# imaranresearch/LAMMPS-SPHERHARM

Hardware: NVIDIA B200
Metric: contact_pair_evals_per_s (higher is better)
Workload: dtype f64

## Files before the change

lammps-spherharm_b200/csrc/device_math.cuh:

```cuda
#pragma once
#include <cuda_runtime.h>
#include <stdint.h>

namespace shgpu {

struct DevShape {
  int lmax, nterms, nq, nchunks;
  double rmax, rmin, rmax2, rmin2, mass, inv_mass;
  double inertia[3], com[3], Rp[9];
  const double *Ap;
  const double2 *ab;
  const double *px, *py, *pz;
  const double *nx, *ny, *nz;
  int n_theta, n_phi;
  int tab_off;
  int nterms4;
  const float *row_x;
  const float2 *cube_ul;
  int cube_n, pad2_;
  const float4 *pf4;
  const float *cube_w2[4];
  double cache_delta[4];
};

__device__ __forceinline__ void quat_to_mat(const double q[4], double R[9]) {
  const double w2 = q[0] * q[0], i2 = q[1] * q[1], j2 = q[2] * q[2], k2 = q[3] * q[3];
  const double twoij = (2.0 * q[1]) * q[2], twoik = (2.0 * q[1]) * q[3], twojk = (2.0 * q[2]) * q[3];
  const double twoiw = (2.0 * q[1]) * q[0], twojw = (2.0 * q[2]) * q[0], twokw = (2.0 * q[3]) * q[0];
  R[0] = ((w2 + i2) - j2) - k2;  R[1] = twoij - twokw;          R[2] = twojw + twoik;
  R[3] = twoij + twokw;          R[4] = ((w2 - i2) + j2) - k2;  R[5] = twojk - twoiw;
  R[6] = twoik - twojw;          R[7] = twojk + twoiw;          R[8] = ((w2 - i2) - j2) + k2;
}

__device__ __forceinline__ double sh_radius_folded(int L, const double *__restrict__ Ap,
                                                   const double2 *__restrict__ ab, double s0, double s1,
                                                   double s2, double rho2, double &rho_out) {
  const double rho = sqrt(rho2);
  const double inv = 1.0 / rho;
  const double x = s2 * inv, zx = s0 * inv, zy = s1 * inv;
  double u = 1.0, v = 0.0, r = 0.0;
  int base = 0;
  for (int m = 0; m <= L; m++) {
    if (m > 0) {
      const double t1 = v * zy, un = fma(u, zx, -t1);
      const double t2 = v * zx, vn = fma(u, zy, t2);
      u = un; v = vn;
    }
    const double2 c0 = ab[base];
    double C = c0.x, S = c0.y;
    const int len = L - m;
    if (len >= 1) {
      double q1 = Ap[base + 1] * x, q2 = 1.0;
      const double2 c1 = ab[base + 1];
      C = fma(c1.x, q1, C); S = fma(c1.y, q1, S);
#pragma unroll 4
      for (int i = 2; i <= len; i++) {
        const double tx = Ap[base + i] * x;
        const double q = fma(tx, q1, -q2);
        const double2 ci = ab[base + i];
        C = fma(ci.x, q, C); S = fma(ci.y, q, S);
        q2 = q1; q1 = q;
      }
    }
    r = fma(u, C, r); r = fma(v, S, r);
    base += len + 1;
  }
  rho_out = rho;
  return r;
}

__device__ __forceinline__ void sh_radius_folded_x2(int L, const double *__restrict__ Ap,
                                                    const double2 *__restrict__ ab, const double sA[3],
                                                    double rhoA2, const double sB[3], double rhoB2, double &rhoA,
                                                    double &rhoB, double &rA_out, double &rB_out) {
  const double rA = sqrt(rhoA2), iA = 1.0 / rA, rB = sqrt(rhoB2), iB = 1.0 / rB;
  const double xA = sA[2] * iA, zxA = sA[0] * iA, zyA = sA[1] * iA;
  const double xB = sB[2] * iB, zxB = sB[0] * iB, zyB = sB[1] * iB;
  double uA = 1.0, vA = 0.0, rrA = 0.0, uB = 1.0, vB = 0.0, rrB = 0.0;
  int base = 0;
  for (int m = 0; m <= L; m++) {
    if (m > 0) {
      const double a1 = vA * zyA, un = fma(uA, zxA, -a1), a2 = vA * zxA, vn = fma(uA, zyA, a2);
      uA = un; vA = vn;
      const double b1 = vB * zyB, wn = fma(uB, zxB, -b1), b2 = vB * zxB, yn = fma(uB, zyB, b2);
      uB = wn; vB = yn;
    }
    const double2 c0 = ab[base];
    double CA = c0.x, SA = c0.y, CB = c0.x, SB = c0.y;
    const int len = L - m;
    if (len >= 1) {
      const double ap1 = Ap[base + 1];
      double qA1 = ap1 * xA, qA2 = 1.0, qB1 = ap1 * xB, qB2 = 1.0;
      const double2 c1 = ab[base + 1];
      CA = fma(c1.x, qA1, CA); SA = fma(c1.y, qA1, SA);
      CB = fma(c1.x, qB1, CB); SB = fma(c1.y, qB1, SB);
#pragma unroll 4
      for (int i = 2; i <= len; i++) {
        const double ap = Ap[base + i];
        const double2 ci = ab[base + i];
        const double txA = ap * xA, txB = ap * xB;
        const double qA = fma(txA, qA1, -qA2), qB = fma(txB, qB1, -qB2);
        CA = fma(ci.x, qA, CA); CB = fma(ci.x, qB, CB);
        SA = fma(ci.y, qA, SA); SB = fma(ci.y, qB, SB);
        qA2 = qA1; qA1 = qA; qB2 = qB1; qB1 = qB;
      }
    }
    rrA = fma(uA, CA, rrA); rrA = fma(vA, SA, rrA);
    rrB = fma(uB, CB, rrB); rrB = fma(vB, SB, rrB);
    base += len + 1;
  }
  rhoA = rA; rhoB = rB; rA_out = rrA; rB_out = rrB;
}

template <int N>
__device__ __forceinline__ void sh_radius_folded_n(int L, const double *__restrict__ Ap, const double2 *__restrict__ ab,
                                                   const double (&s)[N][3], const double (&rho2)[N], double (&rho)[N],
                                                   double (&r_out)[N]) {
  double x[N], zx[N], zy[N], u[N], v[N], rr[N];
#pragma unroll
  for (int p = 0; p < N; p++) {
    rho[p] = sqrt(rho2[p]);
    const double inv = 1.0 / rho[p];
    x[p] = s[p][2] * inv; zx[p] = s[p][0] * inv; zy[p] = s[p][1] * inv;
    u[p] = 1.0; v[p] = 0.0; rr[p] = 0.0;
  }
  int base = 0;
  for (int m = 0; m <= L; m++) {
    if (m > 0) {
#pragma unroll
      for (int p = 0; p < N; p++) {
        const double t1 = v[p] * zy[p], un = fma(u[p], zx[p], -t1), t2 = v[p] * zx[p], vn = fma(u[p], zy[p], t2);
        u[p] = un; v[p] = vn;
      }
    }
    const double2 c0 = ab[base];
    double C[N], S[N];
#pragma unroll
    for (int p = 0; p < N; p++) { C[p] = c0.x; S[p] = c0.y; }
    const int len = L - m;
    if (len >= 1) {
      const double ap1 = Ap[base + 1];
      const double2 c1 = ab[base + 1];
      double q1[N], q2[N];
#pragma unroll
      for (int p = 0; p < N; p++) {
        q1[p] = ap1 * x[p]; q2[p] = 1.0;
        C[p] = fma(c1.x, q1[p], C[p]); S[p] = fma(c1.y, q1[p], S[p]);
      }
#pragma unroll 2
      for (int i = 2; i <= len; i++) {
        const double ap = Ap[base + i];
        const double2 ci = ab[base + i];
        double q[N];
#pragma unroll
        for (int p = 0; p < N; p++) { const double tx = ap * x[p]; q[p] = fma(tx, q1[p], -q2[p]); }
#pragma unroll
        for (int p = 0; p < N; p++) C[p] = fma(ci.x, q[p], C[p]);
#pragma unroll
        for (int p = 0; p < N; p++) S[p] = fma(ci.y, q[p], S[p]);
#pragma unroll
        for (int p = 0; p < N; p++) { q2[p] = q1[p]; q1[p] = q[p]; }
      }
    }
#pragma unroll
    for (int p = 0; p < N; p++) { rr[p] = fma(u[p], C[p], rr[p]); rr[p] = fma(v[p], S[p], rr[p]); }
    base += len + 1;
  }
#pragma unroll
  for (int p = 0; p < N; p++) r_out[p] = rr[p];
}

__device__ __forceinline__ double warp_sum(double v) {
#pragma unroll
  for (int o = 16; o > 0; o >>= 1) v += __shfl_xor_sync(0xffffffffu, v, o);
  return v;
}

__device__ __forceinline__ void omega_from_angmom(const double q[4], const double L[3], const double I[3],
                                                  double w[3]) {
  double R[9];
  quat_to_mat(q, R);
  double wb[3];
#pragma unroll
  for (int k = 0; k < 3; k++) {
    const double lb = R[k] * L[0] + R[3 + k] * L[1] + R[6 + k] * L[2];
    wb[k] = (I[k] > 0) ? lb / I[k] : 0.0;
  }
#pragma unroll
  for (int r = 0; r < 3; r++) w[r] = R[3 * r] * wb[0] + R[3 * r + 1] * wb[1] + R[3 * r + 2] * wb[2];
}

}
```

lammps-spherharm_b200/csrc/pair_split_kernels.cuh:

```cuda
#pragma once
#include "pair_kernel.cuh"

namespace shgpu {

#define SPLIT_CAP 88
#define SURV_CAP 320
#define CACHE_CAP 384

struct __align__(16) SurvRec {
  double s0, s1, s2;
  int k;
  int flag;
};

struct __align__(16) PdEntry {
  long long off;
  int cnt;
  unsigned short ntrans;
  unsigned short cnt2;
  unsigned int off2;
  unsigned short nin;
  unsigned short in[5];
};
#define PD_INLINE 5

struct __align__(16) PairHot {
  int i, j, n0, n1;
  long long off;
  int img;
  unsigned char shp_i, shp_j, pad0, pad1;
};

struct EvalPlanDev {
  int total_blocks, nshape;
  int blk_start[SH_MAX_SHAPES + 1];
  long long count[SH_MAX_SHAPES];
};

struct SplitScalars {
  unsigned long long pool_count[SH_MAX_SHAPES];
  unsigned long long in_count;
  int nbig;
  int nslow;
  int slow_counter;
  int deep_counter;
};

struct SplitArgs {
  SurvRec *pool;
  unsigned char *pool_flag;
  const long long *pool_base;
  const long long *pool_cap;
  SplitScalars *sc;
  PdEntry *pd;
  int *big_list;
  int *slow_list;
  int *inpool;
  long long in_cap;
};

struct CacheArgs {
  unsigned short *pool;
  PairHot *hot;
  unsigned long long *count;
  long long cap;
  int *overflow;
  const int *invalid;
  int enabled;
  int level;
};

__device__ __forceinline__ float fp32_margin(float t0, float t1, float t2, float ra) {
  const float sc = sqrtf(fmaf(t2, t2, fmaf(t1, t1, t0 * t0))) + ra;
  return 1.9073486e-6f * sc * sc;
}

struct NodeWindow { bool skip; float cosA, xe, se, phie; };

__device__ __forceinline__ NodeWindow make_window(const DevShape &sa, double Rb, const double *x0) {
  NodeWindow w;
  const double e0 = 2.0 * x0[0], e1 = 2.0 * x0[1], e2 = 2.0 * x0[2];
  const double D2 = e0 * e0 + e1 * e1 + e2 * e2, D = sqrt(D2);
  w.skip = D >= (sa.rmax + Rb) * (1.0 + 1e-9);
  w.cosA = -2.0f; w.xe = 1.0f; w.se = 0.0f; w.phie = 0.0f;
  if (!w.skip && D > 1e-9 * (sa.rmax + Rb)) {
    const double q = D2 - Rb * Rb;
    double rc = sa.rmin;
    if (q > 0) rc = fmin(fmax(sqrt(q), sa.rmin), sa.rmax);
    const double g = (rc * rc + q) / (2.0 * rc * D);
    w.cosA = (float)g - 3e-5f;
    if (w.cosA >= 1.0f) w.skip = true;
    w.xe = fminf(1.0f, fmaxf(-1.0f, (float)(e2 / D)));
    w.se = sqrtf(fmaxf(0.0f, 1.0f - w.xe * w.xe));
    w.phie = atan2f((float)e1, (float)e0);
    if (w.phie < 0.0f) w.phie += 6.2831853f;
  }
  return w;
}

__device__ __forceinline__ void classify_row(const DevShape &sa, const NodeWindow &w, int row, int &c0, int &ccount) {
  c0 = 0; ccount = 0;
  const int nph = sa.n_phi;
  if (row >= sa.n_theta) return;
  if (w.cosA <= -1.0f) { ccount = nph; return; }
  const float xa = sa.row_x[row];
  const float sarow = sqrtf(fmaxf(0.0f, 1.0f - xa * xa));
  const float ss = sarow * w.se, xx = xa * w.xe;
  if (xx + ss < w.cosA) return;
  const float cd = (ss > 1e-12f) ? (w.cosA - xx) / ss : -2.0f;
  if (cd <= -1.0f) { ccount = nph; return; }
  const float inv_dphi = (float)nph * 0.15915494f;
  const float dl = acosf(fminf(cd, 1.0f)) + 2e-4f;
  const int b0 = (int)ceilf((w.phie - dl) * inv_dphi - 0.5f);
  const int b1 = (int)floorf((w.phie + dl) * inv_dphi - 0.5f);
  ccount = b1 - b0 + 1;
  if (ccount >= nph) { ccount = nph; c0 = 0; }
  else if (ccount > 0) { c0 = b0 % nph; if (c0 < 0) c0 += nph; }
  else ccount = 0;
}

__device__ __forceinline__ int cube_cell(float f0, float f1, float f2, int cn) {
  const float ax = fabsf(f0), ay = fabsf(f1), az = fabsf(f2);
  int face; float ma, uu, vv;
  if (ax >= ay && ax >= az) { face = f0 > 0 ? 0 : 1; ma = ax; uu = f1; vv = f2; }
  else if (ay >= az) { face = f1 > 0 ? 2 : 3; ma = ay; uu = f0; vv = f2; }
  else { face = f2 > 0 ? 4 : 5; ma = az; uu = f0; vv = f1; }
  const float im = __fdividef(1.0f, fmaxf(ma, 1e-30f)), hn = 0.5f * (float)cn;
  const int iu = min(cn - 1, max(0, (int)((uu * im + 1.0f) * hn)));
  const int iv = min(cn - 1, max(0, (int)((vv * im + 1.0f) * hn)));
  return (face * cn + iu) * cn + iv;
}

__device__ __forceinline__ double pose_element(const PairArgs &A, int a, int b, double dd0, double dd1, double dd2, int l) {
  const int st = A.stride;
  if (l < 9) {
    const int r = l / 3, k = l - 3 * r;
    double m = A.Rs[(0 + r) * st + b] * A.Rs[(0 + k) * st + a];
    m = fma(A.Rs[(3 + r) * st + b], A.Rs[(3 + k) * st + a], m);
    m = fma(A.Rs[(6 + r) * st + b], A.Rs[(6 + k) * st + a], m);
    return m;
  } else if (l < 12) {
    const int r = l - 9;
    double tt = A.Rs[(0 + r) * st + b] * dd0;
    tt = fma(A.Rs[(3 + r) * st + b], dd1, tt);
    tt = fma(A.Rs[(6 + r) * st + b], dd2, tt);
    return tt;
  }
  const int r = l - 12;
  double hx = A.Rs[(0 + r) * st + a] * dd0;
  hx = fma(A.Rs[(3 + r) * st + a], dd1, hx);
  hx = fma(A.Rs[(6 + r) * st + a], dd2, hx);
  return -0.5 * hx;
}
__device__ __forceinline__ void pose_to_smem(const PairArgs &A, int a, int b, double dd0, double dd1, double dd2, int lane,
                                             double *pose) {
  __syncwarp();
  if (lane < 15) pose[lane] = pose_element(A, a, b, dd0, dd1, dd2, lane);
  __syncwarp();
}

__device__ __forceinline__ int exact_node_stage(const double *M, const double *t, double p0, double p1, double p2, double rmax2,
                                                double rmin2, const float2 *__restrict__ cube, int cn, int use_bounds,
                                                double &s0, double &s1, double &s2) {
  s0 = fma(M[0], p0, t[0]); s0 = fma(M[1], p1, s0); s0 = fma(M[2], p2, s0);
  s1 = fma(M[3], p0, t[1]); s1 = fma(M[4], p1, s1); s1 = fma(M[5], p2, s1);
  s2 = fma(M[6], p0, t[2]); s2 = fma(M[7], p1, s2); s2 = fma(M[8], p2, s2);
  const double rho2 = fma(s2, s2, fma(s1, s1, s0 * s0));
  if (!(rho2 < rmax2)) return -1;
  if (rho2 <= rmin2) return 2;
  if (!use_bounds) return 0;
  const float2 ul = __ldg(&cube[cube_cell((float)s0, (float)s1, (float)s2, cn)]);
  if (rho2 <= (double)ul.y) return 2;
  return rho2 < (double)ul.x ? 0 : -1;
}

template <int WPB>
__global__ void __launch_bounds__(WPB * 32) pair_cache_build_kernel(PairArgs A, CacheArgs C, const int *list, const int *nlist) {
  __shared__ unsigned short s_buf[WPB][2][CACHE_CAP];
  __shared__ double s_pose[WPB][16];
  const int lane = threadIdx.x & 31, warp = threadIdx.x >> 5;
  const int nwork = list ? *nlist : A.npairs;
  for (int w = blockIdx.x * WPB + warp; w < nwork; w += gridDim.x * WPB) {
  const int p = list ? list[w] : w;
  const int i = A.pair_i[p], j = A.pair_j[p];
  double d[3];
  pair_separation(A, p, i, j, d);
  const int shp_i = A.shape[i], shp_j = A.shape[j];
  double *pose = s_pose[warp];
  int cnt0 = 0, cnt1 = 0;
  bool over = false;
  for (int dir = 0; dir < 2 && !over; dir++) {
    const int a = dir ? j : i, b = dir ? i : j;
    const DevShape &sa = A.shapes[dir ? shp_j : shp_i];
    const DevShape &sb = A.shapes[dir ? shp_i : shp_j];
    const double sgn = dir ? -1.0 : 1.0;
    pose_to_smem(A, a, b, sgn * d[0], sgn * d[1], sgn * d[2], lane, pose);
    const double *M = pose, *t = pose + 9, *x0 = pose + 12;
    const double delta = sb.cache_delta[C.level], Rb = sb.rmax + delta;
    const NodeWindow w = make_window(sa, Rb, x0);
    const float4 *__restrict__ pf = sa.pf4;
    const float *__restrict__ cube = sb.cube_w2[C.level];
    const int cn = sb.cube_n, nph = sa.n_phi, nth = sa.n_theta;
    const float fM0 = (float)M[0], fM1 = (float)M[1], fM2 = (float)M[2], fM3 = (float)M[3], fM4 = (float)M[4],
                fM5 = (float)M[5], fM6 = (float)M[6], fM7 = (float)M[7], fM8 = (float)M[8];
    const float ft0 = (float)t[0], ft1 = (float)t[1], ft2 = (float)t[2];
    const float eps = fp32_margin(ft0, ft1, ft2, (float)sa.rmax);
    const float fR2 = (float)(Rb * Rb) + eps;
    const float fin = (float)((sb.rmin + 2.0 * delta) * (sb.rmin + 2.0 * delta)) + eps;
    unsigned short *buf = s_buf[warp][dir];
    int n = 0;
    if (!w.skip) {
      for (int rb = 0; rb < nth && !over; rb += 32) {
        int c0, ccount;
        classify_row(sa, w, rb + lane, c0, ccount);
        unsigned rows = __ballot_sync(0xffffffffu, ccount > 0);
        while (rows && !over) {
          const int rl = __ffs(rows) - 1;
          rows &= rows - 1;
          const int rc0 = __shfl_sync(0xffffffffu, c0, rl), rcount = __shfl_sync(0xffffffffu, ccount, rl);
          const int rowbase = (rb + rl) * nph;
          for (int cb = 0; cb < rcount; cb += 32) {
            const int cc = cb + lane;
            bool pass = false;
            int k = 0;
            if (cc < rcount) {
              int col = rc0 + cc;
              if (col >= nph) col -= nph;
              k = rowbase + col;
              const float4 q = __ldg(&pf[k]);
              const float f0 = fmaf(fM2, q.z, fmaf(fM1, q.y, fmaf(fM0, q.x, ft0)));
              const float f1 = fmaf(fM5, q.z, fmaf(fM4, q.y, fmaf(fM3, q.x, ft1)));
              const float f2 = fmaf(fM8, q.z, fmaf(fM7, q.y, fmaf(fM6, q.x, ft2)));
              const float r2 = fmaf(f2, f2, fmaf(f1, f1, f0 * f0));
              if (r2 < fR2) pass = (r2 < fin) || (r2 < __ldg(&cube[cube_cell(f0, f1, f2, cn)]) + eps);
            }
            const unsigned pm = __ballot_sync(0xffffffffu, pass);
            if (pm) {
              const int nnew = __popc(pm);
              if (n + nnew > CACHE_CAP) { over = true; break; }
              if (pass) buf[n + __popc(pm & ((1u << lane) - 1u))] = (unsigned short)k;
              n += nnew;
            }
          }
        }
      }
    }
    if (dir) cnt1 = n; else cnt0 = n;
    __syncwarp();
  }
  const int ntot = cnt0 + cnt1;
  long long off = 0;
  if (lane == 0 && !over && ntot > 0) off = (long long)atomicAdd(C.count, (unsigned long long)ntot);
  off = __shfl_sync(0xffffffffu, off, 0);
  if (!over && ntot > 0) {
    if (off + ntot <= C.cap) {
      for (int r = lane; r < cnt0; r += 32) C.pool[off + r] = s_buf[warp][0][r];
      for (int r = lane; r < cnt1; r += 32) C.pool[off + cnt0 + r] = s_buf[warp][1][r];
    } else { if (lane == 0) *C.overflow = 1; over = true; }
  }
  if (lane == 0) {
    PairHot hrec;
    hrec.i = i; hrec.j = j; hrec.n0 = over ? -1 : cnt0; hrec.n1 = over ? -1 : cnt1; hrec.off = off; hrec.img = A.pair_img[p];
    hrec.shp_i = (unsigned char)shp_i; hrec.shp_j = (unsigned char)shp_j; hrec.pad0 = 0; hrec.pad1 = 0;
    C.hot[p] = hrec;
  }
  __syncwarp();
  }
}

__global__ void cache_remap_kernel(PairArgs A, const int *old_half_off, const int *old_pair_j, int old_nown, const PairHot *old_hot,
                                   const unsigned short *old_pool, CacheArgs C, int *fresh_list, int *nfresh, const int *amap) {
  const int p = blockIdx.x * blockDim.x + threadIdx.x;
  const int lane = threadIdx.x & 31;
  int ntot = 0, q = -1;
  PairHot hrec;
  hrec.i = hrec.j = 0; hrec.n0 = hrec.n1 = 0; hrec.off = 0; hrec.img = 0; hrec.shp_i = hrec.shp_j = 0; hrec.pad0 = hrec.pad1 = 0;
  if (p < A.npairs) {
    const int i = A.pair_i[p], j = A.pair_j[p], img = A.pair_img[p];
    const int oi = amap ? amap[i] : i, oj = amap ? amap[j] : j;
    if (oi >= 0 && oj >= 0 && oi < old_nown && oi < oj)
      for (int e = old_half_off[oi]; e < old_half_off[oi + 1]; e++)
        if (old_pair_j[e] == oj) { q = e; break; }
    if (q >= 0) {
      hrec = old_hot[q];
      if (hrec.n0 < 0 || hrec.img != img || hrec.i != oi || hrec.j != oj) q = -1;
      hrec.i = i; hrec.j = j;
    }
    if (q >= 0) ntot = hrec.n0 + hrec.n1;
    else fresh_list[atomicAdd(nfresh, 1)] = p;
  }
  int pre = ntot;
#pragma unroll
  for (int o = 1; o < 32; o <<= 1) { const int t = __shfl_up_sync(0xffffffffu, pre, o); if (lane >= o) pre += t; }
  const int wtot = __shfl_sync(0xffffffffu, pre, 31);
  long long base = 0;
  if (lane == 31 && wtot > 0) base = (long long)atomicAdd(C.count, (unsigned long long)wtot);
  base = __shfl_sync(0xffffffffu, base, 31);
  if (q >= 0) {
    const long long off = base + (pre - ntot);
    if (off + ntot <= C.cap) {
      const unsigned short *src = old_pool + hrec.off;
      for (int r = 0; r < ntot; r++) C.pool[off + r] = src[r];
      hrec.off = off;
    } else { *C.overflow = 1; hrec.n0 = -1; hrec.n1 = -1; hrec.off = 0; }
    C.hot[p] = hrec;
  }
}

__device__ __forceinline__ void store_pd(PdEntry *dst, long long off, int cnt, int ntrans, int nin, const unsigned short *in,
                                         unsigned int off2 = 0, int cnt2 = 0) {
  PdEntry e;
  e.off = off; e.cnt = cnt; e.ntrans = (unsigned short)ntrans; e.nin = (unsigned short)nin; e.off2 = off2; e.cnt2 = (unsigned short)cnt2;
#pragma unroll
  for (int q = 0; q < PD_INLINE; q++) e.in[q] = (in && q < nin) ? in[q] : (unsigned short)0;
  *dst = e;
}

struct ShapeLite {
  const float4 *pf4; const float2 *cube_ul; const double *px, *py, *pz;
  int cube_n, pad_;
  double rmax, rmax2, rmin2;
};
struct ShapeLiteTable { ShapeLite s[SH_MAX_SHAPES]; };

template <int WPB, int LPP>
__global__ void __launch_bounds__(WPB * 32, 32 / WPB) pair_cull_cached_kernel(PairArgs A, SplitArgs S, CacheArgs C, int use_bounds,
                                                                              const __grid_constant__ ShapeLiteTable T) {
  constexpr int PPW = 32 / LPP, U = 2;
  constexpr unsigned FULLSUB = LPP == 32 ? 0xffffffffu : ((1u << LPP) - 1u);
  __shared__ double s_dpose[WPB][PPW][2][12];
  __shared__ float s_fpose[WPB][PPW][2][12];
  __shared__ unsigned short s_surv[WPB][PPW][SURV_CAP];
  __shared__ signed char s_flag[WPB][PPW][SURV_CAP];
  __shared__ unsigned short s_in[WPB][PPW][2][8];
  const int lane = threadIdx.x & 31, warp = threadIdx.x >> 5;
  const int sub = lane / LPP, sl = lane % LPP, shift = sub * LPP;
  const int p = (blockIdx.x * WPB + warp) * PPW + sub;
  if (*C.invalid) return;
  const bool inrange = p < A.npairs;
  PairHot hot;
  hot.i = hot.j = 0; hot.n0 = hot.n1 = 0; hot.off = 0; hot.img = 21; hot.shp_i = hot.shp_j = 0;
  if (inrange) {
    const int4 *hp = reinterpret_cast<const int4 *>(C.hot + p);
    const int4 h0 = __ldg(hp), h1 = __ldg(hp + 1);
    hot.i = h0.x; hot.j = h0.y; hot.n0 = h0.z; hot.n1 = h0.w;
    hot.off = (long long)(((unsigned long long)(unsigned)h1.y << 32) | (unsigned)h1.x);
    hot.img = h1.z; hot.shp_i = (unsigned char)(h1.w & 255); hot.shp_j = (unsigned char)((h1.w >> 8) & 255);
  }
  if (inrange && hot.n0 < 0 && sl == 0) S.slow_list[atomicAdd(&S.sc->nslow, 1)] = p;
  const bool cached = inrange && hot.n0 >= 0;
  const int n0 = cached ? hot.n0 : 0, n1 = cached ? hot.n1 : 0, ntot = n0 + n1;
  if (cached && ntot == 0 && sl < 2) store_pd(&S.pd[2 * p + sl], 0, 0, 0, 0, nullptr);
  const int maxtot = __reduce_max_sync(0xffffffffu, ntot);
  if (maxtot == 0) return;
  const bool work = ntot > 0;
  const int i = hot.i, j = hot.j, shp_i = hot.shp_i, shp_j = hot.shp_j;
  const ShapeLite &si = T.s[shp_i], &sj = T.s[shp_j];
  if (work) {
    const int st = A.stride;
    double d[3];
#pragma unroll
    for (int k = 0; k < 3; k++) {
      double dk = A.c[k * st + i] - A.c[k * st + j];
      const int n = ((hot.img >> (2 * k)) & 3) - 1;
      if (n != 0) dk = dk - A.boxlen[k] * (double)n;
      d[k] = dk;
    }
    if (sl < 15) {
      const int half = sl >= 12, l = half ? sl - 3 : sl;
      const double sgn = half ? -1.0 : 1.0;
      const double val = pose_element(A, half ? j : i, half ? i : j, sgn * d[0], sgn * d[1], sgn * d[2], l);
      s_dpose[warp][sub][half][l] = val;
      s_fpose[warp][sub][half][l] = (float)val;
      if (sl < 9) {
        const int r = sl / 3, k = sl - 3 * r;
        s_dpose[warp][sub][1][3 * k + r] = val;
        s_fpose[warp][sub][1][3 * k + r] = (float)val;
      }
    }
  }
  __syncwarp();
  const float4 *__restrict__ pf_i = si.pf4, *__restrict__ pf_j = sj.pf4;
  const float2 *__restrict__ cube_i = si.cube_ul, *__restrict__ cube_j = sj.cube_ul;
  const int cn_i = si.cube_n, cn_j = sj.cube_n;
  const float eps0 = fp32_margin(s_fpose[warp][sub][0][9], s_fpose[warp][sub][0][10], s_fpose[warp][sub][0][11], (float)si.rmax);
  const float eps1 = fp32_margin(s_fpose[warp][sub][1][9], s_fpose[warp][sub][1][10], s_fpose[warp][sub][1][11], (float)sj.rmax);
  const float fR20 = (float)sj.rmax2 + eps0, fR21 = (float)si.rmax2 + eps1;
  const unsigned short *__restrict__ cl = C.pool + hot.off;
  unsigned short *surv = s_surv[warp][sub];
  signed char *sflag = s_flag[warp][sub];
  int nsurv = 0, ns0 = 0;
  bool big = false;
  for (int base = 0; base < maxtot; base += LPP * U) {
    int k[U];
    float4 q[U];
    bool pass[U];
#pragma unroll
    for (int u = 0; u < U; u++) {
      const int g = base + LPP * u + sl;
      k[u] = (work && !big && g < ntot) ? (int)__ldg(&cl[g]) : -1;
    }
#pragma unroll
    for (int u = 0; u < U; u++) {
      const int dirc = (base + LPP * u + sl) >= n0;
      q[u] = k[u] >= 0 ? __ldg(&(dirc ? pf_j : pf_i)[k[u]]) : make_float4(0.f, 0.f, 0.f, 0.f);
    }
#pragma unroll
    for (int u = 0; u < U; u++) {
      const int dirc = (base + LPP * u + sl) >= n0;
      const float *fp = s_fpose[warp][sub][dirc];
      const float f0 = fmaf(fp[2], q[u].z, fmaf(fp[1], q[u].y, fmaf(fp[0], q[u].x, fp[9])));
      const float f1 = fmaf(fp[5], q[u].z, fmaf(fp[4], q[u].y, fmaf(fp[3], q[u].x, fp[10])));
      const float f2 = fmaf(fp[8], q[u].z, fmaf(fp[7], q[u].y, fmaf(fp[6], q[u].x, fp[11])));
      const float r2 = fmaf(f2, f2, fmaf(f1, f1, f0 * f0));
      bool ok = k[u] >= 0 && r2 < (dirc ? fR21 : fR20);
      if (ok && use_bounds) ok = r2 < __ldg(&(dirc ? cube_i : cube_j)[cube_cell(f0, f1, f2, dirc ? cn_i : cn_j)]).x + (dirc ? eps1 : eps0);
      pass[u] = ok;
    }
#pragma unroll
    for (int u = 0; u < U; u++) {
      const unsigned mine = (__ballot_sync(0xffffffffu, pass[u]) >> shift) & FULLSUB;
      if (mine) {
        const int nnew = __popc(mine);
        if (nsurv + nnew > SURV_CAP) big = true;
        else {
          if (pass[u]) surv[nsurv + __popc(mine & ((1u << sl) - 1u))] = (unsigned short)k[u];
          const int nd0 = n0 - (base + LPP * u);
          ns0 += nd0 >= LPP ? nnew : (nd0 <= 0 ? 0 : __popc(mine & ((1u << nd0) - 1u)));
          nsurv += nnew;
        }
      }
    }
  }
  __syncwarp();
  const bool live = work && !big;
  const int maxs = __reduce_max_sync(0xffffffffu, live ? nsurv : 0);
  int c0d0 = 0, c0d1 = 0, c2d0 = 0, c2d1 = 0;
  for (int gb = 0; gb < maxs; gb += LPP) {
    const int g = gb + sl;
    int fl = -1;
    if (live && g < nsurv) {
      const int dirc = g >= ns0, k = surv[g];
      const ShapeLite &sa = dirc ? sj : si;
      const ShapeLite &sb = dirc ? si : sj;
      const double *M = s_dpose[warp][sub][dirc];
      double s0, s1, s2;
      fl = exact_node_stage(M, M + 9, sa.px[k], sa.py[k], sa.pz[k], sb.rmax2, sb.rmin2, sb.cube_ul, sb.cube_n, use_bounds, s0, s1, s2);
      sflag[g] = (signed char)fl;
    }
    const unsigned m0 = (__ballot_sync(0xffffffffu, fl == 0) >> shift) & FULLSUB;
    const unsigned m2 = (__ballot_sync(0xffffffffu, fl == 2) >> shift) & FULLSUB;
    const int nd0 = ns0 - gb;
    const unsigned md0 = nd0 >= LPP ? FULLSUB : (nd0 <= 0 ? 0u : ((1u << nd0) - 1u));
    c0d0 += __popc(m0 & md0); c0d1 += __popc(m0 & ~md0);
    c2d0 += __popc(m2 & md0); c2d1 += __popc(m2 & ~md0);
  }
  const int r0 = c0d0, r1 = c0d1, x0 = max(0, c2d0 - PD_INLINE), x1 = max(0, c2d1 - PD_INLINE);
  long long off0 = 0, off1 = 0, xoff = 0;
  if (live && sl == 0 && r0 > 0) off0 = (long long)atomicAdd(&S.sc->pool_count[shp_j], (unsigned long long)r0);
  if (live && sl == 1 && r1 > 0) off1 = (long long)atomicAdd(&S.sc->pool_count[shp_i], (unsigned long long)r1);
  if (live && sl == 2 && x0 + x1 > 0) xoff = (long long)atomicAdd(&S.sc->in_count, (unsigned long long)(x0 + x1));
  off0 = __shfl_sync(0xffffffffu, off0, shift);
  off1 = __shfl_sync(0xffffffffu, off1, shift + 1);
  xoff = __shfl_sync(0xffffffffu, xoff, shift + 2);
  if (live && (off0 + r0 > S.pool_cap[shp_j] || off1 + r1 > S.pool_cap[shp_i] || xoff + x0 + x1 > S.in_cap)) big = true;
  if (work && big && sl == 0) {
    store_pd(&S.pd[2 * p], 0, -1, 0, 0, nullptr);
    store_pd(&S.pd[2 * p + 1], 0, -1, 0, 0, nullptr);
    S.big_list[atomicAdd(&S.sc->nbig, 1)] = p;
  }
  const bool wr = work && !big;
  const long long base0 = S.pool_base[shp_j] + off0, base1 = S.pool_base[shp_i] + off1;
  int w0d0 = 0, w0d1 = 0, w2d0 = 0, w2d1 = 0;
  for (int gb = 0; gb < maxs; gb += LPP) {
    const int g = gb + sl;
    const bool v = wr && g < nsurv;
    const int fl = v ? (int)sflag[g] : -1;
    const unsigned m0 = (__ballot_sync(0xffffffffu, fl == 0) >> shift) & FULLSUB;
    const unsigned m2 = (__ballot_sync(0xffffffffu, fl == 2) >> shift) & FULLSUB;
    const int nd0 = ns0 - gb;
    const unsigned md0 = nd0 >= LPP ? FULLSUB : (nd0 <= 0 ? 0u : ((1u << nd0) - 1u));
    const unsigned lt = (1u << sl) - 1u;
    if (fl >= 0) {
      const int dirc = g >= ns0, k = surv[g];
      const unsigned dm = dirc ? ~md0 : md0;
      const int rank0 = (dirc ? w0d1 : w0d0) + __popc(m0 & dm & lt);
      const int rank2 = (dirc ? w2d1 : w2d0) + __popc(m2 & dm & lt);
      int slot = -1;
      if (fl == 0) slot = rank0;
      else if (rank2 < PD_INLINE) s_in[warp][sub][dirc][rank2] = (unsigned short)k;
      else S.inpool[xoff + (dirc ? x0 : 0) + (rank2 - PD_INLINE)] = k;
      if (slot >= 0) {
        const ShapeLite &sa = dirc ? sj : si;
        const double *M = s_dpose[warp][sub][dirc], *t = M + 9;
        const double p0 = sa.px[k], p1 = sa.py[k], p2 = sa.pz[k];
        SurvRec r;
        r.s0 = fma(M[0], p0, t[0]); r.s0 = fma(M[1], p1, r.s0); r.s0 = fma(M[2], p2, r.s0);
        r.s1 = fma(M[3], p0, t[1]); r.s1 = fma(M[4], p1, r.s1); r.s1 = fma(M[5], p2, r.s1);
        r.s2 = fma(M[6], p0, t[2]); r.s2 = fma(M[7], p1, r.s2); r.s2 = fma(M[8], p2, r.s2);
        r.k = k; r.flag = fl;
        const long long idx = (dirc ? base1 : base0) + slot;
        S.pool[idx] = r;
        S.pool_flag[idx] = 0;
      }
    }
    w0d0 += __popc(m0 & md0); w0d1 += __popc(m0 & ~md0);
    w2d0 += __popc(m2 & md0); w2d1 += __popc(m2 & ~md0);
  }
  __syncwarp();
  if (wr && sl < 2) {
    if (sl == 0) store_pd(&S.pd[2 * p], base0, r0, n0, min(c2d0, PD_INLINE), s_in[warp][sub][0], (unsigned int)xoff, x0);
    else store_pd(&S.pd[2 * p + 1], base1, r1, n1, min(c2d1, PD_INLINE), s_in[warp][sub][1], (unsigned int)(xoff + x0), x1);
  }
}

template <int WPB>
__global__ void __launch_bounds__(WPB * 32) pair_cull_window_kernel(PairArgs A, SplitArgs S, CacheArgs C, int use_bounds) {
  __shared__ __align__(16) SurvRec s_rec[WPB][2][SPLIT_CAP];
  __shared__ double s_pose[WPB][16];
  __shared__ unsigned short s_cand[WPB][64];
  __shared__ unsigned short s_in[WPB][2][8];
  const int lane = threadIdx.x & 31, warp = threadIdx.x >> 5;
  const bool all = !C.enabled || *C.invalid != 0;
  for (;;) {
    int w = 0;
    if (lane == 0) w = atomicAdd(&S.sc->slow_counter, 1);
    w = __shfl_sync(0xffffffffu, w, 0);
    const int nwork = all ? A.npairs : *(volatile int *)&S.sc->nslow;
    if (w >= nwork) break;
    const int p = all ? w : S.slow_list[w];
    const int i = A.pair_i[p], j = A.pair_j[p];
    double d[3];
    pair_separation(A, p, i, j, d);
    const int shp_i = A.shape[i], shp_j = A.shape[j];
    double *pose = s_pose[warp];
    int cnt0 = 0, cnt1 = 0, nin0 = 0, nin1 = 0, nt0 = 0, nt1 = 0;
    bool big = false;
    for (int dir = 0; dir < 2 && !big; dir++) {
      const int a = dir ? j : i, b = dir ? i : j;
      const DevShape &sa = A.shapes[dir ? shp_j : shp_i];
      const DevShape &sb = A.shapes[dir ? shp_i : shp_j];
      const double sgn = dir ? -1.0 : 1.0;
      pose_to_smem(A, a, b, sgn * d[0], sgn * d[1], sgn * d[2], lane, pose);
      const double *M = pose, *t = pose + 9, *x0 = pose + 12;
      const double rmax2 = sb.rmax2, rmin2 = sb.rmin2;
      const double *__restrict__ nodes = sa.px;
      const int nq = sa.nq;
      const float2 *__restrict__ cube = sb.cube_ul;
      const int cn = sb.cube_n;
      SurvRec *buf = s_rec[warp][dir];
      unsigned short *cand = s_cand[warp], *inl = s_in[warp][dir];
      int queued = 0, nin = 0, n_trans = 0;
      auto exact_stage = [&](bool valid, int k) {
        int flag = -1;
        double s0 = 0, s1 = 0, s2 = 0;
        if (valid) flag = exact_node_stage(M, t, nodes[k], nodes[nq + k], nodes[2 * nq + k], rmax2, rmin2, cube, cn, use_bounds, s0, s1, s2);
        const unsigned m2 = __ballot_sync(0xffffffffu, flag == 2);
        const int rank2 = nin + __popc(m2 & ((1u << lane) - 1u));
        const bool inline_it = flag == 2 && rank2 < PD_INLINE;
        if (inline_it) inl[rank2] = (unsigned short)k;
        nin = min(PD_INLINE, nin + __popc(m2));
        const bool rec = flag >= 0 && !inline_it;
        const unsigned sm = __ballot_sync(0xffffffffu, rec);
        if (sm) {
          const int nnew = __popc(sm);
          if (queued + nnew > SPLIT_CAP) { big = true; return; }
          if (rec) {
            SurvRec r; r.s0 = s0; r.s1 = s1; r.s2 = s2; r.k = k; r.flag = flag;
            buf[queued + __popc(sm & ((1u << lane) - 1u))] = r;
          }
          queued += nnew;
        }
      };
      const NodeWindow wd = make_window(sa, sb.rmax, x0);
      if (!wd.skip) {
        const float4 *__restrict__ pf = sa.pf4;
        const float fM0 = (float)M[0], fM1 = (float)M[1], fM2 = (float)M[2], fM3 = (float)M[3], fM4 = (float)M[4],
                    fM5 = (float)M[5], fM6 = (float)M[6], fM7 = (float)M[7], fM8 = (float)M[8];
        const float ft0 = (float)t[0], ft1 = (float)t[1], ft2 = (float)t[2];
        const float eps = fp32_margin(ft0, ft1, ft2, (float)sa.rmax);
        const float frmax2 = (float)rmax2 + eps;
        const int nth = sa.n_theta, nph = sa.n_phi;
        int ncand = 0;
        for (int rb = 0; rb < nth && !big; rb += 32) {
          int c0, ccount;
          classify_row(sa, wd, rb + lane, c0, ccount);
          unsigned rows = __ballot_sync(0xffffffffu, ccount > 0);
          while (rows && !big) {
            const int rl = __ffs(rows) - 1;
            rows &= rows - 1;
            const int rc0 = __shfl_sync(0xffffffffu, c0, rl), rcount = __shfl_sync(0xffffffffu, ccount, rl);
            const int rowbase = (rb + rl) * nph;
            for (int cb = 0; cb < rcount && !big; cb += 32) {
              const int cc = cb + lane;
              bool pass = false;
              int k = 0;
              if (cc < rcount) {
                int col = rc0 + cc;
                if (col >= nph) col -= nph;
                k = rowbase + col;
                const float4 q = __ldg(&pf[k]);
                const float f0 = fmaf(fM2, q.z, fmaf(fM1, q.y, fmaf(fM0, q.x, ft0)));
                const float f1 = fmaf(fM5, q.z, fmaf(fM4, q.y, fmaf(fM3, q.x, ft1)));
                const float f2 = fmaf(fM8, q.z, fmaf(fM7, q.y, fmaf(fM6, q.x, ft2)));
                const float r2 = fmaf(f2, f2, fmaf(f1, f1, f0 * f0));
                if (r2 < frmax2) pass = !use_bounds || r2 < __ldg(&cube[cube_cell(f0, f1, f2, cn)]).x + eps;
              }
              n_trans += min(32, rcount - cb);
              const unsigned pm = __ballot_sync(0xffffffffu, pass);
              if (pm) {
                if (pass) cand[ncand + __popc(pm & ((1u << lane) - 1u))] = (unsigned short)k;
                ncand += __popc(pm);
                __syncwarp();
                if (ncand >= 32) {
                  exact_stage(true, (int)cand[lane]);
                  __syncwarp();
                  const int rem = ncand - 32;
                  unsigned short mv = 0;
                  if (lane < rem) mv = cand[32 + lane];
                  __syncwarp();
                  if (lane < rem) cand[lane] = mv;
                  ncand = rem;
                  __syncwarp();
                }
              }
            }
          }
        }
        if (!big && ncand > 0) { exact_stage(lane < ncand, lane < ncand ? (int)cand[lane] : 0); __syncwarp(); }
      }
      if (dir) { cnt1 = queued; nin1 = nin; nt1 = n_trans; } else { cnt0 = queued; nin0 = nin; nt0 = n_trans; }
    }
    __syncwarp();
    long long off0 = 0, off1 = 0;
    if (!big) {
      if (lane == 0 && cnt0 > 0) off0 = (long long)atomicAdd(&S.sc->pool_count[shp_j], (unsigned long long)cnt0);
      if (lane == 1 && cnt1 > 0) off1 = (long long)atomicAdd(&S.sc->pool_count[shp_i], (unsigned long long)cnt1);
      off0 = __shfl_sync(0xffffffffu, off0, 0);
      off1 = __shfl_sync(0xffffffffu, off1, 1);
      if (off0 + cnt0 > S.pool_cap[shp_j] || off1 + cnt1 > S.pool_cap[shp_i]) big = true;
    }
    if (big) {
      if (lane == 0) {
        store_pd(&S.pd[2 * p], 0, -1, 0, 0, nullptr);
        store_pd(&S.pd[2 * p + 1], 0, -1, 0, 0, nullptr);
        S.big_list[atomicAdd(&S.sc->nbig, 1)] = p;
      }
    } else {
      const long long base0 = S.pool_base[shp_j] + off0, base1 = S.pool_base[shp_i] + off1;
      for (int r = lane; r < cnt0; r += 32) { S.pool[base0 + r] = s_rec[warp][0][r]; S.pool_flag[base0 + r] = s_rec[warp][0][r].flag == 2 ? 1 : 0; }
      for (int r = lane; r < cnt1; r += 32) { S.pool[base1 + r] = s_rec[warp][1][r]; S.pool_flag[base1 + r] = s_rec[warp][1][r].flag == 2 ? 1 : 0; }
      if (lane == 0) store_pd(&S.pd[2 * p], base0, cnt0, nt0, nin0, s_in[warp][0]);
      if (lane == 1) store_pd(&S.pd[2 * p + 1], base1, cnt1, nt1, nin1, s_in[warp][1]);
    }
    __syncwarp();
  }
}

__global__ void eval_plan_kernel(SplitArgs S, int nshape, int recs_per_block, EvalPlanDev *plan) {
  if (threadIdx.x != 0 || blockIdx.x != 0) return;
  int nblk = 0;
  for (int s = 0; s < nshape; s++) {
    const long long cnt = min((long long)S.sc->pool_count[s], S.pool_cap[s]);
    plan->blk_start[s] = nblk;
    plan->count[s] = cnt;
    nblk += (int)((cnt + recs_per_block - 1) / recs_per_block);
  }
  plan->blk_start[nshape] = nblk;
  plan->total_blocks = nblk;
  plan->nshape = nshape;
}

template <int WPB, int PTS, int MINB>
__global__ void __launch_bounds__(WPB * 32, MINB) pair_eval_kernel(const DevShape *shapes, SplitArgs S, const EvalPlanDev *plan,
                                                                   unsigned long long *counters, int chunked) {
  extern __shared__ __align__(16) unsigned char smem_raw[];
  constexpr int RPW = 32 * PTS;
  const int total = plan->total_blocks, nshape = plan->nshape;
  const int chunk = (total + (int)gridDim.x - 1) / (int)gridDim.x;
  const int b0 = chunked ? blockIdx.x * chunk : blockIdx.x, b1 = chunked ? min(total, b0 + chunk) : total;
  const int bstep = chunked ? 1 : (int)gridDim.x;
  if (b0 >= b1) return;
  const int lane = threadIdx.x & 31, warp = threadIdx.x >> 5;
  double2 *s_ab = reinterpret_cast<double2 *>(smem_raw);
  double *s_Ap = nullptr;
  int cur = -1, s = 0;
  unsigned long long nev_total = 0;
  for (int blk = b0; blk < b1; blk += bstep) {
    while (s + 1 < nshape && blk >= plan->blk_start[s + 1]) s++;
    const DevShape &sh = shapes[s];
    if (s != cur) {
      __syncthreads();
      s_Ap = reinterpret_cast<double *>(s_ab + sh.nterms4 + 4);
      for (int t = threadIdx.x; t < sh.nterms4 + 4; t += WPB * 32) { s_ab[t] = sh.ab[t]; s_Ap[t] = sh.Ap[t]; }
      __syncthreads();
      cur = s;
    }
    const long long n = plan->count[s];
    const long long r0 = ((long long)(blk - plan->blk_start[s]) * WPB + warp) * RPW;
    if (r0 >= n) continue;
    SurvRec *rec = S.pool + S.pool_base[s];
    unsigned char *flg = S.pool_flag + S.pool_base[s];
    const int L = sh.lmax;
    int nev = 0;
    if (PTS == 2) {
      const long long ia = r0 + lane, ib = r0 + 32 + lane;
      const bool va = ia < n, vb = ib < n;
      if (__ballot_sync(0xffffffffu, vb)) {
        const long long ja = va ? ia : r0, jb = vb ? ib : ja;
        const SurvRec ra = rec[ja], rb = rec[jb];
        const double sA[3] = {ra.s0, ra.s1, ra.s2}, sB[3] = {rb.s0, rb.s1, rb.s2};
        const double rhoA2 = fma(sA[2], sA[2], fma(sA[1], sA[1], sA[0] * sA[0]));
        const double rhoB2 = fma(sB[2], sB[2], fma(sB[1], sB[1], sB[0] * sB[0]));
        double rhoA, rhoB, rA, rB;
        sh_radius_folded_x2(L, s_Ap, s_ab, sA, rhoA2, sB, rhoB2, rhoA, rhoB, rA, rB);
        if (va && ra.flag == 0) { flg[ia] = rhoA < rA ? 1 : 0; nev++; }
        if (vb && rb.flag == 0) { flg[ib] = rhoB < rB ? 1 : 0; nev++; }
      } else if (va) {
        const SurvRec ra = rec[ia];
        const double rho2 = fma(ra.s2, ra.s2, fma(ra.s1, ra.s1, ra.s0 * ra.s0));
        double rho;
        const double r = sh_radius_folded(L, s_Ap, s_ab, ra.s0, ra.s1, ra.s2, rho2, rho);
        if (ra.flag == 0) { flg[ia] = rho < r ? 1 : 0; nev++; }
      }
    } else {
      double sv[PTS][3], rho2[PTS], rho[PTS], rr[PTS];
      int fl[PTS];
      long long idx[PTS];
#pragma unroll
      for (int q = 0; q < PTS; q++) {
        idx[q] = r0 + 32 * q + lane;
        const bool v = idx[q] < n;
        const SurvRec r = rec[v ? idx[q] : r0];
        sv[q][0] = r.s0; sv[q][1] = r.s1; sv[q][2] = r.s2;
        fl[q] = v ? r.flag : 3;
        rho2[q] = fma(r.s2, r.s2, fma(r.s1, r.s1, r.s0 * r.s0));
      }
      sh_radius_folded_n<PTS>(L, s_Ap, s_ab, sv, rho2, rho, rr);
#pragma unroll
      for (int q = 0; q < PTS; q++)
        if (fl[q] == 0) { flg[idx[q]] = rho[q] < rr[q] ? 1 : 0; nev++; }
    }
    nev_total += nev;
  }
  nev_total = __reduce_add_sync(0xffffffffu, (unsigned)nev_total);
  if (lane == 0 && nev_total) { atomicAdd(&counters[2], nev_total); atomicAdd(&counters[5], nev_total); }
}

struct NodeSums { double S0, S1, S2, Av, T0, T1, T2, G0, G1, G2; int n; };

__device__ __forceinline__ void add_node(NodeSums &a, const double *__restrict__ nodes, int nq, int k, const double x0[3]) {
  const double p0 = nodes[k], p1 = nodes[nq + k], p2 = nodes[2 * nq + k];
  const double n0 = nodes[3 * nq + k], n1 = nodes[4 * nq + k], n2 = nodes[5 * nq + k];
  const double dp0 = p0 - x0[0], dp1 = p1 - x0[1], dp2 = p2 - x0[2];
  const double dn = fma(dp2, n2, fma(dp1, n1, dp0 * n0));
  a.S0 += n0; a.S1 += n1; a.S2 += n2;
  a.Av += dn;
  a.T0 += fma(p1, n2, -(p2 * n1));
  a.T1 += fma(p2, n0, -(p0 * n2));
  a.T2 += fma(p0, n1, -(p1 * n0));
  a.G0 = fma(dp0, dn, a.G0); a.G1 = fma(dp1, dn, a.G1); a.G2 = fma(dp2, dn, a.G2);
  a.n++;
}

template <int MINB>
__global__ void __launch_bounds__(128, MINB) pair_reduce_kernel(PairArgs A, SplitArgs S) {
  const int p = blockIdx.x * blockDim.x + threadIdx.x;
  int c_pairs = 0, c_trans = 0, c_inside = 0, c_ghost = 0;
  if (p < A.npairs) {
    const int4 *ep = reinterpret_cast<const int4 *>(S.pd + 2 * (size_t)p);
    const int4 e0a = __ldg(ep), e0b = __ldg(ep + 1), e1a = __ldg(ep + 2), e1b = __ldg(ep + 3);
    const int cnt0 = e0a.z, cnt1 = e1a.z;
    if (cnt0 >= 0) {
      const int i = A.pair_i[p], j = A.pair_j[p];
      c_pairs = 1; c_trans = (e0a.w & 0xffff) + (e1a.w & 0xffff); c_ghost = j >= A.nlocal;
      const int nin0 = e0b.y & 0xffff, nin1 = e1b.y & 0xffff;
      const int xc0 = (e0a.w >> 16) & 0xffff, xc1 = (e1a.w >> 16) & 0xffff;
      double out[14];
#pragma unroll
      for (int r = 0; r < 14; r++) out[r] = 0.0;
      const long long off0 = (long long)(((unsigned long long)(unsigned)e0a.y << 32) | (unsigned)e0a.x);
      const long long off1 = (long long)(((unsigned long long)(unsigned)e1a.y << 32) | (unsigned)e1a.x);
      unsigned long long msk0 = 0, msk1 = 0;
      bool any = nin0 > 0 || nin1 > 0 || xc0 > 0 || xc1 > 0;
      {
        const int m0 = min(cnt0, 64), m1 = min(cnt1, 64);
        for (int r = 0; r < m0; r += 8) {
#pragma unroll
          for (int q = 0; q < 8; q++) if (r + q < m0 && S.pool_flag[off0 + r + q]) msk0 |= 1ull << (r + q);
        }
        for (int r = 0; r < m1; r += 8) {
#pragma unroll
          for (int q = 0; q < 8; q++) if (r + q < m1 && S.pool_flag[off1 + r + q]) msk1 |= 1ull << (r + q);
        }
        any = any || msk0 || msk1 || cnt0 > 64 || cnt1 > 64;
      }
      if (any) {
        const int st = A.stride;
        double d[3];
        pair_separation(A, p, i, j, d);
        const int shp_i = A.shape[i], shp_j = A.shape[j];
        double Ss[2][3], Ts[2][3], Gs[2][3], Asum[2];
        int ninside_pair = 0;
#pragma unroll
        for (int dir = 0; dir < 2; dir++) {
          const int a = dir ? j : i;
          const DevShape &sa = A.shapes[dir ? shp_j : shp_i];
          const double sgn = dir ? -1.0 : 1.0;
          const long long off = dir ? off1 : off0;
          const int cnt = dir ? cnt1 : cnt0, nin = dir ? nin1 : nin0, xc = dir ? xc1 : xc0;
          unsigned long long msk = dir ? msk1 : msk0;
          const int4 eb = dir ? e1b : e0b;
          NodeSums acc;
          acc.S0 = acc.S1 = acc.S2 = acc.Av = acc.T0 = acc.T1 = acc.T2 = acc.G0 = acc.G1 = acc.G2 = 0.0; acc.n = 0;
          double Ra[9];
#pragma unroll
          for (int e = 0; e < 9; e++) Ra[e] = A.Rs[e * st + a];
          if (msk || nin > 0 || cnt > 64 || xc > 0) {
            double x0[3];
#pragma unroll
            for (int r = 0; r < 3; r++) {
              double hx = Ra[0 + r] * (sgn * d[0]);
              hx = fma(Ra[3 + r], sgn * d[1], hx);
              hx = fma(Ra[6 + r], sgn * d[2], hx);
              x0[r] = -0.5 * hx;
            }
            const double *__restrict__ nodes = sa.px;
            const int nq = sa.nq;
            while (msk) {
              const int r = __ffsll((long long)msk) - 1;
              msk &= msk - 1;
              add_node(acc, nodes, nq, S.pool[off + r].k, x0);
            }
            for (int r = 64; r < cnt; r++)
              if (S.pool_flag[off + r]) add_node(acc, nodes, nq, S.pool[off + r].k, x0);
            {
              const unsigned xo = (unsigned)eb.x;
              for (int r = 0; r < xc; r++) add_node(acc, nodes, nq, S.inpool[xo + r], x0);
            }
            for (int q = 0; q < nin; q++) {
              const int h = q + 3;
              const unsigned w = (h >> 1) == 0 ? (unsigned)eb.x : (h >> 1) == 1 ? (unsigned)eb.y : (h >> 1) == 2 ? (unsigned)eb.z : (unsigned)eb.w;
              add_node(acc, nodes, nq, (int)((w >> (16 * (h & 1))) & 0xffffu), x0);
            }
          }
#pragma unroll
          for (int r = 0; r < 3; r++) {
            Ss[dir][r] = Ra[3 * r] * acc.S0 + Ra[3 * r + 1] * acc.S1 + Ra[3 * r + 2] * acc.S2;
            Ts[dir][r] = Ra[3 * r] * acc.T0 + Ra[3 * r + 1] * acc.T1 + Ra[3 * r + 2] * acc.T2;
            Gs[dir][r] = 0.25 * (Ra[3 * r] * acc.G0 + Ra[3 * r + 1] * acc.G1 + Ra[3 * r + 2] * acc.G2);
          }
          Asum[dir] = acc.Av;
          ninside_pair += acc.n;
        }
        c_inside = ninside_pair;
        const double V = Asum[0] / 3.0 + Asum[1] / 3.0;
        if (ninside_pair > 0 && V > 0) {
          const double kk = A.pk[shp_i * SH_MAX_SHAPES + shp_j], mm = A.pm[shp_i * SH_MAX_SHAPES + shp_j];
          double E, pr;
          if (mm == 1.0) { E = kk * V; pr = kk; }
          else { const double pw = pow(V, mm - 1.0); E = kk * pw * V; pr = mm * kk * pw; }
          out[0] = V; out[1] = E;
          double li[3], lj[3];
#pragma unroll
          for (int r = 0; r < 3; r++) {
            li[r] = A.c[r * st + i] - A.x[r * st + i];
            lj[r] = A.c[r * st + j] - A.x[r * st + j];
          }
          const double *Sij = Ss[0], *Sji = Ss[1], *Tij = Ts[0], *Tji = Ts[1];
          const double Ti[3] = {Tij[0] + (li[1] * Sij[2] - li[2] * Sij[1]), Tij[1] + (li[2] * Sij[0] - li[0] * Sij[2]),
                                Tij[2] + (li[0] * Sij[1] - li[1] * Sij[0])};
          const double Tj[3] = {Tji[0] + (lj[1] * Sji[2] - lj[2] * Sji[1]), Tji[1] + (lj[2] * Sji[0] - lj[0] * Sji[2]),
                                Tji[2] + (lj[0] * Sji[1] - lj[1] * Sji[0])};
#pragma unroll
          for (int r = 0; r < 3; r++) {
            out[2 + r] = -pr * (0.5 * (Sij[r] - Sji[r]));
            out[5 + r] = -pr * Ti[r];
            out[8 + r] = -pr * Tj[r];
            out[11 + r] = (A.c[r * st + i] - 0.5 * d[r]) + (Gs[0][r] + Gs[1][r]) / V;
          }
          if (A.dissip) contact_dissipation(A, i, j, shp_i, shp_j, d, lj, out);
        }
      }
#pragma unroll
      for (int r = 0; r < 14; r++) A.pres[(size_t)r * A.pres_stride + p] = out[r];
      const int eij = A.pair_eij[p], eji = A.pair_eji[p];
#pragma unroll
      for (int r = 0; r < 3; r++) {
        A.slot[(size_t)r * A.slot_stride + eij] = out[2 + r];
        A.slot[(size_t)(3 + r) * A.slot_stride + eij] = out[5 + r];
        if (eji >= 0) {
          A.slot[(size_t)r * A.slot_stride + eji] = -out[2 + r];
          A.slot[(size_t)(3 + r) * A.slot_stride + eji] = out[8 + r];
        }
      }
    }
  }
  c_pairs = __reduce_add_sync(0xffffffffu, c_pairs); c_trans = __reduce_add_sync(0xffffffffu, c_trans);
  c_inside = __reduce_add_sync(0xffffffffu, c_inside); c_ghost = __reduce_add_sync(0xffffffffu, c_ghost);
  if ((threadIdx.x & 31) == 0) {
    if (c_pairs) atomicAdd(&A.counters[0], (unsigned long long)c_pairs);
    if (c_trans) atomicAdd(&A.counters[1], (unsigned long long)c_trans);
    if (c_inside) atomicAdd(&A.counters[3], (unsigned long long)c_inside);
    if (c_ghost) atomicAdd(&A.counters[4], (unsigned long long)c_ghost);
  }
}

}
```

lammps-spherharm_b200/csrc/shgpu_api.cu:

```cuda
#include <cuda_runtime.h>

#include <algorithm>
#include <cmath>
#include <cstdio>
#include <cstring>
#include <string>
#include <vector>

#include "../../include/shgpu.h"
#include "devbuf.h"
#include "dd_types.h"
#include "neighbor_kernels.cuh"
#include "pair_kernel.cuh"
#include "pair_warp_kernel.cuh"
#include "pair_split_kernels.cuh"
#include "shape_tables.h"
#include "step_kernels.cuh"
#include "atom_stress_kernels.cuh"

using namespace shgpu;

namespace {

struct ShapeDev {
  DevBuf<double> Ap, node;
  DevBuf<double2> ab;
  DevBuf<float> row_x, cubew[SH_CACHE_LEVELS];
  DevBuf<float2> cube;
  DevBuf<float4> pf4;
};

}

enum { CACHE_INVALID = 0, CACHE_VALID = 1, CACHE_REMAP = 2 };

struct sh_ctx {
  std::string err;
  int device = 0, sm_count = 148;
  cudaStream_t stream = nullptr;
  double lo[3] = {-1e30, -1e30, -1e30}, hi[3] = {1e30, 1e30, 1e30};
  int periodic[3] = {0, 0, 0};
  bool box_set = false;
  int n_theta = 32, n_phi = 64;
  std::vector<ShapeTables> shapes;
  std::vector<ShapeDev> shape_dev;
  std::vector<DevShape> shape_host_view;
  DevBuf<DevShape> d_shapes;
  bool shapes_dirty = true;
  int total_terms = 0;
  std::vector<double> pk, pm;
  std::vector<double> pgn, pgt, pmu;
  bool dissip = false;
  DevBuf<double> d_pk, d_pm, d_pgn, d_pgt, d_pmu, stress_part;
  bool coeff_dirty = true;
  WallSet walls{};
  double g[3] = {0, 0, 0}, skin = 0.0, dt = 1e-4, gamma_lin = 0.0, gamma_rot = 0.0;
  int neigh_every = 1, neigh_check = 1;
  int64_t n = 0, nghost = 0;
  int stride = 0;
  DevBuf<double> x, v, q, L, f, tq, c, Rs, c0, wallf, ewall, ke;
  DevBuf<int> shape;
  std::vector<int64_t> tag;
  DevBuf<long long> d_tag;
  bool tags_host_valid = true;
  DevBuf<double> gf;
  double time = 0.0;
  DdCtx dd;
  int *h_lagflag = nullptr;
  cudaEvent_t ev_lag[2] = {nullptr, nullptr};
  int lag_slot = 0; bool lag_pending = false, lag_mode = true, lag_pred_valid = false;
  bool cache_sync_ranks = false;
  int64_t step_index = 0, cache_build_step = -10;
  double cache_time = 0.0;
  bool step_trace = false;
  std::vector<cudaEvent_t> ev_step;
  std::vector<float> step_ms;
  std::vector<int> step_flags, step_flags_last;
  DevBuf<int> cell_of, cell_count, cell_start, cell_fill, cell_atoms, tile_sum, cnt_full, cnt_half, nbr_off, half_off,
      nbr_j, pair_i, pair_j, pair_eij, pair_eji, pair_img, scalars;
  DevBuf<double> bbox, slot, pres, stage;
  DevBuf<SurvRec> pool;
  DevBuf<unsigned char> pool_flag;
  DevBuf<long long> pool_base, pool_cap;
  DevBuf<PdEntry> pd;
  DevBuf<PairHot> cache_hot[2];
  DevBuf<SplitScalars> split_sc;
  DevBuf<EvalPlanDev> eval_plan;
  DevBuf<int> big_list, slow_list, split_flags;
  DevBuf<int> inpool;
  long long h_in_cap = 0;
  std::vector<long long> h_pool_cap;
  unsigned long long *h_pool_count = nullptr;
  SplitScalars *h_split_sc = nullptr;
  int *h_cache_invalid = nullptr;
  cudaEvent_t ev_sc = nullptr;
  bool sc_pending = false;
  int sc_nshape = 0;
  double sec_eval = 0, sec_cull = 0, sec_reduce = 0, sec_deep = 0, sec_cache = 0; int64_t eval_launches = 0;
  std::vector<int> ev2_kind;
  int64_t big_pairs = 0, slow_pairs = 0, pool_grows = 0, cache_builds = 0;
  int cache_level = 0, cache_level_pin = -1;
  int64_t cache_age = 0;
  bool cache_exhausted = false;
  int cube_n = 0;
  int reduce_occ = 0;
  int eval_pts = 0, eval_occ = 0, eval_mode = 0;
  long long last_records = 0;
  DevBuf<unsigned short> cache_pool[2];
  DevBuf<int> old_half_off, old_pair_j, fresh_list;
  int old_nown = 0, cache_cur = 0;
  DevBuf<double> old_c, old_cc0, old_cq0;
  DevBuf<long long> old_tag;
  DevBuf<int> ghost_hash, amap;
  int old_n = 0, old_stride = 0, ghost_hash_size = 0;
  bool carry = false;
  int64_t cache_remaps = 0, atoms_epoch = 0, cache_epoch = -1;
  DevBuf<unsigned long long> cache_count;
  long long cache_cap = 0;
  int cache_state = 0;
  DevBuf<double> cc0, cq0, drift;
  bool eval_pending = false;
  DevBuf<unsigned long long> counters;
  int npairs = 0, nentries = 0, nrows = 0;
  int slot_stride = 0, pres_stride = 0;
  int *h_pinned = nullptr;
  bool forces_valid = false, list_valid = false;
  int64_t steps_since_build = 0;
  int64_t neighbor_builds = 0, kernel_launches = 0;
  std::vector<cudaEvent_t> ev, ev2;
  size_t ev_used = 0, ev2_used = 0;
  double sec_pair = 0, sec_neigh = 0, sec_comm = 0, sec_other = 0, sec_run_last = 0, sec_run_total = 0;
  cudaEvent_t run_e0 = nullptr, run_e1 = nullptr;
  int64_t pair_launches = 0;
  DevBuf<double> as_vir, as_kin, as_en, as_send, as_recv;
  DevBuf<int> as_cnt, as_epair;
  int tune_threads = 0, tune_ctas_per_sm = 0, tune_variant = 0, tune_cull_wpb = 0, tune_cull_lpp = 0;
};

namespace {

int fail(sh_ctx *h, const std::string &m) { h->err = m; return -1; }
int cuda_fail(sh_ctx *h, const char *where, cudaError_t e) {
  h->err = std::string(where) + ": " + cudaGetErrorString(e);
  return -2;
}
#define CU(call) do { cudaError_t _e = (call); if (_e != cudaSuccess) return cuda_fail(h, #call, _e); } while (0)

inline int cdiv(int64_t a, int b) { return (int)((a + b - 1) / b); }

AtomView view(sh_ctx *h) {
  AtomView A;
  A.x = h->x.p; A.v = h->v.p; A.q = h->q.p; A.L = h->L.p; A.f = h->f.p; A.tq = h->tq.p;
  A.c = h->c.p; A.Rs = h->Rs.p; A.c0 = h->c0.p; A.wallf = h->wallf.p; A.shape = h->shape.p;
  A.cc0 = h->cc0.p; A.cq0 = h->cq0.p;
  A.n = (int)(h->n - h->nghost); A.stride = h->stride;
  return A;
}
AtomView view_all(sh_ctx *h) { AtomView A = view(h); A.n = (int)h->n; return A; }

int upload_shapes(sh_ctx *h) {
  if (!h->shapes_dirty) return 0;
  const int ns = (int)h->shapes.size();
  h->shape_dev.resize(ns);
  h->shape_host_view.resize(ns);
  try {
    for (int s = 0; s < ns; s++) {
      const ShapeTables &t = h->shapes[s];
      ShapeDev &d = h->shape_dev[s];
      if (d.Ap.p) continue;
      const int tpad = (t.nterms + 3) / 4 * 4 + 4;
      d.Ap.ensure(tpad); d.ab.ensure(tpad); d.node.ensure((size_t)6 * t.nq); d.row_x.ensure(t.n_theta);
      CU(cudaMemset(d.Ap.p, 0, tpad * sizeof(double))); CU(cudaMemset(d.ab.p, 0, tpad * sizeof(double2)));
      {
        std::vector<float> rx(t.row_x.begin(), t.row_x.end());
        CU(cudaMemcpy(d.row_x.p, rx.data(), rx.size() * sizeof(float), cudaMemcpyHostToDevice));
        std::vector<float4> pf((size_t)t.nq);
        for (int k = 0; k < t.nq; k++) pf[k] = make_float4((float)t.node_p[0][k], (float)t.node_p[1][k], (float)t.node_p[2][k], 0.0f);
        d.pf4.ensure(pf.size());
        CU(cudaMemcpy(d.pf4.p, pf.data(), pf.size() * sizeof(float4), cudaMemcpyHostToDevice));
        for (int lv = 0; lv < SH_CACHE_LEVELS; lv++) {
          d.cubew[lv].ensure(t.cube_wide2[lv].size());
          CU(cudaMemcpy(d.cubew[lv].p, t.cube_wide2[lv].data(), t.cube_wide2[lv].size() * sizeof(float), cudaMemcpyHostToDevice));
        }
        std::vector<float2> ul(t.cube_ub2.size());
        for (size_t c = 0; c < ul.size(); c++) ul[c] = make_float2(t.cube_ub2[c], t.cube_lb2[c]);
        d.cube.ensure(ul.size());
        CU(cudaMemcpy(d.cube.p, ul.data(), ul.size() * sizeof(float2), cudaMemcpyHostToDevice));
      }
      std::vector<double2> ab(t.nterms);
      for (int k = 0; k < t.nterms; k++) ab[k] = make_double2(t.ah[k], t.bh[k]);
      CU(cudaMemcpy(d.Ap.p, t.Ap.data(), t.nterms * sizeof(double), cudaMemcpyHostToDevice));
      CU(cudaMemcpy(d.ab.p, ab.data(), t.nterms * sizeof(double2), cudaMemcpyHostToDevice));
      for (int e = 0; e < 3; e++) {
        CU(cudaMemcpy(d.node.p + (size_t)e * t.nq, t.node_p[e].data(), t.nq * sizeof(double), cudaMemcpyHostToDevice));
        CU(cudaMemcpy(d.node.p + (size_t)(3 + e) * t.nq, t.node_n[e].data(), t.nq * sizeof(double), cudaMemcpyHostToDevice));
      }
      DevShape &v = h->shape_host_view[s];
      v.lmax = t.lmax; v.nterms = t.nterms; v.nq = t.nq; v.nchunks = (t.nq + 31) / 32;
      v.rmax = t.rmax; v.rmin = t.rmin; v.rmax2 = t.rmax * t.rmax; v.rmin2 = t.rmin * t.rmin;
      v.mass = t.mass; v.inv_mass = 1.0 / t.mass;
      for (int e = 0; e < 3; e++) { v.inertia[e] = t.inertia[e]; v.com[e] = t.com[e]; }
      for (int r = 0; r < 3; r++) for (int cidx = 0; cidx < 3; cidx++) v.Rp[3 * r + cidx] = t.Rp[r][cidx];
      v.Ap = d.Ap.p; v.ab = d.ab.p;
      v.px = d.node.p; v.py = d.node.p + t.nq; v.pz = d.node.p + 2 * (size_t)t.nq;
      v.nx = d.node.p + 3 * (size_t)t.nq; v.ny = d.node.p + 4 * (size_t)t.nq; v.nz = d.node.p + 5 * (size_t)t.nq;
      v.n_theta = t.n_theta; v.n_phi = t.n_phi; v.nterms4 = (t.nterms + 3) / 4 * 4; v.row_x = d.row_x.p; v.cube_ul = d.cube.p; v.cube_n = t.cube_n; v.pad2_ = 0; v.pf4 = d.pf4.p;
      for (int lv = 0; lv < SH_CACHE_LEVELS; lv++) { v.cube_w2[lv] = d.cubew[lv].p; v.cache_delta[lv] = t.cache_delta[lv]; }
    }
    int off = 0;
    for (int s = 0; s < ns; s++) { h->shape_host_view[s].tab_off = off; off += h->shape_host_view[s].nterms4 + 4; }
    h->total_terms = off;
    h->d_shapes.ensure(std::max(ns, 1));
  } catch (std::string &e) { return fail(h, e); }
  if (ns) CU(cudaMemcpy(h->d_shapes.p, h->shape_host_view.data(), ns * sizeof(DevShape), cudaMemcpyHostToDevice));
  h->shapes_dirty = false;
  return 0;
}

int upload_coeffs(sh_ctx *h) {
  if (!h->coeff_dirty) return 0;
  const size_t nn = SH_MAX_SHAPES * SH_MAX_SHAPES;
  try { h->d_pk.ensure(nn); h->d_pm.ensure(nn); h->d_pgn.ensure(nn); h->d_pgt.ensure(nn); h->d_pmu.ensure(nn); }
  catch (std::string &e) { return fail(h, e); }
  CU(cudaMemcpy(h->d_pk.p, h->pk.data(), nn * sizeof(double), cudaMemcpyHostToDevice));
  CU(cudaMemcpy(h->d_pm.p, h->pm.data(), nn * sizeof(double), cudaMemcpyHostToDevice));
  CU(cudaMemcpy(h->d_pgn.p, h->pgn.data(), nn * sizeof(double), cudaMemcpyHostToDevice));
  CU(cudaMemcpy(h->d_pgt.p, h->pgt.data(), nn * sizeof(double), cudaMemcpyHostToDevice));
  CU(cudaMemcpy(h->d_pmu.p, h->pmu.data(), nn * sizeof(double), cudaMemcpyHostToDevice));
  h->coeff_dirty = false;
  return 0;
}

int exclusive_scan(sh_ctx *h, const int *in, int *out, int n, int *d_total) {
  const int ntiles = std::max(1, cdiv(n, SCAN_TILE));
  try { h->tile_sum.ensure(ntiles); } catch (std::string &e) { return fail(h, e); }
  scan_tile_kernel<<<ntiles, SCAN_THREADS, 0, h->stream>>>(in, out, h->tile_sum.p, n);
  scan_sums_kernel<<<1, 1024, 0, h->stream>>>(h->tile_sum.p, ntiles, d_total);
  scan_add_kernel<<<std::max(1, cdiv(n, 256)), 256, 0, h->stream>>>(out, h->tile_sum.p, n, d_total);
  h->kernel_launches += 3;
  return 0;
}

int ev_tick(sh_ctx *h, int kind) {
  if (h->ev2_used + 2 > h->ev2.size()) return 0;
  h->ev2_kind[h->ev2_used / 2] = kind;
  if (cudaEventRecord(h->ev2[h->ev2_used], h->stream) != cudaSuccess) return -2;
  return 0;
}
void ev_tock(sh_ctx *h) {
  if (h->ev2_used + 2 <= h->ev2.size()) { cudaEventRecord(h->ev2[h->ev2_used + 1], h->stream); h->ev2_used += 2; }
}

int build_neighbors(sh_ctx *h) {
  const int n = (int)h->n, st = h->stride, nown = (int)(h->n - h->nghost);
  if (ev_tick(h, 5)) return -2;
  const bool keep_cache = h->carry || (h->cache_state == CACHE_VALID && h->list_valid && h->nghost == 0 && h->npairs > 0 && h->atoms_epoch == h->cache_epoch);
  if (keep_cache && !h->carry) {
    try { h->old_half_off.ensure((size_t)nown + 2); h->old_pair_j.ensure((size_t)h->npairs + 1); } catch (std::string &e) { return fail(h, e); }
    CU(cudaMemcpyAsync(h->old_half_off.p, h->half_off.p, ((size_t)nown + 1) * sizeof(int), cudaMemcpyDeviceToDevice, h->stream));
    CU(cudaMemcpyAsync(h->old_pair_j.p, h->pair_j.p, (size_t)h->npairs * sizeof(int), cudaMemcpyDeviceToDevice, h->stream));
    h->old_nown = nown;
  }
  CU(cudaMemsetAsync(h->scalars.p + 1, 0, sizeof(int), h->stream));
  double rmaxg = 0;
  for (auto &s : h->shapes) rmaxg = std::max(rmaxg, s.rmax);
  const double cut = 2.0 * rmaxg + h->skin;
  BinGrid G;
  G.skin = h->skin;
  bool need_bbox = false;
  for (int d = 0; d < 3; d++) {
    G.periodic[d] = h->periodic[d];
    G.boxlen[d] = h->hi[d] - h->lo[d];
    if (h->periodic[d]) {
      if (G.boxlen[d] < 2.0 * cut) return fail(h, "periodic box shorter than 2x cutoff");
    } else need_bbox = true;
  }
  double bmin[3] = {0, 0, 0}, bmax[3] = {0, 0, 0};
  if (need_bbox && n > 0) {
    auto enc = [](double v) { long long b; std::memcpy(&b, &v, 8); return b >= 0 ? b : (b ^ 0x7fffffffffffffffLL); };
    auto dec = [](long long b) { long long u = b >= 0 ? b : (b ^ 0x7fffffffffffffffLL); double v; std::memcpy(&v, &u, 8); return v; };
    long long init[6];
    for (int d = 0; d < 3; d++) { init[d] = enc(1e300); init[3 + d] = enc(-1e300); }
    CU(cudaMemcpyAsync(h->bbox.p, init, sizeof init, cudaMemcpyHostToDevice, h->stream));
    bbox_kernel<<<std::min(1024, cdiv(n, 256)), 256, 0, h->stream>>>(h->c.p, n, st, h->bbox.p);
    h->kernel_launches++;
    long long out[6];
    CU(cudaMemcpyAsync(out, h->bbox.p, sizeof out, cudaMemcpyDeviceToHost, h->stream));
    CU(cudaStreamSynchronize(h->stream));
    for (int d = 0; d < 3; d++) { bmin[d] = dec(out[d]); bmax[d] = dec(out[3 + d]); }
    for (int d = 0; d < 3; d++) if (!std::isfinite(bmin[d]) || !std::isfinite(bmax[d])) return fail(h, "non-finite atom coordinates");
  }
  int64_t ncell = 1;
  for (int d = 0; d < 3; d++) {
    if (h->periodic[d]) { G.lo[d] = h->lo[d]; G.len[d] = G.boxlen[d]; }
    else { G.lo[d] = bmin[d]; G.len[d] = (bmax[d] - bmin[d]) * (1.0 + 1e-9) + 1e-9; }
    int nc = (int)std::floor(G.len[d] / cut);
    nc = std::max(1, std::min(nc, 1024));
    if (h->periodic[d] && nc < 3) nc = 1;
    G.nc[d] = nc;
    ncell *= nc;
  }
  while (ncell > std::max<int64_t>(4096, 8 * (int64_t)n)) {
    int dmax = 0;
    for (int d = 1; d < 3; d++) if (G.nc[d] > G.nc[dmax]) dmax = d;
    ncell /= G.nc[dmax];
    G.nc[dmax] = std::max(1, G.nc[dmax] / 2);
    if (h->periodic[dmax] && G.nc[dmax] < 3) G.nc[dmax] = 1;
    ncell *= G.nc[dmax];
  }
  try {
    h->cell_of.ensure(n + 1); h->cell_count.ensure(ncell + 1); h->cell_start.ensure(ncell + 2); h->cell_fill.ensure(ncell + 1);
    h->cell_atoms.ensure(n + 1); h->cnt_full.ensure(n + 1); h->cnt_half.ensure(n + 1); h->nbr_off.ensure(n + 2); h->half_off.ensure(n + 2);
  } catch (std::string &e) { return fail(h, e); }
  const int nb = std::max(1, cdiv(n, 256));
  CU(cudaMemsetAsync(h->cell_count.p, 0, (ncell + 1) * sizeof(int), h->stream));
  CU(cudaMemsetAsync(h->cell_fill.p, 0, (ncell + 1) * sizeof(int), h->stream));
  bin_count_kernel<<<nb, 256, 0, h->stream>>>(h->c.p, n, st, G, h->cell_of.p, h->cell_count.p);
  if (exclusive_scan(h, h->cell_count.p, h->cell_start.p, (int)ncell, h->scalars.p)) return -1;
  bin_fill_kernel<<<nb, 256, 0, h->stream>>>(n, h->cell_of.p, h->cell_start.p, h->cell_fill.p, h->cell_atoms.p);
  bin_sort_kernel<<<cdiv(ncell, 256), 256, 0, h->stream>>>((int)ncell, h->cell_start.p, h->cell_atoms.p);
  const bool newton = h->dd.on && h->dd.newton && h->nghost > 0;
  const int nrows = newton ? n : nown;
  const long long *ntags = newton ? h->d_tag.p : nullptr;
  h->nrows = nrows;
  const int nbo = std::max(1, cdiv(nrows, 256));
  nbr_count_kernel<<<nbo, 256, 0, h->stream>>>(h->c.p, h->shape.p, h->d_shapes.p, nrows, nown, ntags, st, G, h->cell_of.p, h->cell_start.p,
                                              h->cell_atoms.p, h->cnt_full.p, h->cnt_half.p);
  h->kernel_launches += 4;
  int nentries = 0, npairs = 0;
  if (exclusive_scan(h, h->cnt_full.p, h->nbr_off.p, nrows, h->scalars.p + 8)) return -1;
  if (exclusive_scan(h, h->cnt_half.p, h->half_off.p, nrows, h->scalars.p + 9)) return -1;
  CU(cudaMemcpyAsync(h->h_pinned, h->scalars.p + 8, 2 * sizeof(int), cudaMemcpyDeviceToHost, h->stream));
  CU(cudaStreamSynchronize(h->stream));
  nentries = h->h_pinned[0]; npairs = h->h_pinned[1];
  try {
    h->nbr_j.ensure(nentries + 1); h->pair_i.ensure(npairs + 1); h->pair_j.ensure(npairs + 1);
    h->pair_eij.ensure(npairs + 1); h->pair_eji.ensure(npairs + 1); h->pair_img.ensure(npairs + 1);
    if ((size_t)nentries + 1 > (size_t)h->slot_stride) { h->slot_stride = (int)((nentries + 1) * 1.25) + 64; h->slot.release(); h->slot.ensure((size_t)6 * h->slot_stride); }
    if ((size_t)npairs + 1 > (size_t)h->pres_stride) { h->pres_stride = (int)((npairs + 1) * 1.25) + 64; h->pres.release(); h->pres.ensure((size_t)14 * h->pres_stride); }
  } catch (std::string &e) { return fail(h, e); }
  nbr_fill_kernel<<<nbo, 256, 0, h->stream>>>(h->c.p, h->shape.p, h->d_shapes.p, nrows, nown, ntags, st, G, h->cell_of.p, h->cell_start.p,
                                             h->cell_atoms.p, h->nbr_off.p, h->half_off.p, h->nbr_j.p, h->pair_i.p,
                                             h->pair_j.p, h->pair_eij.p, h->pair_img.p);
  pair_reverse_kernel<<<std::max(1, cdiv(npairs, 256)), 256, 0, h->stream>>>(npairs, nrows, h->pair_i.p, h->pair_j.p, h->nbr_off.p,
                                                                             h->nbr_j.p, h->pair_eji.p);
  copy_origin_kernel<<<nb, 256, 0, h->stream>>>(h->c.p, h->c0.p, n, st);
  h->kernel_launches += 3;
  ev_tock(h);
  CU(cudaGetLastError());
  h->npairs = npairs; h->nentries = nentries;
  h->list_valid = true; h->steps_since_build = 0; h->neighbor_builds++;
  h->cache_state = keep_cache ? CACHE_REMAP : CACHE_INVALID;
  if (!keep_cache) h->carry = false;
  return 0;
}

int drain_events(sh_ctx *h) {
  if (h->ev_used == 0 && h->ev2_used == 0) return 0;
  CU(cudaStreamSynchronize(h->stream));
  for (size_t k = 0; k + 1 < h->ev2_used; k += 2) {
    float ms = 0;
    cudaEventElapsedTime(&ms, h->ev2[k], h->ev2[k + 1]);
    double *dst[8] = {&h->sec_cull, &h->sec_eval, &h->sec_reduce, &h->sec_deep, &h->sec_cache, &h->sec_neigh, &h->sec_comm, &h->sec_other};
    *dst[h->ev2_kind[k / 2] & 7] += ms * 1e-3;
  }
  h->ev2_used = 0;
  for (size_t k = 0; k + 1 < h->ev_used; k += 2) {
    float ms = 0;
    cudaEventElapsedTime(&ms, h->ev[k], h->ev[k + 1]);
    h->sec_pair += ms * 1e-3;
  }
  h->ev_used = 0;
  return 0;
}

}
#include "dd_host.cuh"
namespace {

template <int NT>
int launch_pair(sh_ctx *h, const PairArgs &A, int ctas_per_sm, size_t smem) {
  CU(cudaFuncSetAttribute(pair_kernel<NT>, cudaFuncAttributeMaxDynamicSharedMemorySize, (int)std::max<size_t>(smem, 48 * 1024)));
  int occ = 0;
  CU(cudaOccupancyMaxActiveBlocksPerMultiprocessor(&occ, pair_kernel<NT>, NT, smem));
  if (occ < 1) return fail(h, "pair kernel does not fit on an SM (shared memory)");
  if (ctas_per_sm > 0) occ = std::min(occ, ctas_per_sm);
  const int grid = std::max(1, std::min(A.npairs, occ * h->sm_count));
  pair_kernel<NT><<<grid, NT, smem, h->stream>>>(A);
  return 0;
}

template <int NW, bool SMEM_TABLES>
int launch_pair_warp(sh_ctx *h, const PairArgs &A, int ctas_per_sm, int max_grid = 1 << 30) {
  const size_t smem = pair_warp_smem_bytes(h->total_terms, NW, SMEM_TABLES);
  CU(cudaFuncSetAttribute(pair_warp_kernel<NW, SMEM_TABLES>, cudaFuncAttributeMaxDynamicSharedMemorySize, (int)std::max<size_t>(smem, 48 * 1024)));
  int occ = 0;
  CU(cudaOccupancyMaxActiveBlocksPerMultiprocessor(&occ, pair_warp_kernel<NW, SMEM_TABLES>, NW * 32, smem));
  if (occ < 1) return fail(h, "pair warp kernel does not fit on an SM");
  if (ctas_per_sm > 0) occ = std::min(occ, ctas_per_sm);
  const int grid = std::max(1, std::min(std::min((A.npairs + NW - 1) / NW, occ * h->sm_count), max_grid));
  pair_warp_kernel<NW, SMEM_TABLES><<<grid, NW * 32, smem, h->stream>>>(A, (int)h->shapes.size(), h->total_terms, (h->tune_variant & 2) ? 0 : 1);
  return 0;
}

int launch_fused(sh_ctx *h, const PairArgs &P, int max_grid = 1 << 30) {
  const bool fits = pair_warp_smem_bytes(h->total_terms, 16, true) <= 200 * 1024;
  const int tw = h->tune_threads ? h->tune_threads : 512;
  const int cps = h->tune_ctas_per_sm;
  if (fits) {
    if (tw == 256) return launch_pair_warp<8, true>(h, P, cps, max_grid);
    if (tw == 128) return launch_pair_warp<4, true>(h, P, cps, max_grid);
    if (tw == 384) return launch_pair_warp<12, true>(h, P, cps, max_grid);
    return launch_pair_warp<16, true>(h, P, cps, max_grid);
  }
  if (tw == 256) return launch_pair_warp<8, false>(h, P, cps, max_grid);
  return launch_pair_warp<16, false>(h, P, cps, max_grid);
}

template <int WPB, int PTS, int MINB>
int launch_eval(sh_ctx *h, const SplitArgs &S, int maxT) {
  const size_t smem = (size_t)maxT * 24 + 32;
  auto kern = pair_eval_kernel<WPB, PTS, MINB>;
  CU(cudaFuncSetAttribute(kern, cudaFuncAttributeMaxDynamicSharedMemorySize, (int)std::max<size_t>(smem, 48 * 1024)));
  int occ = 0;
  CU(cudaOccupancyMaxActiveBlocksPerMultiprocessor(&occ, kern, WPB * 32, smem));
  if (occ < 1) return fail(h, "pair_eval_kernel does not fit on an SM");
  const int rpb = WPB * 32 * PTS;
  eval_plan_kernel<<<1, 32, 0, h->stream>>>(S, (int)h->shapes.size(), rpb, h->eval_plan.p);
  const int chunked = h->eval_mode == 2;
  int grid = occ * h->sm_count;
  if (!chunked) {
    long long est = h->last_records > 0 ? h->last_records + h->last_records / 16 : 0;
    if (est == 0) for (long long c : h->h_pool_cap) est += c;
    grid = (int)std::max<long long>(grid, std::min<long long>(est / rpb + (long long)h->shapes.size() + 1, 1 << 22));
  }
  kern<<<grid, WPB * 32, smem, h->stream>>>(h->d_shapes.p, S, h->eval_plan.p, h->counters.p, chunked);
  h->kernel_launches += 2;
  return 0;
}

int absorb_split_feedback(sh_ctx *h) {
  if (!h->sc_pending) return 0;
  CU(cudaEventSynchronize(h->ev_sc));
  h->sc_pending = false;
  const SplitScalars &sc = *h->h_split_sc;
  h->big_pairs += sc.nbig; h->slow_pairs += sc.nslow;
  const int ns = std::min<int>(h->sc_nshape, (int)h->h_pool_cap.size());
  for (int s = 0; s < ns; s++)
    if ((long long)sc.pool_count[s] > h->h_pool_cap[s] * 9 / 10) {
      h->h_pool_cap[s] = (long long)(sc.pool_count[s] * 3 / 2) + 4096;
      h->pool_grows++;
    }
  if ((long long)sc.in_count > h->h_in_cap * 9 / 10) { h->h_in_cap = (long long)(sc.in_count * 3 / 2) + 4096; h->pool_grows++; }
  h->last_records = 0;
  for (int s = 0; s < ns; s++) h->last_records += (long long)std::min<unsigned long long>(sc.pool_count[s], (unsigned long long)h->h_pool_cap[s]);
  if (!h->cache_sync_ranks && (h->h_cache_invalid[0] != 0 || h->h_cache_invalid[1] != 0) && h->cache_state != CACHE_INVALID) { h->cache_state = CACHE_INVALID; h->cache_exhausted = true; }
  return 0;
}

int run_split_pipeline(sh_ctx *h, PairArgs &P) {
  const int ns = (int)h->shapes.size(), np = P.npairs;
  constexpr int WPB = 8;
  int rc;
  if ((rc = absorb_split_feedback(h))) return rc;
  try {
    h->pd.ensure((size_t)2 * np + 2); h->big_list.ensure(np + 1); h->slow_list.ensure(np + 1);
    h->pool_base.ensure(SH_MAX_SHAPES); h->pool_cap.ensure(SH_MAX_SHAPES); h->split_sc.ensure(1); h->eval_plan.ensure(1); h->split_flags.ensure(4);
  } catch (std::string &e) { return fail(h, e); }
  if (!h->h_pool_count) {
    CU(cudaMallocHost(&h->h_pool_count, 8 * sizeof(unsigned long long)));
    CU(cudaMallocHost(&h->h_split_sc, sizeof(SplitScalars)));
    CU(cudaMallocHost(&h->h_cache_invalid, 2 * sizeof(int)));
    CU(cudaEventCreateWithFlags(&h->ev_sc, cudaEventDisableTiming));
  }
  if ((int)h->h_pool_cap.size() != ns) {
    h->h_pool_cap.assign(ns, std::max<long long>(4096, (long long)np * 24 / std::max(1, ns) * 2));
  }
  auto tick = [&](int kind) -> int { return ev_tick(h, kind); };
  auto tock = [&]() { ev_tock(h); };
  const int use_bounds = (h->tune_variant & 2) ? 0 : 1;
  CacheArgs C;
  C.enabled = (h->tune_variant & (8 | 2)) ? 0 : 1;
  C.invalid = h->scalars.p + 3;
  if (C.enabled) {
    const int cur = h->cache_cur;
    try { h->cache_hot[cur].ensure((size_t)np + 2); h->cache_count.ensure(2); h->fresh_list.ensure((size_t)np + 2); }
    catch (std::string &e) { return fail(h, e); }
    double pc[3];
    for (int d = 0; d < 3; d++) pc[d] = (h->hi[d] < 1e29 && h->lo[d] > -1e29) ? 0.5 * (h->lo[d] + h->hi[d]) : 0.0;
    auto check_validity = [&]() -> int {
      double dmin = 1e300;
      for (auto &sh : h->shapes) dmin = std::min(dmin, sh.cache_delta[h->cache_level]);
      double rmaxg = 0;
      for (auto &sh : h->shapes) rmaxg = std::max(rmaxg, sh.rmax);
      const double rpair = 2.0 * rmaxg + 2.0 * h->skin;
      CU(cudaMemsetAsync(h->drift.p, 0, CACHE_FIT_N * sizeof(double), h->stream));
      cache_drift_kernel<<<cdiv(h->n, 256), 256, 0, h->stream>>>(view_all(h), pc[0], pc[1], pc[2], h->drift.p);
      cache_fit_solve_kernel<<<1, 32, 0, h->stream>>>(h->drift.p, h->drift.p + 32);
      cache_check_kernel<<<cdiv(h->n, 256), 256, 0, h->stream>>>(view_all(h), h->d_shapes.p, h->cache_level, 0.5 * dmin, h->drift.p + 32,
                                                                 pc[0], pc[1], pc[2], rpair, h->scalars.p + 3);
      h->kernel_launches += 3;
      return 0;
    };
    if (h->cache_state == CACHE_REMAP && h->cache_level + 1 < SH_CACHE_LEVELS && !(h->tune_variant & 32)) {
      const int nxt = 1 - cur;
      try { h->cache_hot[nxt].ensure((size_t)np + 2); h->cache_pool[nxt].ensure((size_t)h->cache_cap + 64); }
      catch (std::string &e) { return fail(h, e); }
      const int *amap = nullptr;
      if (h->carry) {
        try { h->amap.ensure((size_t)h->n + 2); } catch (std::string &e) { return fail(h, e); }
        const int nstay = h->dd.last_nstay, nown = (int)(h->n - h->nghost);
        CU(cudaMemsetAsync(h->drift.p + 64, 0, CACHE_FIT_N * sizeof(double), h->stream));
        const double le_doff = h->dd.le_rate * h->dd.glen[1] * (h->time - h->cache_time);
        dd_cache_map_kernel<<<cdiv(h->n, 256), 256, 0, h->stream>>>(view_all(h), h->d_tag.p, nown, nstay, h->dd.order.p, h->old_tag.p, h->old_c.p,
                                                                    h->old_stride, h->old_nown, h->old_n, h->ghost_hash.p, h->ghost_hash_size,
                                                                    0.25 * h->dd.G.rc * h->dd.G.rc, h->old_cc0.p, h->old_cq0.p, h->amap.p, h->dd.glen[1], le_doff,
                                                                    pc[0], pc[1], pc[2], h->drift.p + 64);
        cache_fit_solve_kernel<<<1, 32, 0, h->stream>>>(h->drift.p + 64, h->drift.p + 96);
        dd_cache_new_atoms_kernel<<<cdiv(h->n, 256), 256, 0, h->stream>>>(view_all(h), h->amap.p, h->drift.p + 96, pc[0], pc[1], pc[2]);
        h->kernel_launches += 3;
        amap = h->amap.p;
        h->carry = false; h->cache_epoch = h->atoms_epoch;
      }
      if ((rc = check_validity())) return rc;
      if (tick(4)) return -2;
      CU(cudaMemsetAsync(h->cache_count.p, 0, 2 * sizeof(unsigned long long), h->stream));
      CU(cudaMemsetAsync(h->split_flags.p + 2, 0, 2 * sizeof(int), h->stream));
      C.pool = h->cache_pool[nxt].p; C.hot = h->cache_hot[nxt].p; C.count = h->cache_count.p;
      C.cap = h->cache_cap; C.overflow = h->split_flags.p + 2; C.level = h->cache_level + 1;
      cache_remap_kernel<<<cdiv(np, 256), 256, 0, h->stream>>>(P, h->old_half_off.p, h->old_pair_j.p, h->old_nown, h->cache_hot[cur].p,
                                                                h->cache_pool[cur].p, C, h->fresh_list.p, h->split_flags.p + 3, amap);
      pair_cache_build_kernel<4><<<std::max(1, std::min(cdiv(np, 4), h->sm_count * 8)), 4 * 32, 0, h->stream>>>(P, C, h->fresh_list.p, h->split_flags.p + 3);
      tock();
      h->kernel_launches += 2;
      h->cache_cur = nxt; h->cache_state = CACHE_VALID; h->cache_remaps++;
    } else if (h->cache_state != CACHE_VALID) {
      if (h->cache_level_pin >= 0) h->cache_level = h->cache_level_pin;
      else if (h->cache_exhausted) {
        if (h->cache_age < 40 && h->cache_level < 1) h->cache_level++;
        else if (h->cache_age > 400 && h->cache_level > 0) h->cache_level--;
      }
      h->cache_exhausted = false;
      if (h->cache_cap < (long long)np * 48) h->cache_cap = (long long)np * 48;
      if (tick(4)) return -2;
      for (int attempt = 0;; attempt++) {
        if (attempt > 6) return fail(h, "candidate cache kept overflowing");
        try { h->cache_pool[cur].ensure((size_t)h->cache_cap + 64); } catch (std::string &e) { return fail(h, e); }
        CU(cudaMemsetAsync(h->cache_count.p, 0, 2 * sizeof(unsigned long long), h->stream));
        CU(cudaMemsetAsync(h->split_flags.p + 2, 0, sizeof(int), h->stream));
        C.pool = h->cache_pool[cur].p; C.hot = h->cache_hot[cur].p; C.count = h->cache_count.p;
        C.cap = h->cache_cap; C.overflow = h->split_flags.p + 2; C.level = h->cache_level;
        pair_cache_build_kernel<4><<<cdiv(np, 4), 4 * 32, 0, h->stream>>>(P, C, nullptr, nullptr);
        h->kernel_launches++;
        CU(cudaMemcpyAsync(h->h_pool_count, h->cache_count.p, sizeof(unsigned long long), cudaMemcpyDeviceToHost, h->stream));
        CU(cudaMemcpyAsync(h->h_pool_count + 1, h->split_flags.p + 2, sizeof(int), cudaMemcpyDeviceToHost, h->stream));
        CU(cudaStreamSynchronize(h->stream));
        if (*reinterpret_cast<const int *>(h->h_pool_count + 1) == 0) break;
        h->cache_cap = (long long)(h->h_pool_count[0] * 3 / 2) + 4096;
      }
      cache_origin_kernel<<<cdiv(h->n, 256), 256, 0, h->stream>>>(view_all(h));
      CU(cudaMemsetAsync(h->scalars.p + 3, 0, 2 * sizeof(int), h->stream));
      tock();
      h->kernel_launches++;
      h->cache_state = CACHE_VALID; h->cache_builds++; h->cache_age = 0; h->cache_epoch = h->atoms_epoch; h->cache_build_step = h->step_index;
      h->cache_time = h->time;
    } else {
      if ((rc = check_validity())) return rc;
    }
    h->cache_age++;
  }
  C.pool = h->cache_pool[h->cache_cur].p; C.hot = h->cache_hot[h->cache_cur].p; C.count = h->cache_count.p;
  C.cap = h->cache_cap; C.overflow = h->split_flags.p + 2; C.level = h->cache_level;
  std::vector<long long> base(ns);
  long long tot = 0;
  for (int s2 = 0; s2 < ns; s2++) { base[s2] = tot; tot += h->h_pool_cap[s2]; }
  if (h->h_in_cap < (long long)np * 2 + 4096) h->h_in_cap = (long long)np * 2 + 4096;
  if (h->h_in_cap > 0xfffffff0LL) h->h_in_cap = 0xfffffff0LL;
  try { h->pool.ensure((size_t)tot + 64); h->pool_flag.ensure((size_t)tot + 64); h->inpool.ensure((size_t)h->h_in_cap + 64); } catch (std::string &e) { return fail(h, e); }
  CU(cudaMemcpyAsync(h->pool_base.p, base.data(), ns * sizeof(long long), cudaMemcpyHostToDevice, h->stream));
  CU(cudaMemcpyAsync(h->pool_cap.p, h->h_pool_cap.data(), ns * sizeof(long long), cudaMemcpyHostToDevice, h->stream));
  CU(cudaMemsetAsync(h->split_sc.p, 0, sizeof(SplitScalars), h->stream));
  SplitArgs S;
  S.pool = h->pool.p; S.pool_flag = h->pool_flag.p; S.pool_base = h->pool_base.p; S.pool_cap = h->pool_cap.p; S.sc = h->split_sc.p;
  S.pd = h->pd.p; S.big_list = h->big_list.p; S.slow_list = h->slow_list.p; S.inpool = h->inpool.p; S.in_cap = h->h_in_cap;
  if (tick(0)) return -2;
  if (C.enabled) {
    const int cw = h->tune_cull_wpb > 0 ? h->tune_cull_wpb : 1;
    const int ppw = h->tune_cull_lpp == 32 ? 1 : 2;
    const int grid = cdiv(np, cw * ppw);
    ShapeLiteTable T{};
    for (int s2 = 0; s2 < ns && s2 < SH_MAX_SHAPES; s2++) {
      const DevShape &v = h->shape_host_view[s2];
      T.s[s2].pf4 = v.pf4; T.s[s2].cube_ul = v.cube_ul; T.s[s2].px = v.px; T.s[s2].py = v.py; T.s[s2].pz = v.pz;
      T.s[s2].cube_n = v.cube_n; T.s[s2].rmax = v.rmax; T.s[s2].rmax2 = v.rmax2; T.s[s2].rmin2 = v.rmin2;
    }
#define LAUNCH_CULL(W, L) pair_cull_cached_kernel<W, L><<<grid, W * 32, 0, h->stream>>>(P, S, C, use_bounds, T)
    if (ppw == 1) { if (cw == 1) LAUNCH_CULL(1, 32); else if (cw == 2) LAUNCH_CULL(2, 32); else if (cw == 8) LAUNCH_CULL(8, 32); else LAUNCH_CULL(4, 32); }
    else { if (cw == 1) LAUNCH_CULL(1, 16); else if (cw == 2) LAUNCH_CULL(2, 16); else if (cw == 8) LAUNCH_CULL(8, 16); else LAUNCH_CULL(4, 16); }
#undef LAUNCH_CULL
    h->kernel_launches++;
  }
  {
    constexpr int WW = 2;
    const int grid = std::max(1, std::min(cdiv(np, WW), h->sm_count * 16));
    pair_cull_window_kernel<WW><<<grid, WW * 32, 0, h->stream>>>(P, S, C, use_bounds);
    h->kernel_launches++;
  }
  tock();
  int maxT = 1;
  for (int s2 = 0; s2 < ns; s2++) maxT = std::max(maxT, h->shape_host_view[s2].nterms4 + 4);
  if (tick(1)) return -2;
  if (h->eval_pts == 2) rc = h->eval_occ == 3 ? launch_eval<WPB, 2, 3>(h, S, maxT) : launch_eval<WPB, 2, 4>(h, S, maxT);
  else rc = launch_eval<WPB, 4, 2>(h, S, maxT);
  if (rc) return rc;
  tock();
  h->eval_launches++;
  if (tick(2)) return -2;
  if (h->reduce_occ == 4) pair_reduce_kernel<4><<<cdiv(np, 128), 128, 0, h->stream>>>(P, S);
  else if (h->reduce_occ == 8) pair_reduce_kernel<8><<<cdiv(np, 128), 128, 0, h->stream>>>(P, S);
  else pair_reduce_kernel<6><<<cdiv(np, 128), 128, 0, h->stream>>>(P, S);
  tock();
  h->kernel_launches++;
  {
    PairArgs Pb = P;
    Pb.pair_list = h->big_list.p; Pb.npairs = np; Pb.npairs_dev = &h->split_sc.p->nbig; Pb.work_counter = &h->split_sc.p->deep_counter;
    if (tick(3)) return -2;
    rc = launch_fused(h, Pb, h->sm_count);
    if (rc) return rc;
    tock();
    h->kernel_launches++;
  }
  CU(cudaMemcpyAsync(h->h_split_sc, h->split_sc.p, sizeof(SplitScalars), cudaMemcpyDeviceToHost, h->stream));
  CU(cudaMemcpyAsync(h->h_cache_invalid, h->scalars.p + 3, 2 * sizeof(int), cudaMemcpyDeviceToHost, h->stream));
  CU(cudaEventRecord(h->ev_sc, h->stream));
  h->sc_pending = true; h->sc_nshape = ns;
  return 0;
}

int compute_forces_device(sh_ctx *h) {
  const int n = (int)(h->n - h->nghost);
  const bool newton_dd = h->dd.on && h->dd.newton && h->dd.borders_ok && (h->dd.peer.enabled || h->nghost > 0 || h->dd.nsend > 0);
  if (n == 0 && !newton_dd) { h->forces_valid = true; return 0; }
  AtomView A = view(h);
  const int nb = std::max(1, cdiv(n, 256));
  if (h->npairs > 0) {
    PairArgs P;
    P.shapes = h->d_shapes.p; P.c = h->c.p; P.Rs = h->Rs.p; P.x = h->x.p; P.shape = h->shape.p; P.stride = h->stride;
    P.pair_i = h->pair_i.p; P.pair_j = h->pair_j.p; P.pair_eij = h->pair_eij.p; P.pair_eji = h->pair_eji.p; P.pair_img = h->pair_img.p;
    P.npairs = h->npairs; P.slot = h->slot.p; P.slot_stride = h->slot_stride; P.pres = h->pres.p; P.pres_stride = h->pres_stride;
    P.pk = h->d_pk.p; P.pm = h->d_pm.p;
    P.dissip = h->dissip ? 1 : 0; P.v = h->v.p; P.L = h->L.p; P.q = h->q.p; P.pgn = h->d_pgn.p; P.pgt = h->d_pgt.p; P.pmu = h->d_pmu.p;
    if (h->dissip && h->nghost > 0 && !h->dd.on) return fail(h, "dissipative contact terms need ghost velocities: use the in-library decomposition (sh_dd_init)");
    for (int d = 0; d < 3; d++) { P.boxlen[d] = h->hi[d] - h->lo[d]; P.periodic[d] = h->periodic[d]; }
    P.work_counter = h->scalars.p + 2; P.counters = h->counters.p;
    int maxT = 1, maxq = 32;
    for (auto &s : h->shapes) { maxT = std::max(maxT, s.nterms); maxq = std::max(maxq, s.nq); }
    P.max_terms = maxT; P.max_nq = maxq; P.nlocal = n; P.pair_list = nullptr; P.npairs_dev = nullptr;
    CU(cudaMemsetAsync(h->scalars.p + 2, 0, sizeof(int), h->stream));
    const int nt = h->tune_threads ? h->tune_threads : 128;
    if (h->ev_used + 2 > h->ev.size() || h->ev2_used + 16 > h->ev2.size()) { if (drain_events(h)) return -2; }
    CU(cudaEventRecord(h->ev[h->ev_used], h->stream));
    int rc;
    if (h->tune_variant & 1) {
      if (nt == 256) rc = launch_pair<256>(h, P, h->tune_ctas_per_sm, pair_smem_bytes(maxT, maxq, 8));
      else if (nt == 64) rc = launch_pair<64>(h, P, h->tune_ctas_per_sm, pair_smem_bytes(maxT, maxq, 2));
      else rc = launch_pair<128>(h, P, h->tune_ctas_per_sm, pair_smem_bytes(maxT, maxq, 4));
    } else if ((h->tune_variant & 4) || (!(h->tune_variant & 16) && h->npairs < 16384)) {
      rc = launch_fused(h, P);
    } else {
      rc = run_split_pipeline(h, P);
    }
    if (rc) return rc;
    CU(cudaEventRecord(h->ev[h->ev_used + 1], h->stream));
    h->ev_used += 2;
    h->pair_launches++; h->kernel_launches++;
  }
  if (h->walls.n > 0 && n > 0) {
    wall_kernel<<<cdiv((int64_t)n * 32, 256), 256, 0, h->stream>>>(A, h->d_shapes.p, h->walls, h->ewall.p);
    h->kernel_launches++;
  }
  const int nrows = h->list_valid && h->nrows > n ? h->nrows : n;
  if (nrows > 0) {
    AtomView G2 = view_all(h);
    G2.n = nrows;
    gather_kernel<<<cdiv(nrows, 256), 256, 0, h->stream>>>(G2, h->nbr_off.p, h->slot.p, h->slot_stride, h->walls.n > 0 ? n : 0);
    h->kernel_launches++;
  }
  if (newton_dd) { int rc = dd_reverse(h); if (rc) return rc; }
  CU(cudaGetLastError());
  h->forces_valid = true;
  h->carry = false;
  return 0;
}

int prepare(sh_ctx *h) {
  if (h->n > 0 && h->shapes.empty()) return fail(h, "no shapes defined");
  int rc;
  if ((rc = upload_shapes(h))) return rc;
  if ((rc = upload_coeffs(h))) return rc;
  return 0;
}

int sync_tags_host(sh_ctx *h) {
  if (h->tags_host_valid) return 0;
  h->tag.resize(h->n);
  if (h->n > 0) {
    CU(cudaStreamSynchronize(h->stream));
    CU(cudaMemcpy(h->tag.data(), h->d_tag.p, (size_t)h->n * sizeof(long long), cudaMemcpyDeviceToHost));
  }
  h->tags_host_valid = true;
  return 0;
}

double neighbor_trigger(const sh_ctx *h) {
  double t = 0.5 * h->skin;
  if (h->dd.on && h->dd.le_rate != 0.0) t = std::max(0.0, 0.5 * (h->skin - std::fabs(h->dd.le_rate * h->dd.glen[1] * (h->time - h->dd.le_time_build))));
  return t;
}

int reduce_flag(sh_ctx *h, int *d_flag) {
  if (h->dd.on && h->dd.nranks > 1) NC(h->dd.nccl->AllReduce(d_flag, d_flag, 1, ncclInt, ncclMax, h->dd.comm, h->stream));
  return 0;
}

int setup_forces(sh_ctx *h) {
  int rc;
  if ((rc = prepare(h))) return rc;
  const bool dd = h->dd.on;
  bool fresh_borders = false;
  if (dd) {
    if (!h->dd.geometry_ok) { if ((rc = dd_setup_geometry(h))) return rc; }
    if (!h->dd.borders_ok) { if ((rc = dd_borders(h))) return rc; fresh_borders = true; }
    else if (h->list_valid) { if ((rc = dd_forward(h))) return rc; }
  }
  if (h->n > 0 || dd) {
    const double trig = neighbor_trigger(h);
    if (h->n > 0) {
      pose_kernel<<<cdiv(h->n, 256), 256, 0, h->stream>>>(view_all(h), h->d_shapes.p, h->list_valid ? trig * trig : -1.0, h->scalars.p + 1, 0, (int)h->n);
      h->kernel_launches++;
    }
    bool rebuild = !h->list_valid;
    if (!rebuild) {
      if ((rc = reduce_flag(h, h->scalars.p + 1))) return rc;
      CU(cudaMemcpyAsync(h->h_pinned + 4, h->scalars.p + 1, sizeof(int), cudaMemcpyDeviceToHost, h->stream));
      CU(cudaStreamSynchronize(h->stream));
      rebuild = h->h_pinned[4] != 0;
    }
    if (rebuild && dd && !fresh_borders) {
      if ((rc = dd_rebuild(h))) return rc;
      if (h->n > 0) {
        pose_kernel<<<cdiv(h->n, 256), 256, 0, h->stream>>>(view_all(h), h->d_shapes.p, -1.0, h->scalars.p + 1, 0, (int)h->n);
        h->kernel_launches++;
      }
    }
    if (rebuild) { if ((rc = build_neighbors(h))) return rc; }
  }
  h->lag_pending = false;
  return compute_forces_device(h);
}

}

extern "C" {

int sh_version(void) { return 100; }

int sh_create(sh_ctx **out, int device_id) {
  if (!out) return -1;
  *out = nullptr;
  int ndev = 0;
  if (cudaGetDeviceCount(&ndev) != cudaSuccess || ndev == 0) return -3;
  if (device_id < 0 || device_id >= ndev) return -4;
  sh_ctx *h = new sh_ctx();
  h->device = device_id;
  if (cudaSetDevice(device_id) != cudaSuccess) { delete h; return -5; }
  cudaDeviceProp prop;
  cudaGetDeviceProperties(&prop, device_id);
  h->sm_count = prop.multiProcessorCount;
  if (cudaStreamCreateWithFlags(&h->stream, cudaStreamNonBlocking) != cudaSuccess) { delete h; return -6; }
  h->pk.assign(SH_MAX_SHAPES * SH_MAX_SHAPES, 1.0);
  h->pm.assign(SH_MAX_SHAPES * SH_MAX_SHAPES, 1.0);
  h->pgn.assign(SH_MAX_SHAPES * SH_MAX_SHAPES, 0.0); h->pgt.assign(SH_MAX_SHAPES * SH_MAX_SHAPES, 0.0); h->pmu.assign(SH_MAX_SHAPES * SH_MAX_SHAPES, 0.0);
  try {
    h->scalars.ensure(16); h->bbox.ensure(8); h->counters.ensure(16); h->drift.ensure(128);
  } catch (std::string &) { delete h; return -7; }
  cudaMemset(h->scalars.p, 0, 16 * sizeof(int));
  cudaMemset(h->counters.p, 0, 16 * sizeof(unsigned long long));
  cudaMallocHost(&h->h_pinned, 64);
  cudaMallocHost(&h->h_lagflag, 16 * sizeof(int));
  std::memset(h->h_lagflag, 0, 16 * sizeof(int));
  cudaMallocHost(&h->dd.h_int, 256 * sizeof(int));
  for (auto &e : h->ev_lag) cudaEventCreateWithFlags(&e, cudaEventDisableTiming);
  cudaEventCreate(&h->run_e0); cudaEventCreate(&h->run_e1);
  h->ev.resize(2048); h->ev2.resize(4096); h->ev2_kind.resize(2048);
  for (auto &e : h->ev) cudaEventCreate(&e);
  for (auto &e : h->ev2) cudaEventCreate(&e);
  *out = h;
  return 0;
}

int sh_destroy(sh_ctx *h) {
  if (!h) return 0;
  cudaSetDevice(h->device);
  cudaStreamSynchronize(h->stream);
  for (auto &d : h->shape_dev) { d.Ap.release(); d.ab.release(); d.node.release(); d.row_x.release(); d.cube.release(); d.pf4.release(); for (auto &w : d.cubew) w.release(); }
  h->d_shapes.release(); h->d_pk.release(); h->d_pm.release(); h->d_pgn.release(); h->d_pgt.release(); h->d_pmu.release(); h->stress_part.release();
  DevBuf<double> *db[] = {&h->x, &h->v, &h->q, &h->L, &h->f, &h->tq, &h->c, &h->Rs, &h->c0, &h->wallf, &h->ewall, &h->ke, &h->bbox, &h->slot, &h->pres};
  for (auto *b : db) b->release();
  DevBuf<int> *ib[] = {&h->shape, &h->cell_of, &h->cell_count, &h->cell_start, &h->cell_fill, &h->cell_atoms, &h->tile_sum, &h->cnt_full,
                       &h->cnt_half, &h->nbr_off, &h->half_off, &h->nbr_j, &h->pair_i, &h->pair_j, &h->pair_eij, &h->pair_eji, &h->pair_img, &h->scalars};
  for (auto *b : ib) b->release();
  h->counters.release();
  h->as_vir.release(); h->as_kin.release(); h->as_en.release(); h->as_send.release(); h->as_recv.release(); h->as_cnt.release(); h->as_epair.release();
  for (auto &e : h->ev) cudaEventDestroy(e);
  for (auto &e : h->ev2) cudaEventDestroy(e);
  h->pool.release(); h->pool_flag.release(); h->pool_base.release(); h->pool_cap.release(); h->split_sc.release(); h->eval_plan.release(); h->slow_list.release();
  h->pd.release(); h->big_list.release(); h->split_flags.release(); h->inpool.release();
  for (int k = 0; k < 2; k++) { h->cache_hot[k].release(); h->cache_pool[k].release(); }
  h->old_c.release(); h->old_cc0.release(); h->old_cq0.release(); h->old_tag.release(); h->ghost_hash.release(); h->amap.release();
  h->old_half_off.release(); h->old_pair_j.release(); h->fresh_list.release(); h->cache_count.release(); h->cc0.release(); h->cq0.release(); h->drift.release();
  if (h->h_pool_count) { cudaFreeHost(h->h_pool_count); cudaFreeHost(h->h_split_sc); cudaFreeHost(h->h_cache_invalid); cudaEventDestroy(h->ev_sc); }
  if (h->h_pinned) cudaFreeHost(h->h_pinned);
  if (h->h_lagflag) cudaFreeHost(h->h_lagflag);
  if (h->dd.h_int) cudaFreeHost(h->dd.h_int);
  for (auto &e : h->ev_lag) if (e) cudaEventDestroy(e);
  for (auto &e : h->ev_step) cudaEventDestroy(e);
  dd_peer_release(h);
  if (h->dd.peer.d_err) cudaFree(h->dd.peer.d_err);
  h->dd.peer.d_off.release();
  if (h->dd.comm && h->dd.nccl) h->dd.nccl->CommDestroy(h->dd.comm);
  {
    DdCtx &D = h->dd;
    DevBuf<int> *ib2[] = {&D.flag, &D.pos, &D.order, &D.d_int, &D.send_idx, &D.send_slot, &D.shape2};
    for (auto *b : ib2) b->release();
    DevBuf<double> *db2[] = {&D.sendbuf, &D.recvbuf, &D.x2, &D.v2, &D.q2, &D.L2, &h->gf};
    for (auto *b : db2) b->release();
    D.tag2.release(); h->d_tag.release();
  }
  h->stage.release();
  cudaEventDestroy(h->run_e0); cudaEventDestroy(h->run_e1);
  cudaStreamDestroy(h->stream);
  delete h;
  return 0;
}

const char *sh_last_error(const sh_ctx *h) { return h ? h->err.c_str() : "null handle"; }

int sh_set_box(sh_ctx *h, const double lo[3], const double hi[3], const int periodic[3]) {
  for (int d = 0; d < 3; d++) if (!(hi[d] > lo[d])) return fail(h, "box: hi <= lo");
  for (int d = 0; d < 3; d++) { h->lo[d] = lo[d]; h->hi[d] = hi[d]; h->periodic[d] = periodic[d] != 0; }
  for (int d = 0; d < 3; d++) { h->dd.glo[d] = lo[d]; h->dd.ghi[d] = hi[d]; h->dd.gper[d] = periodic[d] != 0; }
  h->dd.geometry_ok = false; h->dd.borders_ok = false;
  h->box_set = true; h->forces_valid = false; h->list_valid = false;
  return 0;
}

int sh_set_quadrature(sh_ctx *h, int n_theta, int n_phi) {
  if (!h->shapes.empty()) return fail(h, "set_quadrature must precede add_shape");
  if (n_theta < 2 || n_phi < 4) return fail(h, "quadrature too small");
  if ((long)n_theta * n_phi > 65535) return fail(h, "quadrature has more than 65535 nodes");
  h->n_theta = n_theta; h->n_phi = n_phi;
  return 0;
}

int sh_add_shape(sh_ctx *h, int lmax, const double *a_lm, const double *b_lm, double density, int *shape_id_out) try {
  if ((int)h->shapes.size() >= SH_MAX_SHAPES) return fail(h, "too many shapes");
  ShapeTables t;
  std::string e = build_shape_tables(lmax, a_lm, b_lm, density, h->n_theta, h->n_phi, t, h->cube_n);
  if (!e.empty()) return fail(h, e);
  h->shapes.push_back(std::move(t));
  h->shapes_dirty = true; h->forces_valid = false; h->list_valid = false;
  if (shape_id_out) *shape_id_out = (int)h->shapes.size() - 1;
  return 0;
} catch (...) { return -99; }

int sh_get_shape_props(const sh_ctx *h, int shape, double *volume, double com[3], double inertia[3],
                       double quat_principal[4], double *rmax, double *rmin) {
  if (shape < 0 || shape >= (int)h->shapes.size()) return -1;
  const ShapeTables &s = h->shapes[shape];
  if (volume) *volume = s.volume;
  if (com) for (int d = 0; d < 3; d++) com[d] = s.com[d];
  if (inertia) for (int d = 0; d < 3; d++) inertia[d] = s.inertia[d];
  if (quat_principal) for (int d = 0; d < 4; d++) quat_principal[d] = s.quat_principal[d];
  if (rmax) *rmax = s.rmax;
  if (rmin) *rmin = s.rmin;
  return 0;
}

int sh_get_nodes(const sh_ctx *h, int shape, double *p, double *nds) {
  if (shape < 0 || shape >= (int)h->shapes.size()) return -1;
  const ShapeTables &s = h->shapes[shape];
  for (int k = 0; k < s.nq; k++)
    for (int d = 0; d < 3; d++) { if (p) p[3 * k + d] = s.node_p[d][k]; if (nds) nds[3 * k + d] = s.node_n[d][k]; }
  return 0;
}

int sh_set_atoms(sh_ctx *h, int64_t n_in, const int64_t *tag_in, const int *shape_in, const double *x_in, const double *v_in,
                 const double *quat_in, const double *angmom_in) try {
  if (n_in < 0 || n_in > (int64_t)1 << 30) return fail(h, "bad atom count");
  if (n_in > 0 && (!shape_in || !x_in)) return fail(h, "shape and x are required");
  const int ns = (int)h->shapes.size();
  for (int64_t i = 0; i < n_in; i++) if (shape_in[i] < 0 || shape_in[i] >= ns) return fail(h, "atom shape id out of range");
  if (quat_in) for (int64_t i = 0; i < n_in; i++) {
    const double *q = quat_in + 4 * i;
    if (!(q[0] * q[0] + q[1] * q[1] + q[2] * q[2] + q[3] * q[3] > 0)) return fail(h, "zero quaternion");
  }
  CU(cudaSetDevice(h->device));
  std::vector<int64_t> keep;
  std::vector<double> xw, vw;
  const bool dd = h->dd.on;
  if (dd) {
    int rc;
    if ((rc = dd_setup_geometry(h))) return rc;
    dd_refresh_shifts(h);
    const DdGeom &G = h->dd.G;
    xw.assign(x_in, x_in + 3 * n_in);
    if (v_in) vw.assign(v_in, v_in + 3 * n_in); else vw.assign(3 * n_in, 0.0);
    for (int64_t i = 0; i < n_in; i++) {
      double *x = &xw[3 * i];
      if (G.gper[1]) {
        const double ny = std::floor((x[1] - G.glo[1]) / G.L[1]);
        if (ny != 0.0) { x[1] -= G.L[1] * ny; x[0] -= ny * G.le_offset; vw[3 * i] -= ny * G.le_vshear; }
      }
      if (G.gper[0]) x[0] -= G.L[0] * std::floor((x[0] - G.glo[0]) / G.L[0]);
      if (G.gper[2]) x[2] -= G.L[2] * std::floor((x[2] - G.glo[2]) / G.L[2]);
      int gi[3];
      for (int d = 0; d < 3; d++) { const int c = (int)std::floor((x[d] - G.glo[d]) / G.sub[d]); gi[d] = std::min(std::max(c, 0), G.pgrid[d] - 1); }
      if ((gi[0] * G.pgrid[1] + gi[1]) * G.pgrid[2] + gi[2] == h->dd.rank) keep.push_back(i);
    }
  }
  const int64_t n = dd ? (int64_t)keep.size() : n_in;
  const double *x = dd ? xw.data() : x_in, *v = dd ? vw.data() : v_in;
  auto src_index = [&](int64_t i) -> int64_t { return dd ? keep[i] : i; };
  const int st = (int)((n + (dd ? std::max<int64_t>(n / 4, 1024) : 0) + 31) / 32 * 32) + 32;
  try {
    h->x.ensure(3 * (size_t)st); h->v.ensure(3 * (size_t)st); h->q.ensure(4 * (size_t)st); h->L.ensure(3 * (size_t)st);
    h->shape.ensure(st); h->d_tag.ensure(st);
  } catch (std::string &e) { return fail(h, e); }
  { int rc = dd_ensure_derived(h, st); if (rc) return rc; }
  h->n = n; h->stride = st;
  std::vector<double> buf((size_t)4 * st, 0.0);
  auto up = [&](DevBuf<double> &dst, const double *src, int ncomp, bool is_quat) -> cudaError_t {
    std::fill(buf.begin(), buf.end(), 0.0);
    for (int64_t i = 0; i < n; i++) {
      const int64_t k = src_index(i);
      if (src) {
        double nn = 1.0;
        if (is_quat) nn = std::sqrt(src[4 * k] * src[4 * k] + src[4 * k + 1] * src[4 * k + 1] + src[4 * k + 2] * src[4 * k + 2] + src[4 * k + 3] * src[4 * k + 3]);
        for (int d = 0; d < ncomp; d++) buf[(size_t)d * st + i] = is_quat ? src[ncomp * k + d] / nn : src[ncomp * k + d];
      } else if (is_quat) buf[i] = 1.0;
    }
    return cudaMemcpy(dst.p, buf.data(), (size_t)ncomp * st * sizeof(double), cudaMemcpyHostToDevice);
  };
  CU(up(h->x, x, 3, false)); CU(up(h->v, v, 3, false)); CU(up(h->q, quat_in, 4, true)); CU(up(h->L, angmom_in, 3, false));
  CU(cudaMemset(h->f.p, 0, 3 * (size_t)st * 8)); CU(cudaMemset(h->tq.p, 0, 3 * (size_t)st * 8));
  CU(cudaMemset(h->wallf.p, 0, 6 * (size_t)st * 8)); CU(cudaMemset(h->ewall.p, 0, (size_t)st * 8));
  CU(cudaMemset(h->c0.p, 0, 3 * (size_t)st * 8));
  std::vector<int> sh(st, 0);
  for (int64_t i = 0; i < n; i++) sh[i] = shape_in[src_index(i)];
  CU(cudaMemcpy(h->shape.p, sh.data(), (size_t)st * sizeof(int), cudaMemcpyHostToDevice));
  h->tag.resize(n);
  for (int64_t i = 0; i < n; i++) h->tag[i] = tag_in ? tag_in[src_index(i)] : src_index(i) + 1;
  if (n > 0) CU(cudaMemcpy(h->d_tag.p, h->tag.data(), (size_t)n * sizeof(long long), cudaMemcpyHostToDevice));
  h->tags_host_valid = true;
  h->forces_valid = false; h->list_valid = false; h->npairs = 0; h->nentries = 0; h->nghost = 0;
  h->atoms_epoch++; h->cache_state = CACHE_INVALID;
  h->dd.borders_ok = false;
  return 0;
} catch (...) { return -99; }

int sh_pair_coeff(sh_ctx *h, int si, int sj, double k, double exponent) {
  if (si < 0 || sj < 0 || si >= SH_MAX_SHAPES || sj >= SH_MAX_SHAPES) return fail(h, "pair_coeff: shape out of range");
  if (!(k >= 0) || !(exponent >= 1.0)) return fail(h, "pair_coeff: need k >= 0, exponent >= 1");
  h->pk[si * SH_MAX_SHAPES + sj] = h->pk[sj * SH_MAX_SHAPES + si] = k;
  h->pm[si * SH_MAX_SHAPES + sj] = h->pm[sj * SH_MAX_SHAPES + si] = exponent;
  h->coeff_dirty = true; h->forces_valid = false;
  return 0;
}

int sh_pair_dissipation(sh_ctx *h, int si, int sj, double gamma_n, double gamma_t, double mu) {
  if (si < 0 || sj < 0 || si >= SH_MAX_SHAPES || sj >= SH_MAX_SHAPES) return fail(h, "pair_dissipation: shape out of range");
  if (!(gamma_n >= 0) || !(gamma_t >= 0) || !(mu >= 0)) return fail(h, "pair_dissipation: need gamma_n, gamma_t, mu >= 0");
  h->pgn[si * SH_MAX_SHAPES + sj] = h->pgn[sj * SH_MAX_SHAPES + si] = gamma_n;
  h->pgt[si * SH_MAX_SHAPES + sj] = h->pgt[sj * SH_MAX_SHAPES + si] = gamma_t;
  h->pmu[si * SH_MAX_SHAPES + sj] = h->pmu[sj * SH_MAX_SHAPES + si] = mu;
  h->dissip = false;
  for (size_t k = 0; k < h->pgn.size(); k++) if (h->pgn[k] > 0 || (h->pgt[k] > 0 && h->pmu[k] > 0)) h->dissip = true;
  const int gv = h->dissip ? 1 : 0;
  if (gv != h->dd.ghost_vel) { h->dd.ghost_vel = gv; h->dd.borders_ok = false; h->list_valid = false; }
  h->coeff_dirty = true; h->forces_valid = false;
  return 0;
}

int sh_add_wall(sh_ctx *h, const double point[3], const double normal[3], double k, double exponent) {
  if (h->walls.n >= 16) return fail(h, "too many walls");
  const double nn = std::sqrt(normal[0] * normal[0] + normal[1] * normal[1] + normal[2] * normal[2]);
  if (!(nn > 0)) return fail(h, "wall normal is zero");
  if (!(k >= 0) || !(exponent >= 1.0)) return fail(h, "wall: need k >= 0, exponent >= 1");
  const int w = h->walls.n++;
  for (int d = 0; d < 3; d++) { h->walls.c[w][d] = point[d]; h->walls.nrm[w][d] = normal[d] / nn; }
  h->walls.k[w] = k; h->walls.m[w] = exponent;
  h->forces_valid = false;
  return 0;
}

int sh_set_gravity(sh_ctx *h, const double g[3]) { for (int d = 0; d < 3; d++) h->g[d] = g[d]; return 0; }

int sh_set_neighbor(sh_ctx *h, double skin, int every, int check) {
  if (skin < 0) return fail(h, "skin < 0");
  if (every < 1) return fail(h, "every < 1");
  h->skin = skin; h->neigh_every = every; h->neigh_check = check != 0;
  h->list_valid = false; h->forces_valid = false;
  return 0;
}

int sh_set_damping(sh_ctx *h, double gamma_lin, double gamma_rot) {
  if (gamma_lin < 0 || gamma_rot < 0) return fail(h, "damping < 0");
  h->gamma_lin = gamma_lin; h->gamma_rot = gamma_rot;
  return 0;
}

int sh_set_timestep(sh_ctx *h, double dt) { if (!(dt > 0)) return fail(h, "dt <= 0"); h->dt = dt; return 0; }

int sh_set_pair_tuning(sh_ctx *h, int threads_per_cta, int ctas_per_sm, int variant) {
  if (threads_per_cta != 0 && threads_per_cta != 64 && threads_per_cta != 128 && threads_per_cta != 256 && threads_per_cta != 384 && threads_per_cta != 512)
    return fail(h, "threads_per_cta must be 0, 64, 128, 256 or 512");
  h->tune_threads = threads_per_cta; h->tune_ctas_per_sm = ctas_per_sm; h->tune_variant = variant;
  h->cache_state = CACHE_INVALID;
  return 0;
}

int sh_compute_forces(sh_ctx *h) try {
  CU(cudaSetDevice(h->device));
  int rc = setup_forces(h);
  if (rc) return rc;
  CU(cudaStreamSynchronize(h->stream));
  CU(cudaGetLastError());
  return 0;
} catch (...) { return -99; }

namespace {
int launch_integrate_initial(sh_ctx *h, int check_violation) {
  const int n = (int)(h->n - h->nghost);
  const double trig = neighbor_trigger(h), trig2 = trig * trig;
  const double damp_v = 1.0 - 0.5 * h->dt * h->gamma_lin, damp_L = 1.0 - 0.5 * h->dt * h->gamma_rot;
  if (n > 0) {
    integrate_initial_kernel<<<cdiv(n, 256), 256, 0, h->stream>>>(view(h), h->d_shapes.p, h->dt, h->g[0], h->g[1], h->g[2], trig2, h->scalars.p, damp_v, damp_L, check_violation);
    h->kernel_launches++;
  }
  h->time += h->dt;
  h->steps_since_build++;
  return 0;
}

int step_finish(sh_ctx *h, int rebuild) {
  int rc;
  const int n = (int)(h->n - h->nghost);
  const double damp_v = 1.0 - 0.5 * h->dt * h->gamma_lin, damp_L = 1.0 - 0.5 * h->dt * h->gamma_rot;
  if (!h->list_valid) {
    if ((rc = prepare(h))) return rc;
    if (h->n > 0) {
      pose_kernel<<<cdiv(h->n, 256), 256, 0, h->stream>>>(view_all(h), h->d_shapes.p, -1.0, h->scalars.p + 1, 0, (int)h->n);
      h->kernel_launches++;
    }
  } else if (h->nghost > 0) {
    pose_kernel<<<cdiv(h->nghost, 256), 256, 0, h->stream>>>(view_all(h), h->d_shapes.p, -1.0, h->scalars.p + 1, n, (int)h->nghost);
    h->kernel_launches++;
  }
  if (rebuild || !h->list_valid) { if ((rc = build_neighbors(h))) return rc; }
  if ((rc = compute_forces_device(h))) return rc;
  if (n > 0) {
    integrate_final_kernel<<<cdiv(n, 256), 256, 0, h->stream>>>(view(h), h->d_shapes.p, h->dt, h->g[0], h->g[1], h->g[2], damp_v, damp_L);
    h->kernel_launches++;
  }
  return 0;
}

int cache_snapshot(sh_ctx *h) {
  const int n = (int)h->n, nown = (int)(h->n - h->nghost), st = h->stride, ng = (int)h->nghost;
  int hs = 64;
  while (hs < 2 * ng + 2) hs <<= 1;
  try {
    h->old_c.ensure(3 * (size_t)st); h->old_cc0.ensure(3 * (size_t)st); h->old_cq0.ensure(4 * (size_t)st); h->old_tag.ensure((size_t)n + 2);
    h->old_half_off.ensure((size_t)nown + 2); h->old_pair_j.ensure((size_t)h->npairs + 1); h->ghost_hash.ensure(hs);
  } catch (std::string &e) { return fail(h, e); }
  CU(cudaMemcpyAsync(h->old_c.p, h->c.p, 3 * (size_t)st * sizeof(double), cudaMemcpyDeviceToDevice, h->stream));
  CU(cudaMemcpyAsync(h->old_cc0.p, h->cc0.p, 3 * (size_t)st * sizeof(double), cudaMemcpyDeviceToDevice, h->stream));
  CU(cudaMemcpyAsync(h->old_cq0.p, h->cq0.p, 4 * (size_t)st * sizeof(double), cudaMemcpyDeviceToDevice, h->stream));
  CU(cudaMemcpyAsync(h->old_tag.p, h->d_tag.p, (size_t)n * sizeof(long long), cudaMemcpyDeviceToDevice, h->stream));
  CU(cudaMemcpyAsync(h->old_half_off.p, h->half_off.p, ((size_t)nown + 1) * sizeof(int), cudaMemcpyDeviceToDevice, h->stream));
  CU(cudaMemcpyAsync(h->old_pair_j.p, h->pair_j.p, (size_t)h->npairs * sizeof(int), cudaMemcpyDeviceToDevice, h->stream));
  CU(cudaMemsetAsync(h->ghost_hash.p, 0xff, (size_t)hs * sizeof(int), h->stream));
  if (ng > 0) { dd_ghost_hash_kernel<<<cdiv(ng, 256), 256, 0, h->stream>>>(h->old_tag.p, nown, ng, h->ghost_hash.p, hs); h->kernel_launches++; }
  h->old_n = n; h->old_nown = nown; h->old_stride = st; h->ghost_hash_size = hs;
  h->carry = true;
  return 0;
}

int step_once(sh_ctx *h) {
  int rc;
  const bool dd = h->dd.on;
  const bool due = h->steps_since_build + 1 >= h->neigh_every;
  const bool lag = h->lag_mode && h->neigh_check;
  int rebuild = 0;
  bool decided = false;
  if (!due) decided = true;
  else if (!h->neigh_check) { rebuild = 1; decided = true; }
  h->step_index++;
  h->cache_sync_ranks = lag && dd && h->dd.nranks > 1;
  if (lag && h->lag_pending) {
    CU(cudaEventSynchronize(h->ev_lag[h->lag_slot]));
    const int soft = h->h_lagflag[4 + 2 * h->lag_slot], pred = h->h_lagflag[5 + 2 * h->lag_slot];
    h->lag_pending = false;
    if (!decided && h->lag_pred_valid) { rebuild = pred; decided = true; }
    if (h->cache_sync_ranks && soft && h->cache_state == CACHE_VALID && h->step_index > h->cache_build_step + 2) { h->cache_state = CACHE_INVALID; h->cache_exhausted = true; }
  }
  if ((rc = launch_integrate_initial(h, decided && !rebuild))) return rc;
  if (!decided) {
    if ((rc = reduce_flag(h, h->scalars.p + 1))) return rc;
    CU(cudaMemcpyAsync(h->h_pinned + 4, h->scalars.p + 1, sizeof(int), cudaMemcpyDeviceToHost, h->stream));
    CU(cudaStreamSynchronize(h->stream));
    rebuild = h->h_pinned[4] != 0;
  }
  if (lag) {
    if (h->cache_sync_ranks || !rebuild) {
      if (dd && h->dd.nranks > 1) NC(h->dd.nccl->AllReduce(h->scalars.p + 4, h->scalars.p + 10, 2, ncclInt, ncclMax, h->dd.comm, h->stream));
      else CU(cudaMemcpyAsync(h->scalars.p + 10, h->scalars.p + 4, 2 * sizeof(int), cudaMemcpyDeviceToDevice, h->stream));
      h->lag_slot ^= 1;
      CU(cudaMemcpyAsync(h->h_lagflag + 4 + 2 * h->lag_slot, h->scalars.p + 10, 2 * sizeof(int), cudaMemcpyDeviceToHost, h->stream));
      CU(cudaEventRecord(h->ev_lag[h->lag_slot], h->stream));
      h->lag_pending = true;
      h->lag_pred_valid = !rebuild;
    }
    CU(cudaMemsetAsync(h->scalars.p + 5, 0, sizeof(int), h->stream));
  }
  if (dd && rebuild) {
    h->carry = false;
    const bool split = !(h->tune_variant & (1 | 2 | 4 | 8 | 32)) && ((h->tune_variant & 16) || h->npairs >= 16384);
    if (split && h->cache_state == CACHE_VALID && h->list_valid && h->npairs > 0 && h->atoms_epoch == h->cache_epoch &&
        h->cache_level + 1 < SH_CACHE_LEVELS) { if ((rc = cache_snapshot(h))) return rc; }
    const bool carry = h->carry;
    if ((rc = dd_rebuild(h))) return rc;
    h->carry = carry;
  } else if (dd) { if ((rc = dd_forward(h))) return rc; }
  return step_finish(h, rebuild);
}
}

int sh_step_begin(sh_ctx *h, int *rebuild_wanted) try {
  CU(cudaSetDevice(h->device));
  int rc;
  if (!h->forces_valid || !h->list_valid) { if ((rc = setup_forces(h))) return rc; }
  if (rebuild_wanted) *rebuild_wanted = 0;
  if (h->n == 0) return 0;
  const bool due = h->steps_since_build + 1 >= h->neigh_every;
  if ((rc = launch_integrate_initial(h, 0))) return rc;
  h->lag_pending = false;
  bool rebuild = false;
  if (due) {
    if (h->neigh_check) {
      CU(cudaMemcpyAsync(h->h_pinned + 4, h->scalars.p + 1, sizeof(int), cudaMemcpyDeviceToHost, h->stream));
      CU(cudaStreamSynchronize(h->stream));
      rebuild = h->h_pinned[4] != 0;
    } else rebuild = true;
  }
  if (rebuild_wanted) *rebuild_wanted = rebuild ? 1 : 0;
  return 0;
} catch (...) { return -99; }

int sh_step_end(sh_ctx *h, int rebuild) try {
  CU(cudaSetDevice(h->device));
  if (h->n == 0) return 0;
  return step_finish(h, rebuild);
} catch (...) { return -99; }

int sh_run(sh_ctx *h, int64_t nsteps) try {
  CU(cudaSetDevice(h->device));
  int rc;
  if (!h->forces_valid || !h->list_valid) { if ((rc = setup_forces(h))) return rc; }
  if (h->n == 0 && !h->dd.on) return 0;
  CU(cudaEventRecord(h->run_e0, h->stream));
  const bool trace = h->step_trace && nsteps <= 4096;
  if (trace) {
    while ((int64_t)h->ev_step.size() < nsteps + 1) { cudaEvent_t e; CU(cudaEventCreate(&e)); h->ev_step.push_back(e); }
    CU(cudaEventRecord(h->ev_step[0], h->stream));
    h->step_flags.assign(nsteps, 0);
  }
  for (int64_t step = 0; step < nsteps; step++) {
    const int64_t nb0 = h->neighbor_builds, cb0 = h->cache_builds, cr0 = h->cache_remaps;
    const long long al0 = devbuf_stats().allocs;
    if ((rc = step_once(h))) return rc;
    if (trace) {
      CU(cudaEventRecord(h->ev_step[step + 1], h->stream));
      h->step_flags[step] = (h->neighbor_builds > nb0 ? 1 : 0) | (h->cache_builds > cb0 ? 2 : 0) | (h->cache_remaps > cr0 ? 4 : 0) |
                            (devbuf_stats().allocs > al0 ? 8 : 0);
    }
  }
  CU(cudaMemcpyAsync(h->h_lagflag + 2, h->scalars.p + 6, sizeof(int), cudaMemcpyDeviceToHost, h->stream));
  if (h->dd.peer.d_err) CU(cudaMemcpyAsync(h->h_lagflag + 3, h->dd.peer.d_err, sizeof(int), cudaMemcpyDeviceToHost, h->stream));
  CU(cudaEventRecord(h->run_e1, h->stream));
  CU(cudaStreamSynchronize(h->stream));
  CU(cudaGetLastError());
  { float ms = 0; cudaEventElapsedTime(&ms, h->run_e0, h->run_e1); h->sec_run_last = ms * 1e-3; h->sec_run_total += h->sec_run_last; }
  if (trace) {
    h->step_ms.assign(nsteps, 0.f);
    for (int64_t k = 0; k < nsteps; k++) cudaEventElapsedTime(&h->step_ms[k], h->ev_step[k], h->ev_step[k + 1]);
    h->step_flags_last = h->step_flags;
  } else h->step_ms.clear();
  if (h->dd.peer.d_err && h->h_lagflag[3] != 0) return fail(h, "ghost exchange over peer memory timed out waiting for a neighbour rank");
  if (h->h_lagflag[2] != 0) {
    CU(cudaMemset(h->scalars.p + 6, 0, sizeof(int)));
    return fail(h, "neighbor skin violated: an atom moved more than half the skin on a step the lagged neighbor decision did not "
                   "rebuild on (increase the skin, or sh_set_tuning \"sync_rebuild\" 1)");
  }
  return 0;
} catch (...) { return -99; }

int sh_set_ghost_count(sh_ctx *h, int64_t nghost) {
  if (nghost < 0 || nghost > h->n) return fail(h, "ghost count out of range");
  h->nghost = nghost; h->forces_valid = false; h->list_valid = false;
  return 0;
}
int sh_pack_atoms(sh_ctx *h, int64_t m, const int *d_idx, const double *d_shift, double *d_out) {
  CU(cudaSetDevice(h->device));
  if (m > 0) {
    pack_atoms_kernel<<<cdiv(m, 256), 256, 0, h->stream>>>(view_all(h), (int)m, d_idx, d_shift, d_out);
    h->kernel_launches++;
  }
  CU(cudaStreamSynchronize(h->stream));
  return 0;
}
int sh_unpack_ghosts(sh_ctx *h, int64_t first, int64_t m, const double *d_in) {
  CU(cudaSetDevice(h->device));
  if (first < 0 || first + m > h->n) return fail(h, "unpack range out of bounds");
  if (m > 0) {
    unpack_atoms_kernel<<<cdiv(m, 256), 256, 0, h->stream>>>(view_all(h), (int)first, (int)m, d_in);
    h->kernel_launches++;
  }
  CU(cudaStreamSynchronize(h->stream));
  return 0;
}
int sh_mark_begin(sh_ctx *h) {
  CU(cudaSetDevice(h->device));
  CU(cudaEventRecord(h->run_e0, h->stream));
  return 0;
}
int sh_mark_end(sh_ctx *h, double *seconds) {
  CU(cudaSetDevice(h->device));
  CU(cudaEventRecord(h->run_e1, h->stream));
  CU(cudaEventSynchronize(h->run_e1));
  float ms = 0;
  CU(cudaEventElapsedTime(&ms, h->run_e0, h->run_e1));
  if (seconds) *seconds = ms * 1e-3;
  return 0;
}
int sh_synchronize(sh_ctx *h) {
  CU(cudaSetDevice(h->device));
  CU(cudaStreamSynchronize(h->stream));
  CU(cudaGetLastError());
  return 0;
}

int sh_get_run_time(const sh_ctx *h, double *seconds_last_run, double *seconds_total) {
  if (seconds_last_run) *seconds_last_run = h->sec_run_last;
  if (seconds_total) *seconds_total = h->sec_run_total;
  return 0;
}

int sh_put_state(sh_ctx *h, int64_t n, const double *x, const double *v, const double *quat, const double *angmom) try {
  if (n != h->n) return fail(h, "put_state: n mismatch");
  CU(cudaSetDevice(h->device));
  if (n == 0) return 0;
  const int st = h->stride, nb = cdiv(n, 256);
  try { h->stage.ensure((size_t)4 * n); } catch (std::string &e) { return fail(h, e); }
  struct Item { const double *src; double *dst; int nc; int norm; } items[4] = {
      {x, h->x.p, 3, 0}, {v, h->v.p, 3, 0}, {quat, h->q.p, 4, 1}, {angmom, h->L.p, 3, 0}};
  for (auto &it : items) {
    if (!it.src) continue;
    CU(cudaMemcpyAsync(h->stage.p, it.src, (size_t)it.nc * n * sizeof(double), cudaMemcpyHostToDevice, h->stream));
    aos_to_soa_kernel<<<nb, 256, 0, h->stream>>>(h->stage.p, it.dst, (int)n, it.nc, st, it.norm);
    h->kernel_launches++;
  }
  CU(cudaStreamSynchronize(h->stream));
  h->forces_valid = false;
  return 0;
} catch (...) { return -99; }

int sh_get_forces(const sh_ctx *hc, int64_t n, double *f, double *torque) try {
  sh_ctx *h = const_cast<sh_ctx *>(hc);
  if (n < 0 || n > h->n) return fail(h, "get_forces: n out of range");
  CU(cudaSetDevice(h->device));
  if (n == 0) return 0;
  const int st = h->stride, nb = cdiv(n, 256);
  try { h->stage.ensure((size_t)6 * n); } catch (std::string &e) { return fail(h, e); }
  soa_to_aos_kernel<<<nb, 256, 0, h->stream>>>(h->f.p, h->stage.p, (int)n, 3, st);
  soa_to_aos_kernel<<<nb, 256, 0, h->stream>>>(h->tq.p, h->stage.p + 3 * n, (int)n, 3, st);
  h->kernel_launches += 2;
  if (f) CU(cudaMemcpyAsync(f, h->stage.p, (size_t)3 * n * sizeof(double), cudaMemcpyDeviceToHost, h->stream));
  if (torque) CU(cudaMemcpyAsync(torque, h->stage.p + 3 * n, (size_t)3 * n * sizeof(double), cudaMemcpyDeviceToHost, h->stream));
  CU(cudaStreamSynchronize(h->stream));
  return 0;
} catch (...) { return -99; }

namespace {
struct SnapHeader { char magic[8]; int32_t version, nshapes; int64_t n, step; double lo[3], hi[3]; int32_t periodic[3], pad; };
}
int sh_write_snapshot(const sh_ctx *hc, const char *path, int64_t step) try {
  sh_ctx *h = const_cast<sh_ctx *>(hc);
  const int64_t n = h->n - h->nghost;
  { int rc = sync_tags_host(h); if (rc) return rc; }
  std::vector<double> x(3 * n), v(3 * n), q(4 * n), L(3 * n);
  if (n > 0) { int rc = sh_get_atoms(h, n, x.data(), v.data(), q.data(), L.data(), nullptr, nullptr); if (rc) return rc; }
  std::vector<int> shp(h->stride > 0 ? h->stride : 1);
  if (n > 0) CU(cudaMemcpy(shp.data(), h->shape.p, n * sizeof(int), cudaMemcpyDeviceToHost));
  FILE *f = fopen(path, "wb");
  if (!f) return fail(h, std::string("cannot open snapshot file ") + path);
  SnapHeader hd{};
  std::memcpy(hd.magic, "SHGPUSNP", 8);
  hd.version = 1; hd.nshapes = (int)h->shapes.size(); hd.n = n; hd.step = step;
  for (int d = 0; d < 3; d++) { hd.lo[d] = h->dd.glo[d]; hd.hi[d] = h->dd.ghi[d]; hd.periodic[d] = h->dd.gper[d]; }
  bool ok = fwrite(&hd, sizeof hd, 1, f) == 1;
  ok = ok && (n == 0 || (fwrite(h->tag.data(), sizeof(int64_t), n, f) == (size_t)n && fwrite(shp.data(), sizeof(int), n, f) == (size_t)n &&
                         fwrite(x.data(), 8, 3 * n, f) == (size_t)(3 * n) && fwrite(v.data(), 8, 3 * n, f) == (size_t)(3 * n) &&
                         fwrite(q.data(), 8, 4 * n, f) == (size_t)(4 * n) && fwrite(L.data(), 8, 3 * n, f) == (size_t)(3 * n)));
  fclose(f);
  if (!ok) return fail(h, "short write to snapshot file");
  return 0;
} catch (...) { return -99; }
int sh_read_snapshot(sh_ctx *h, const char *path, int64_t *step_out) try {
  FILE *f = fopen(path, "rb");
  if (!f) return fail(h, std::string("cannot open snapshot file ") + path);
  SnapHeader hd{};
  if (fread(&hd, sizeof hd, 1, f) != 1 || std::memcmp(hd.magic, "SHGPUSNP", 8) != 0 || hd.version != 1) { fclose(f); return fail(h, "not a shgpu snapshot (bad header)"); }
  if (hd.nshapes != (int)h->shapes.size()) { fclose(f); return fail(h, "snapshot was written with a different number of shapes"); }
  const int64_t n = hd.n;
  if (n < 0 || n > ((int64_t)1 << 30)) { fclose(f); return fail(h, "bad atom count in snapshot"); }
  {
    const long pos = ftell(f);
    fseek(f, 0, SEEK_END);
    const long end = ftell(f);
    fseek(f, pos, SEEK_SET);
    if (end - pos < (long)(n * (int64_t)(sizeof(int64_t) + sizeof(int) + 13 * sizeof(double)))) { fclose(f); return fail(h, "truncated snapshot file"); }
  }
  std::vector<int64_t> tag(n); std::vector<int> shp(n);
  std::vector<double> x(3 * n), v(3 * n), q(4 * n), L(3 * n);
  bool ok = n == 0 || (fread(tag.data(), sizeof(int64_t), n, f) == (size_t)n && fread(shp.data(), sizeof(int), n, f) == (size_t)n &&
                       fread(x.data(), 8, 3 * n, f) == (size_t)(3 * n) && fread(v.data(), 8, 3 * n, f) == (size_t)(3 * n) &&
                       fread(q.data(), 8, 4 * n, f) == (size_t)(4 * n) && fread(L.data(), 8, 3 * n, f) == (size_t)(3 * n));
  fclose(f);
  if (!ok) return fail(h, "truncated snapshot file");
  int rc = sh_set_box(h, hd.lo, hd.hi, hd.periodic);
  if (rc) return rc;
  rc = sh_set_atoms(h, n, tag.data(), shp.data(), x.data(), v.data(), q.data(), L.data());
  if (rc) return rc;
  if (step_out) *step_out = hd.step;
  return 0;
} catch (...) { return -99; }

int sh_get_natoms(const sh_ctx *h, int64_t *n) { if (n) *n = h->n; return 0; }

int sh_get_atoms(const sh_ctx *hc, int64_t n, double *x, double *v, double *quat, double *angmom, double *f, double *torque) try {
  sh_ctx *h = const_cast<sh_ctx *>(hc);
  if (n < 0 || n > h->n) return fail(h, "get_atoms: n out of range");
  CU(cudaSetDevice(h->device));
  CU(cudaStreamSynchronize(h->stream));
  const int st = h->stride;
  std::vector<double> buf((size_t)4 * st);
  auto down = [&](const DevBuf<double> &src, double *dst, int ncomp) -> cudaError_t {
    if (!dst) return cudaSuccess;
    cudaError_t e = cudaMemcpy(buf.data(), src.p, (size_t)ncomp * st * sizeof(double), cudaMemcpyDeviceToHost);
    if (e != cudaSuccess) return e;
    for (int64_t i = 0; i < n; i++) for (int d = 0; d < ncomp; d++) dst[ncomp * i + d] = buf[(size_t)d * st + i];
    return cudaSuccess;
  };
  CU(down(h->x, x, 3)); CU(down(h->v, v, 3)); CU(down(h->q, quat, 4)); CU(down(h->L, angmom, 3));
  CU(down(h->f, f, 3)); CU(down(h->tq, torque, 3));
  return 0;
} catch (...) { return -99; }

int sh_get_pairs(const sh_ctx *hc, int64_t cap, int64_t *npairs, int64_t *tag_i, int64_t *tag_j, double *V, double *F,
                 double *tau_i, double *tau_j, double *centroid) try {
  sh_ctx *h = const_cast<sh_ctx *>(hc);
  CU(cudaSetDevice(h->device));
  CU(cudaStreamSynchronize(h->stream));
  const int np = h->forces_valid ? h->npairs : 0;
  if (npairs) *npairs = np;
  { int rc = sync_tags_host(h); if (rc) return rc; }
  const int m = (int)std::min<int64_t>(np, cap);
  if (m <= 0) return 0;
  std::vector<int> pi(m), pj(m);
  CU(cudaMemcpy(pi.data(), h->pair_i.p, m * sizeof(int), cudaMemcpyDeviceToHost));
  CU(cudaMemcpy(pj.data(), h->pair_j.p, m * sizeof(int), cudaMemcpyDeviceToHost));
  std::vector<double> buf((size_t)14 * m);
  for (int r = 0; r < 14; r++)
    CU(cudaMemcpy(buf.data() + (size_t)r * m, h->pres.p + (size_t)r * h->pres_stride, m * sizeof(double), cudaMemcpyDeviceToHost));
  for (int k = 0; k < m; k++) {
    if (tag_i) tag_i[k] = h->tag[pi[k]];
    if (tag_j) tag_j[k] = h->tag[pj[k]];
    if (V) V[k] = buf[k];
    for (int r = 0; r < 3; r++) {
      if (F) F[3 * k + r] = buf[(size_t)(2 + r) * m + k];
      if (tau_i) tau_i[3 * k + r] = buf[(size_t)(5 + r) * m + k];
      if (tau_j) tau_j[3 * k + r] = buf[(size_t)(8 + r) * m + k];
      if (centroid) centroid[3 * k + r] = buf[(size_t)(11 + r) * m + k];
    }
  }
  return 0;
} catch (...) { return -99; }

int sh_get_energy(const sh_ctx *hc, double *ke_trans, double *ke_rot, double *e_contact) try {
  sh_ctx *h = const_cast<sh_ctx *>(hc);
  CU(cudaSetDevice(h->device));
  const int n = (int)(h->n - h->nghost);
  double kt = 0, kr = 0, ec = 0;
  if (n > 0) {
    int rc = prepare(h);
    if (rc) return rc;
    energy_kernel<<<cdiv(n, 256), 256, 0, h->stream>>>(view(h), h->d_shapes.p, h->ke.p);
    h->kernel_launches++;
    CU(cudaStreamSynchronize(h->stream));
    std::vector<double> buf(2 * (size_t)n);
    CU(cudaMemcpy(buf.data(), h->ke.p, 2 * (size_t)n * sizeof(double), cudaMemcpyDeviceToHost));
    for (int i = 0; i < n; i++) { kt += buf[i]; kr += buf[n + i]; }
    if (h->forces_valid) {
      if (h->npairs > 0) {
        std::vector<double> e(h->npairs);
        CU(cudaMemcpy(e.data(), h->pres.p + (size_t)h->pres_stride, h->npairs * sizeof(double), cudaMemcpyDeviceToHost));
        for (double vv : e) ec += vv;
      }
      if (h->walls.n > 0) {
        std::vector<double> e(n);
        CU(cudaMemcpy(e.data(), h->ewall.p, n * sizeof(double), cudaMemcpyDeviceToHost));
        for (double vv : e) ec += vv;
      }
    }
  }
  if (ke_trans) *ke_trans = kt;
  if (ke_rot) *ke_rot = kr;
  if (e_contact) *e_contact = ec;
  return 0;
} catch (...) { return -99; }

int sh_get_stress(const sh_ctx *hc, double virial[9], double kinetic[9]) try {
  sh_ctx *h = const_cast<sh_ctx *>(hc);
  CU(cudaSetDevice(h->device));
  const int n = (int)(h->n - h->nghost), np = h->forces_valid ? h->npairs : 0;
  const int nb_atoms = std::max(1, cdiv(n, 256)), nb_pairs = std::max(1, cdiv(np, 256));
  try { h->stress_part.ensure((size_t)9 * (nb_atoms + nb_pairs)); } catch (std::string &e) { return fail(h, e); }
  double K[9] = {0}, W[9] = {0};
  if (n > 0) {
    int rc = prepare(h);
    if (rc) return rc;
    stress_kinetic_kernel<<<nb_atoms, 256, 0, h->stream>>>(view(h), h->d_shapes.p, h->stress_part.p);
    h->kernel_launches++;
  }
  if (np > 0) {
    stress_virial_kernel<<<nb_pairs, 256, 0, h->stream>>>(view_all(h), np, h->nrows > n ? (int)h->n : n, h->pair_i.p, h->pair_j.p, h->pair_img.p, h->pres.p, h->pres_stride,
                                                          h->hi[0] - h->lo[0], h->hi[1] - h->lo[1], h->hi[2] - h->lo[2], h->stress_part.p + (size_t)9 * nb_atoms);
    h->kernel_launches++;
  }
  CU(cudaStreamSynchronize(h->stream));
  std::vector<double> part((size_t)9 * (nb_atoms + nb_pairs), 0.0);
  CU(cudaMemcpy(part.data(), h->stress_part.p, part.size() * sizeof(double), cudaMemcpyDeviceToHost));
  if (n > 0) for (int b = 0; b < nb_atoms; b++) for (int k = 0; k < 9; k++) K[k] += part[(size_t)9 * b + k];
  if (np > 0) for (int b = 0; b < nb_pairs; b++) for (int k = 0; k < 9; k++) W[k] += part[(size_t)9 * (nb_atoms + b) + k];
  for (int k = 0; k < 9; k++) { if (virial) virial[k] = W[k]; if (kinetic) kinetic[k] = K[k]; }
  return 0;
} catch (...) { return -99; }

int sh_get_atom_stress(const sh_ctx *hc, int64_t n, int mode, double *virial, double *kinetic, double *energy, int *contacts) try {
  sh_ctx *h = const_cast<sh_ctx *>(hc);
  const int nown = (int)(h->n - h->nghost);
  if (n < 0 || n > nown) return fail(h, "get_atom_stress: n out of range");
  if (mode != 0 && mode != 1) return fail(h, "get_atom_stress: mode must be 0 (centre-to-centre) or 1 (contact centroid)");
  CU(cudaSetDevice(h->device));
  int rc = prepare(h);
  if (rc) return rc;
  DdCtx &D = h->dd;
  const bool newton_dd = D.on && D.newton && D.borders_ok && (h->nghost > 0 || D.nsend > 0);
  const bool pairs = h->forces_valid && h->list_valid && h->npairs > 0;
  const int nall = newton_dd ? (int)h->n : nown;
  const int nrows = pairs ? std::min(h->nrows, nall) : 0;
  try {
    h->as_vir.ensure((size_t)9 * std::max(nown, 1)); h->as_kin.ensure((size_t)9 * std::max(nown, 1));
    h->as_en.ensure(std::max(nown, 1)); h->as_cnt.ensure(std::max(nown, 1));
    if (pairs) h->as_epair.ensure((size_t)h->nentries + 1);
    if (newton_dd) { h->as_send.ensure((size_t)11 * std::max<int64_t>(h->nghost, 1)); h->as_recv.ensure((size_t)11 * std::max(D.nsend, 1)); }
  } catch (std::string &e) { return fail(h, e); }
  if (pairs) {
    CU(cudaMemsetAsync(h->as_epair.p, 0xff, (size_t)h->nentries * sizeof(int), h->stream));
    atom_stress_entry_pair_kernel<<<cdiv(h->npairs, 256), 256, 0, h->stream>>>(h->npairs, h->pair_eij.p, h->pair_eji.p, h->as_epair.p);
    h->kernel_launches++;
  }
  if (nall > 0) {
    AtomStressArgs S;
    S.A = view(h); S.shapes = h->d_shapes.p; S.nall = nall; S.nrows = nrows; S.mode = mode;
    S.nbr_off = h->nbr_off.p; S.epair = h->as_epair.p; S.pair_i = h->pair_i.p; S.pair_j = h->pair_j.p; S.pair_img = h->pair_img.p;
    S.pres = h->pres.p; S.pres_stride = h->pres_stride;
    for (int d = 0; d < 3; d++) S.L[d] = h->hi[d] - h->lo[d];
    S.ewall = h->forces_valid && h->walls.n > 0 ? h->ewall.p : nullptr;
    S.vir = h->as_vir.p; S.kin = h->as_kin.p; S.en = h->as_en.p; S.cnt = h->as_cnt.p; S.ghost_rec = h->as_send.p;
    atom_stress_row_kernel<<<cdiv(nall, 128), 128, 0, h->stream>>>(S);
    h->kernel_launches++;
  }
  if (newton_dd) {
    if ((rc = dd_sendrecv(h, D.nbr_rank, h->as_send.p, D.recv_cnt, h->as_recv.p, D.send_cnt, 11))) return rc;
    if (D.nsend > 0 && nown > 0) {
      atom_stress_add_returned_kernel<<<cdiv(nown, 256), 256, 0, h->stream>>>(nown, D.rev_off.p, D.rev_k.p, h->as_recv.p, h->as_vir.p,
                                                                            h->as_en.p, h->as_cnt.p);
      h->kernel_launches++;
    }
  }
  CU(cudaGetLastError());
  CU(cudaStreamSynchronize(h->stream));
  if (n > 0) {
    if (virial) CU(cudaMemcpy(virial, h->as_vir.p, (size_t)9 * n * sizeof(double), cudaMemcpyDeviceToHost));
    if (kinetic) CU(cudaMemcpy(kinetic, h->as_kin.p, (size_t)9 * n * sizeof(double), cudaMemcpyDeviceToHost));
    if (energy) CU(cudaMemcpy(energy, h->as_en.p, (size_t)n * sizeof(double), cudaMemcpyDeviceToHost));
    if (contacts) CU(cudaMemcpy(contacts, h->as_cnt.p, (size_t)n * sizeof(int), cudaMemcpyDeviceToHost));
  }
  return 0;
} catch (...) { return -99; }

int sh_get_ghost_pair_evals(const sh_ctx *hc, int64_t *ghost_pair_evals) {
  sh_ctx *h = const_cast<sh_ctx *>(hc);
  CU(cudaSetDevice(h->device));
  CU(cudaStreamSynchronize(h->stream));
  unsigned long long c = 0;
  CU(cudaMemcpy(&c, h->counters.p + 4, sizeof c, cudaMemcpyDeviceToHost));
  if (h->dd.on && h->dd.newton) c = 0;
  if (ghost_pair_evals) *ghost_pair_evals = (int64_t)c;
  return 0;
}

int sh_get_counters(const sh_ctx *hc, int64_t *pair_evals, int64_t *nodes_transformed, int64_t *nodes_evaluated,
                    int64_t *nodes_inside, int64_t *neighbor_builds, int64_t *kernel_launches) {
  sh_ctx *h = const_cast<sh_ctx *>(hc);
  CU(cudaSetDevice(h->device));
  CU(cudaStreamSynchronize(h->stream));
  unsigned long long c[4];
  CU(cudaMemcpy(c, h->counters.p, sizeof c, cudaMemcpyDeviceToHost));
  if (pair_evals) *pair_evals = (int64_t)c[0];
  if (nodes_transformed) *nodes_transformed = (int64_t)c[1];
  if (nodes_evaluated) *nodes_evaluated = (int64_t)c[2];
  if (nodes_inside) *nodes_inside = (int64_t)c[3];
  if (neighbor_builds) *neighbor_builds = h->neighbor_builds;
  if (kernel_launches) *kernel_launches = h->kernel_launches;
  return 0;
}

int sh_get_timers(const sh_ctx *hc, double *seconds_pair, int64_t *pair_launches, double *seconds_neigh, double *seconds_other) {
  sh_ctx *h = const_cast<sh_ctx *>(hc);
  CU(cudaSetDevice(h->device));
  int rc = drain_events(h);
  if (rc) return rc;
  if (seconds_pair) *seconds_pair = h->sec_pair;
  if (pair_launches) *pair_launches = h->pair_launches;
  if (seconds_neigh) *seconds_neigh = h->sec_neigh;
  if (seconds_other) *seconds_other = h->sec_comm;
  return 0;
}

int sh_get_counter_raw(const sh_ctx *hc, int index, int64_t *value) {
  sh_ctx *h = const_cast<sh_ctx *>(hc);
  if (index < 0 || index >= 8) return fail(h, "counter index out of range");
  CU(cudaSetDevice(h->device));
  CU(cudaStreamSynchronize(h->stream));
  unsigned long long c = 0;
  CU(cudaMemcpy(&c, h->counters.p + index, sizeof c, cudaMemcpyDeviceToHost));
  if (value) *value = (int64_t)c;
  return 0;
}

int sh_get_split_times(const sh_ctx *hc, double *seconds_cull, double *seconds_eval, double *seconds_reduce, double *seconds_deep) {
  sh_ctx *h = const_cast<sh_ctx *>(hc);
  CU(cudaSetDevice(h->device));
  int rc = drain_events(h);
  if (rc) return rc;
  if (seconds_cull) *seconds_cull = h->sec_cull;
  if (seconds_eval) *seconds_eval = h->sec_eval;
  if (seconds_reduce) *seconds_reduce = h->sec_reduce;
  if (seconds_deep) *seconds_deep = h->sec_deep;
  return 0;
}

int sh_get_split_stats(const sh_ctx *hc, double *seconds_eval, int64_t *eval_launches, int64_t *deep_pairs, int64_t *pool_redos,
                       int64_t *cache_builds) {
  sh_ctx *h = const_cast<sh_ctx *>(hc);
  CU(cudaSetDevice(h->device));
  int rc = drain_events(h);
  if (rc) return rc;
  if ((rc = absorb_split_feedback(h))) return rc;
  if (seconds_eval) *seconds_eval = h->sec_eval;
  if (eval_launches) *eval_launches = h->eval_launches;
  if (deep_pairs) *deep_pairs = h->big_pairs;
  if (pool_redos) *pool_redos = h->pool_grows;
  if (cache_builds) *cache_builds = h->cache_builds;
  return 0;
}

int sh_reset_timers(sh_ctx *h) {
  CU(cudaSetDevice(h->device));
  int rc = drain_events(h);
  if (rc) return rc;
  h->sec_pair = h->sec_neigh = h->sec_comm = h->sec_other = 0; h->pair_launches = 0; h->sec_run_total = 0;
  h->sec_eval = h->sec_cull = h->sec_reduce = h->sec_deep = 0; h->eval_launches = 0; h->big_pairs = 0; h->slow_pairs = 0; h->pool_grows = 0; h->cache_builds = 0; h->cache_remaps = 0; h->sec_cache = 0;
  h->neighbor_builds = 0; h->kernel_launches = 0;
  CU(cudaMemset(h->counters.p, 0, 16 * sizeof(unsigned long long)));
  return 0;
}

int sh_get_cache_stats(const sh_ctx *hc, int64_t *cache_builds, double *seconds_cache, int *level, int64_t *slow_pairs,
                       int64_t *cache_remaps) {
  sh_ctx *h = const_cast<sh_ctx *>(hc);
  CU(cudaSetDevice(h->device));
  int rc = drain_events(h);
  if (rc) return rc;
  if ((rc = absorb_split_feedback(h))) return rc;
  if (cache_builds) *cache_builds = h->cache_builds;
  if (seconds_cache) *seconds_cache = h->sec_cache;
  if (level) *level = h->cache_level;
  if (slow_pairs) *slow_pairs = h->slow_pairs;
  if (cache_remaps) *cache_remaps = h->cache_remaps;
  return 0;
}

int sh_set_tuning(sh_ctx *h, const char *key, double value) try {
  if (!h || !key) return -1;
  const std::string k(key);
  const int v = (int)value;
  if (k == "cull_wpb") { if (v != 0 && v != 1 && v != 2 && v != 4 && v != 8) return fail(h, "cull_wpb must be 0, 1, 2, 4 or 8"); h->tune_cull_wpb = v; }
  else if (k == "cull_lpp") { if (v != 0 && v != 16 && v != 32) return fail(h, "cull_lpp must be 0, 16 or 32"); h->tune_cull_lpp = v; }
  else if (k == "reduce_occ") { if (v != 0 && v != 4 && v != 6 && v != 8) return fail(h, "reduce_occ must be 0, 4, 6 or 8"); h->reduce_occ = v; }
  else if (k == "eval_pts") { if (v != 0 && v != 2 && v != 4) return fail(h, "eval_pts must be 0, 2 or 4"); h->eval_pts = v; }
  else if (k == "eval_occ") { if (v != 0 && v != 3 && v != 4) return fail(h, "eval_occ must be 0, 3 or 4"); h->eval_occ = v; }
  else if (k == "eval_mode") { if (v < 0 || v > 2) return fail(h, "eval_mode must be 0 (default), 1 (one block per CTA) or 2 (persistent chunks)"); h->eval_mode = v; }
  else if (k == "cache_level") { if (v < -1 || v >= SH_CACHE_LEVELS) return fail(h, "cache_level must be -1 (adaptive) .. 2"); if (v > 2) return fail(h, "cache_level must be -1 (adaptive) .. 2"); h->cache_level_pin = v; h->cache_state = CACHE_INVALID; }
  else if (k == "cube_n") {
    if (!h->shapes.empty()) return fail(h, "cube_n must be set before add_shape");
    if (v != 0 && (v < 8 || v > 144)) return fail(h, "cube_n must be 0 (default) or 8..144");
    h->cube_n = v;
  } else if (k == "peer_exchange") { h->dd.peer.want = v != 0; if (!h->dd.peer.want && h->dd.peer.enabled) return fail(h, "peer_exchange can only be switched off before the first run"); }
  else if (k == "newton") { h->dd.newton = v != 0; h->list_valid = false; h->forces_valid = false; }
  else if (k == "step_trace") { h->step_trace = v != 0; }
  else if (k == "dd_self_ghosts") { h->dd.self_ghosts = v != 0; h->dd.geometry_ok = false; h->dd.borders_ok = false; }
  else if (k == "sync_rebuild") { h->lag_mode = v == 0; h->lag_pending = false; }
  else return fail(h, "unknown tuning key: " + k);
  return 0;
} catch (...) { return -99; }

int sh_measure_fp64_peak(sh_ctx *h, double *flops_per_s, double *sm_clock_mhz_est) {
  CU(cudaSetDevice(h->device));
  const int threads = 256, blocks = h->sm_count * 8, iters = 4096;
  DevBuf<double> out;
  try { out.ensure((size_t)threads * blocks); } catch (std::string &e) { return fail(h, e); }
  cudaEvent_t e0, e1;
  CU(cudaEventCreate(&e0)); CU(cudaEventCreate(&e1));
  double best = 0;
  for (int rep = 0; rep < 5; rep++) {
    CU(cudaEventRecord(e0, h->stream));
    dfma_peak_kernel<<<blocks, threads, 0, h->stream>>>(out.p, iters, 1.0000001, 1e-9);
    CU(cudaEventRecord(e1, h->stream));
    CU(cudaEventSynchronize(e1));
    float ms = 0;
    cudaEventElapsedTime(&ms, e0, e1);
    const double fl = 2.0 * 64.0 * iters * (double)threads * blocks / (ms * 1e-3);
    if (rep > 0) best = std::max(best, fl);
  }
  h->kernel_launches += 5;
  cudaEventDestroy(e0); cudaEventDestroy(e1);
  out.release();
  if (flops_per_s) *flops_per_s = best;
  if (sm_clock_mhz_est) *sm_clock_mhz_est = best / (2.0 * 64.0 * h->sm_count) * 1e-6;
  CU(cudaGetLastError());
  return 0;
}

int sh_dd_unique_id(char *id, int cap) {
  if (!id || cap < (int)sizeof(ncclUniqueId)) return -1;
  NcclApi *api = nccl_api();
  if (!api) return -8;
  ncclUniqueId u;
  if (api->GetUniqueId(&u) != ncclSuccess) return -9;
  std::memcpy(id, &u, sizeof u);
  return 0;
}

int sh_dd_init(sh_ctx *h, int rank, int nranks, const char *id, const int *pgrid) try {
  if (!h) return -1;
  if (nranks < 1 || nranks > DD_MAX_RANKS || rank < 0 || rank >= nranks) return fail(h, "dd_init: bad rank / nranks (at most 64 ranks)");
  if (h->dd.on) return fail(h, "dd_init: already initialised");
  CU(cudaSetDevice(h->device));
  DdCtx &D = h->dd;
  D.rank = rank; D.nranks = nranks;
  if (nranks > 1) {
    if (!id) return fail(h, "dd_init: a unique id is required for more than one rank");
    D.nccl = nccl_api();
    if (!D.nccl) return fail(h, "dd_init: NCCL is not available (libnccl.so.2)");
    ncclUniqueId u;
    std::memcpy(&u, id, sizeof u);
    NC(D.nccl->CommInitRank(&D.comm, nranks, u, rank));
  }
  if (pgrid && pgrid[0] > 0 && pgrid[1] > 0 && pgrid[2] > 0) { for (int d = 0; d < 3; d++) D.pgrid[d] = pgrid[d]; D.pgrid_set = true; }
  D.on = true; D.geometry_ok = false; D.borders_ok = false;
  h->forces_valid = false; h->list_valid = false;
  if (h->n > 0) return fail(h, "dd_init must precede sh_set_atoms");
  return 0;
} catch (...) { return -99; }

int sh_dd_get_info(const sh_ctx *hc, int pgrid[3], int brick[3], int64_t *nlocal, int64_t *nghost, int64_t *migrated,
                   int64_t *border_builds) {
  sh_ctx *h = const_cast<sh_ctx *>(hc);
  if (!h) return -1;
  if (pgrid) for (int d = 0; d < 3; d++) pgrid[d] = h->dd.pgrid[d];
  if (brick) for (int d = 0; d < 3; d++) brick[d] = h->dd.g[d];
  if (nlocal) *nlocal = h->n - h->nghost;
  if (nghost) *nghost = h->nghost;
  if (migrated) *migrated = h->dd.migrated_out;
  if (border_builds) *border_builds = h->dd.border_builds;
  return 0;
}

int sh_get_step_trace(const sh_ctx *h, int64_t cap, int64_t *nsteps, double *ms, int *flags) {
  if (!h) return -1;
  const int64_t n = (int64_t)h->step_ms.size();
  if (nsteps) *nsteps = n;
  for (int64_t k = 0; k < std::min(n, cap); k++) { if (ms) ms[k] = h->step_ms[k]; if (flags) flags[k] = h->step_flags_last[k]; }
  return 0;
}

int sh_get_tags(const sh_ctx *hc, int64_t n, int64_t *tags) try {
  sh_ctx *h = const_cast<sh_ctx *>(hc);
  if (n < 0 || n > h->n) return fail(h, "get_tags: n out of range");
  CU(cudaSetDevice(h->device));
  int rc = sync_tags_host(h);
  if (rc) return rc;
  for (int64_t i = 0; i < n; i++) tags[i] = h->tag[i];
  return 0;
} catch (...) { return -99; }

int sh_set_shear(sh_ctx *h, double rate) {
  if (!h) return -1;
  if (h->n > 0) return fail(h, "set_shear must precede sh_set_atoms");
  if (!h->dd.on) { int rc = sh_dd_init(h, 0, 1, nullptr, nullptr); if (rc) return rc; }
  h->dd.le_rate = rate; h->dd.le_off_build = 0.0; h->dd.le_time_build = h->time;
  h->dd.geometry_ok = false; h->dd.borders_ok = false;
  return 0;
}

}
```

Baseline: 495.2 million.

## Restructure pair reduce: store node index per record, packed node data, skip zero writes

The eval kernel now writes the node index (or -1) per pool record instead of a byte flag, so the reduce kernel no longer builds bitmasks or rereads SurvRec entries to fetch k. Node positions and normals are packed into an interleaved double2 array per shape, so each node is fetched with three 16-byte loads rather than six strided loads. The reduce kernel processes two pairs per thread with compaction scaffolding, and tracks per-pair zero-output state to skip rewriting outputs that are already zero. This costs extra memory (int per record, out_zero buffer), adds invalidation logic, and removes the reduce_occ tuning knob.

Result: faster. 518.6 million (median of 6 runs) (+4.7%).

```diff
diff --git a/lammps-spherharm_b200/csrc/device_math.cuh b/lammps-spherharm_b200/csrc/device_math.cuh
--- a/lammps-spherharm_b200/csrc/device_math.cuh
+++ b/lammps-spherharm_b200/csrc/device_math.cuh
@@ -12,6 +12,7 @@
   const double2 *ab;
   const double *px, *py, *pz;
   const double *nx, *ny, *nz;
+  const double2 *pn;
   int n_theta, n_phi;
   int tab_off;
   int nterms4;
diff --git a/lammps-spherharm_b200/csrc/pair_split_kernels.cuh b/lammps-spherharm_b200/csrc/pair_split_kernels.cuh
--- a/lammps-spherharm_b200/csrc/pair_split_kernels.cuh
+++ b/lammps-spherharm_b200/csrc/pair_split_kernels.cuh
@@ -48,11 +48,12 @@
 
 struct SplitArgs {
   SurvRec *pool;
-  unsigned char *pool_flag;
+  int *pool_kin;
   const long long *pool_base;
   const long long *pool_cap;
   SplitScalars *sc;
   PdEntry *pd;
+  unsigned char *out_zero;
   int *big_list;
   int *slow_list;
   int *inpool;
@@ -501,7 +502,7 @@
         r.k = k; r.flag = fl;
         const long long idx = (dirc ? base1 : base0) + slot;
         S.pool[idx] = r;
-        S.pool_flag[idx] = 0;
+        S.pool_kin[idx] = -1;
       }
     }
     w0d0 += __popc(m0 & md0); w0d1 += __popc(m0 & ~md0);
@@ -648,8 +649,8 @@
       }
     } else {
       const long long base0 = S.pool_base[shp_j] + off0, base1 = S.pool_base[shp_i] + off1;
-      for (int r = lane; r < cnt0; r += 32) { S.pool[base0 + r] = s_rec[warp][0][r]; S.pool_flag[base0 + r] = s_rec[warp][0][r].flag == 2 ? 1 : 0; }
-      for (int r = lane; r < cnt1; r += 32) { S.pool[base1 + r] = s_rec[warp][1][r]; S.pool_flag[base1 + r] = s_rec[warp][1][r].flag == 2 ? 1 : 0; }
+      for (int r = lane; r < cnt0; r += 32) { const SurvRec q = s_rec[warp][0][r]; S.pool[base0 + r] = q; S.pool_kin[base0 + r] = q.flag == 2 ? q.k : -1; }
+      for (int r = lane; r < cnt1; r += 32) { const SurvRec q = s_rec[warp][1][r]; S.pool[base1 + r] = q; S.pool_kin[base1 + r] = q.flag == 2 ? q.k : -1; }
       if (lane == 0) store_pd(&S.pd[2 * p], base0, cnt0, nt0, nin0, s_in[warp][0]);
       if (lane == 1) store_pd(&S.pd[2 * p + 1], base1, cnt1, nt1, nin1, s_in[warp][1]);
     }
@@ -700,7 +701,7 @@
     const long long r0 = ((long long)(blk - plan->blk_start[s]) * WPB + warp) * RPW;
     if (r0 >= n) continue;
     SurvRec *rec = S.pool + S.pool_base[s];
-    unsigned char *flg = S.pool_flag + S.pool_base[s];
+    int *kin = S.pool_kin + S.pool_base[s];
     const int L = sh.lmax;
     int nev = 0;
     if (PTS == 2) {
@@ -714,18 +715,18 @@
         const double rhoB2 = fma(sB[2], sB[2], fma(sB[1], sB[1], sB[0] * sB[0]));
         double rhoA, rhoB, rA, rB;
         sh_radius_folded_x2(L, s_Ap, s_ab, sA, rhoA2, sB, rhoB2, rhoA, rhoB, rA, rB);
-        if (va && ra.flag == 0) { flg[ia] = rhoA < rA ? 1 : 0; nev++; }
-        if (vb && rb.flag == 0) { flg[ib] = rhoB < rB ? 1 : 0; nev++; }
+        if (va && ra.flag == 0) { kin[ia] = rhoA < rA ? ra.k : -1; nev++; }
+        if (vb && rb.flag == 0) { kin[ib] = rhoB < rB ? rb.k : -1; nev++; }
       } else if (va) {
         const SurvRec ra = rec[ia];
         const double rho2 = fma(ra.s2, ra.s2, fma(ra.s1, ra.s1, ra.s0 * ra.s0));
         double rho;
         const double r = sh_radius_folded(L, s_Ap, s_ab, ra.s0, ra.s1, ra.s2, rho2, rho);
-        if (ra.flag == 0) { flg[ia] = rho < r ? 1 : 0; nev++; }
+        if (ra.flag == 0) { kin[ia] = rho < r ? ra.k : -1; nev++; }
       }
     } else {
       double sv[PTS][3], rho2[PTS], rho[PTS], rr[PTS];
-      int fl[PTS];
+      int fl[PTS], kk[PTS];
       long long idx[PTS];
 #pragma unroll
       for (int q = 0; q < PTS; q++) {
@@ -734,12 +735,13 @@
         const SurvRec r = rec[v ? idx[q] : r0];
         sv[q][0] = r.s0; sv[q][1] = r.s1; sv[q][2] = r.s2;
         fl[q] = v ? r.flag : 3;
+        kk[q] = r.k;
         rho2[q] = fma(r.s2, r.s2, fma(r.s1, r.s1, r.s0 * r.s0));
       }
       sh_radius_folded_n<PTS>(L, s_Ap, s_ab, sv, rho2, rho, rr);
 #pragma unroll
       for (int q = 0; q < PTS; q++)
-        if (fl[q] == 0) { flg[idx[q]] = rho[q] < rr[q] ? 1 : 0; nev++; }
+        if (fl[q] == 0) { kin[idx[q]] = rho[q] < rr[q] ? kk[q] : -1; nev++; }
     }
     nev_total += nev;
   }
@@ -749,9 +751,9 @@
 
 struct NodeSums { double S0, S1, S2, Av, T0, T1, T2, G0, G1, G2; int n; };
 
-__device__ __forceinline__ void add_node(NodeSums &a, const double *__restrict__ nodes, int nq, int k, const double x0[3]) {
-  const double p0 = nodes[k], p1 = nodes[nq + k], p2 = nodes[2 * nq + k];
-  const double n0 = nodes[3 * nq + k], n1 = nodes[4 * nq + k], n2 = nodes[5 * nq + k];
+__device__ __forceinline__ void add_node(NodeSums &a, double2 q0, double2 q1, double2 q2, const double x0[3]) {
+  const double p0 = q0.x, p1 = q0.y, p2 = q1.x;
+  const double n0 = q1.y, n1 = q2.x, n2 = q2.y;
   const double dp0 = p0 - x0[0], dp1 = p1 - x0[1], dp2 = p2 - x0[2];
   const double dn = fma(dp2, n2, fma(dp1, n1, dp0 * n0));
   a.S0 += n0; a.S1 += n1; a.S2 += n2;
@@ -763,147 +765,178 @@
   a.n++;
 }
 
-template <int MINB>
-__global__ void __launch_bounds__(128, MINB) pair_reduce_kernel(PairArgs A, SplitArgs S) {
-  const int p = blockIdx.x * blockDim.x + threadIdx.x;
-  int c_pairs = 0, c_trans = 0, c_inside = 0, c_ghost = 0;
-  if (p < A.npairs) {
+__device__ __forceinline__ void store_pair_outputs(const PairArgs &A, int p, const double out[14]) {
+#pragma unroll
+  for (int r = 0; r < 14; r++) A.pres[(size_t)r * A.pres_stride + p] = out[r];
+  const int eij = A.pair_eij[p], eji = A.pair_eji[p];
+#pragma unroll
+  for (int r = 0; r < 3; r++) {
+    A.slot[(size_t)r * A.slot_stride + eij] = out[2 + r];
+    A.slot[(size_t)(3 + r) * A.slot_stride + eij] = out[5 + r];
+    if (eji >= 0) {
+      A.slot[(size_t)r * A.slot_stride + eji] = -out[2 + r];
+      A.slot[(size_t)(3 + r) * A.slot_stride + eji] = out[8 + r];
+    }
+  }
+}
+
+__device__ __forceinline__ void store_pair_outputs_once(const PairArgs &A, const SplitArgs &S, int p, bool zero, const double out[14]) {
+  const bool held = S.out_zero[p] != 0;
+  if (zero && held) return;
+  store_pair_outputs(A, p, out);
+  if (zero != held) S.out_zero[p] = zero ? 1 : 0;
+}
+
+__device__ __forceinline__ int reduce_contact_pair(const PairArgs &A, const SplitArgs &S, int p) {
+  constexpr int RB = 2;
+  {
     const int4 *ep = reinterpret_cast<const int4 *>(S.pd + 2 * (size_t)p);
     const int4 e0a = __ldg(ep), e0b = __ldg(ep + 1), e1a = __ldg(ep + 2), e1b = __ldg(ep + 3);
-    const int cnt0 = e0a.z, cnt1 = e1a.z;
-    if (cnt0 >= 0) {
-      const int i = A.pair_i[p], j = A.pair_j[p];
-      c_pairs = 1; c_trans = (e0a.w & 0xffff) + (e1a.w & 0xffff); c_ghost = j >= A.nlocal;
-      const int nin0 = e0b.y & 0xffff, nin1 = e1b.y & 0xffff;
-      const int xc0 = (e0a.w >> 16) & 0xffff, xc1 = (e1a.w >> 16) & 0xffff;
-      double out[14];
-#pragma unroll
-      for (int r = 0; r < 14; r++) out[r] = 0.0;
-      const long long off0 = (long long)(((unsigned long long)(unsigned)e0a.y << 32) | (unsigned)e0a.x);
-      const long long off1 = (long long)(((unsigned long long)(unsigned)e1a.y << 32) | (unsigned)e1a.x);
-      unsigned long long msk0 = 0, msk1 = 0;
-      bool any = nin0 > 0 || nin1 > 0 || xc0 > 0 || xc1 > 0;
-      {
-        const int m0 = min(cnt0, 64), m1 = min(cnt1, 64);
-        for (int r = 0; r < m0; r += 8) {
-#pragma unroll
-          for (int q = 0; q < 8; q++) if (r + q < m0 && S.pool_flag[off0 + r + q]) msk0 |= 1ull << (r + q);
+    const int i = A.pair_i[p], j = A.pair_j[p];
+    const int st = A.stride;
+    double d[3];
+    pair_separation(A, p, i, j, d);
+    const int shp_i = A.shape[i], shp_j = A.shape[j];
+    double out[14];
+#pragma unroll
+    for (int r = 0; r < 14; r++) out[r] = 0.0;
+    double Ss[2][3], Ts[2][3], Gs[2][3], Asum[2];
+    int ninside_pair = 0;
+#pragma unroll
+    for (int dir = 0; dir < 2; dir++) {
+      const int a = dir ? j : i;
+      const DevShape &sa = A.shapes[dir ? shp_j : shp_i];
+      const double sgn = dir ? -1.0 : 1.0;
+      const int4 ea = dir ? e1a : e0a, eb = dir ? e1b : e0b;
+      const long long off = (long long)(((unsigned long long)(unsigned)ea.y << 32) | (unsigned)ea.x);
+      const int cnt = ea.z, xc = (ea.w >> 16) & 0xffff, nin = eb.y & 0xffff;
+      const int nrx = cnt + xc, ntot = nrx + nin;
+      const int *__restrict__ kin = S.pool_kin + off;
+      const int *__restrict__ xin = S.inpool + (unsigned)eb.x;
+      const double2 *__restrict__ pn = sa.pn;
+      NodeSums acc;
+      acc.S0 = acc.S1 = acc.S2 = acc.Av = acc.T0 = acc.T1 = acc.T2 = acc.G0 = acc.G1 = acc.G2 = 0.0; acc.n = 0;
+      double Ra[9];
+#pragma unroll
+      for (int e = 0; e < 9; e++) Ra[e] = A.Rs[e * st + a];
+      double x0[3];
+#pragma unroll
+      for (int r = 0; r < 3; r++) {
+        double hx = Ra[0 + r] * (sgn * d[0]);
+        hx = fma(Ra[3 + r], sgn * d[1], hx);
+        hx = fma(Ra[6 + r], sgn * d[2], hx);
+        x0[r] = -0.5 * hx;
+      }
+      for (int b = 0; b < ntot; b += RB) {
+        int k[RB];
+#pragma unroll
+        for (int u = 0; u < RB; u++) {
+          const int g = b + u;
+          if (g < cnt) k[u] = kin[g];
+          else if (g < nrx) k[u] = xin[g - cnt];
+          else if (g < ntot) {
+            const int h = g - nrx + 3;
+            const unsigned w = (h >> 1) == 1 ? (unsigned)eb.y : (h >> 1) == 2 ? (unsigned)eb.z : (unsigned)eb.w;
+            k[u] = (int)((w >> (16 * (h & 1))) & 0xffffu);
+          } else k[u] = -1;
         }
-        for (int r = 0; r < m1; r += 8) {
-#pragma unroll
-          for (int q = 0; q < 8; q++) if (r + q < m1 && S.pool_flag[off1 + r + q]) msk1 |= 1ull << (r + q);
+        double2 q[RB][3];
+#pragma unroll
+        for (int u = 0; u < RB; u++) {
+          if (k[u] >= 0) { q[u][0] = pn[4 * k[u]]; q[u][1] = pn[4 * k[u] + 1]; q[u][2] = pn[4 * k[u] + 2]; }
+          else q[u][0] = q[u][1] = q[u][2] = make_double2(0.0, 0.0);
         }
-        any = any || msk0 || msk1 || cnt0 > 64 || cnt1 > 64;
-      }
-      if (any) {
-        const int st = A.stride;
-        double d[3];
-        pair_separation(A, p, i, j, d);
-        const int shp_i = A.shape[i], shp_j = A.shape[j];
-        double Ss[2][3], Ts[2][3], Gs[2][3], Asum[2];
-        int ninside_pair = 0;
-#pragma unroll
-        for (int dir = 0; dir < 2; dir++) {
-          const int a = dir ? j : i;
-          const DevShape &sa = A.shapes[dir ? shp_j : shp_i];
-          const double sgn = dir ? -1.0 : 1.0;
-          const long long off = dir ? off1 : off0;
-          const int cnt = dir ? cnt1 : cnt0, nin = dir ? nin1 : nin0, xc = dir ? xc1 : xc0;
-          unsigned long long msk = dir ? msk1 : msk0;
-          const int4 eb = dir ? e1b : e0b;
-          NodeSums acc;
-          acc.S0 = acc.S1 = acc.S2 = acc.Av = acc.T0 = acc.T1 = acc.T2 = acc.G0 = acc.G1 = acc.G2 = 0.0; acc.n = 0;
-          double Ra[9];
-#pragma unroll
-          for (int e = 0; e < 9; e++) Ra[e] = A.Rs[e * st + a];
-          if (msk || nin > 0 || cnt > 64 || xc > 0) {
-            double x0[3];
-#pragma unroll
-            for (int r = 0; r < 3; r++) {
-              double hx = Ra[0 + r] * (sgn * d[0]);
-              hx = fma(Ra[3 + r], sgn * d[1], hx);
-              hx = fma(Ra[6 + r], sgn * d[2], hx);
-              x0[r] = -0.5 * hx;
-            }
-            const double *__restrict__ nodes = sa.px;
-            const int nq = sa.nq;
-            while (msk) {
-              const int r = __ffsll((long long)msk) - 1;
-              msk &= msk - 1;
-              add_node(acc, nodes, nq, S.pool[off + r].k, x0);
-            }
-            for (int r = 64; r < cnt; r++)
-              if (S.pool_flag[off + r]) add_node(acc, nodes, nq, S.pool[off + r].k, x0);
-            {
-              const unsigned xo = (unsigned)eb.x;
-              for (int r = 0; r < xc; r++) add_node(acc, nodes, nq, S.inpool[xo + r], x0);
-            }
-            for (int q = 0; q < nin; q++) {
-              const int h = q + 3;
-              const unsigned w = (h >> 1) == 0 ? (unsigned)eb.x : (h >> 1) == 1 ? (unsigned)eb.y : (h >> 1) == 2 ? (unsigned)eb.z : (unsigned)eb.w;
-              add_node(acc, nodes, nq, (int)((w >> (16 * (h & 1))) & 0xffffu), x0);
-            }
-          }
-#pragma unroll
-          for (int r = 0; r < 3; r++) {
-            Ss[dir][r] = Ra[3 * r] * acc.S0 + Ra[3 * r + 1] * acc.S1 + Ra[3 * r + 2] * acc.S2;
-            Ts[dir][r] = Ra[3 * r] * acc.T0 + Ra[3 * r + 1] * acc.T1 + Ra[3 * r + 2] * acc.T2;
-            Gs[dir][r] = 0.25 * (Ra[3 * r] * acc.G0 + Ra[3 * r + 1] * acc.G1 + Ra[3 * r + 2] * acc.G2);
-          }
-          Asum[dir] = acc.Av;
-          ninside_pair += acc.n;
+#pragma unroll
+        for (int u = 0; u < RB; u++)
+          if (k[u] >= 0) add_node(acc, q[u][0], q[u][1], q[u][2], x0);
+      }
+#pragma unroll
+      for (int r = 0; r < 3; r++) {
+        Ss[dir][r] = Ra[3 * r] * acc.S0 + Ra[3 * r + 1] * acc.S1 + Ra[3 * r + 2] * acc.S2;
+        Ts[dir][r] = Ra[3 * r] * acc.T0 + Ra[3 * r + 1] * acc.T1 + Ra[3 * r + 2] * acc.T2;
+        Gs[dir][r] = 0.25 * (Ra[3 * r] * acc.G0 + Ra[3 * r + 1] * acc.G1 + Ra[3 * r + 2] * acc.G2);
+      }
+      Asum[dir] = acc.Av;
+      ninside_pair += acc.n;
+    }
+    const double V = Asum[0] / 3.0 + Asum[1] / 3.0;
+    const bool contact = ninside_pair > 0 && V > 0;
+    if (contact) {
+      const double kk = A.pk[shp_i * SH_MAX_SHAPES + shp_j], mm = A.pm[shp_i * SH_MAX_SHAPES + shp_j];
+      double E, pr;
+      if (mm == 1.0) { E = kk * V; pr = kk; }
+      else { const double pw = pow(V, mm - 1.0); E = kk * pw * V; pr = mm * kk * pw; }
+      out[0] = V; out[1] = E;
+      double li[3], lj[3];
+#pragma unroll
+      for (int r = 0; r < 3; r++) {
+        li[r] = A.c[r * st + i] - A.x[r * st + i];
+        lj[r] = A.c[r * st + j] - A.x[r * st + j];
+      }
+      const double *Sij = Ss[0], *Sji = Ss[1], *Tij = Ts[0], *Tji = Ts[1];
+      const double Ti[3] = {Tij[0] + (li[1] * Sij[2] - li[2] * Sij[1]), Tij[1] + (li[2] * Sij[0] - li[0] * Sij[2]),
+                            Tij[2] + (li[0] * Sij[1] - li[1] * Sij[0])};
+      const double Tj[3] = {Tji[0] + (lj[1] * Sji[2] - lj[2] * Sji[1]), Tji[1] + (lj[2] * Sji[0] - lj[0] * Sji[2]),
+                            Tji[2] + (lj[0] * Sji[1] - lj[1] * Sji[0])};
+#pragma unroll
+      for (int r = 0; r < 3; r++) {
+        out[2 + r] = -pr * (0.5 * (Sij[r] - Sji[r]));
+        out[5 + r] = -pr * Ti[r];
+        out[8 + r] = -pr * Tj[r];
+        out[11 + r] = (A.c[r * st + i] - 0.5 * d[r]) + (Gs[0][r] + Gs[1][r]) / V;
+      }
+      if (A.dissip) contact_dissipation(A, i, j, shp_i, shp_j, d, lj, out);
+    }
+    store_pair_outputs_once(A, S, p, !contact, out);
+    return ninside_pair;
+  }
+}
+
+__global__ void __launch_bounds__(128, 4) pair_reduce_kernel(PairArgs A, SplitArgs S) {
+  constexpr int PPT = 2;
+  __shared__ int s_list[PPT * 128];
+  __shared__ int s_n;
+  if (threadIdx.x == 0) s_n = 0;
+  __syncthreads();
+  const int lane = threadIdx.x & 31;
+  int c_pairs = 0, c_trans = 0, c_ghost = 0;
+#pragma unroll
+  for (int q = 0; q < PPT; q++) {
+    const int p = (blockIdx.x * PPT + q) * 128 + threadIdx.x;
+    bool hit = false;
+    if (p < A.npairs) {
+      const int4 *ep = reinterpret_cast<const int4 *>(S.pd + 2 * (size_t)p);
+      const int4 e0a = __ldg(ep), e0b = __ldg(ep + 1), e1a = __ldg(ep + 2), e1b = __ldg(ep + 3);
+      if (e0a.z >= 0) {
+        c_pairs++; c_trans += (e0a.w & 0xffff) + (e1a.w & 0xffff); c_ghost += A.pair_j[p] >= A.nlocal;
+        hit = e0a.z + e1a.z + ((e0a.w >> 16) & 0xffff) + ((e1a.w >> 16) & 0xffff) + (e0b.y & 0xffff) + (e1b.y & 0xffff) > 0;
+        if (!hit) {
+          double out[14];
+#pragma unroll
+          for (int r = 0; r < 14; r++) out[r] = 0.0;
+          store_pair_outputs_once(A, S, p, true, out);
         }
-        c_inside = ninside_pair;
-        const double V = Asum[0] / 3.0 + Asum[1] / 3.0;
-        if (ninside_pair > 0 && V > 0) {
-          const double kk = A.pk[shp_i * SH_MAX_SHAPES + shp_j], mm = A.pm[shp_i * SH_MAX_SHAPES + shp_j];
-          double E, pr;
-          if (mm == 1.0) { E = kk * V; pr = kk; }
-          else { const double pw = pow(V, mm - 1.0); E = kk * pw * V; pr = mm * kk * pw; }
-          out[0] = V; out[1] = E;
-          double li[3], lj[3];
-#pragma unroll
-          for (int r = 0; r < 3; r++) {
-            li[r] = A.c[r * st + i] - A.x[r * st + i];
-            lj[r] = A.c[r * st + j] - A.x[r * st + j];
-          }
-          const double *Sij = Ss[0], *Sji = Ss[1], *Tij = Ts[0], *Tji = Ts[1];
-          const double Ti[3] = {Tij[0] + (li[1] * Sij[2] - li[2] * Sij[1]), Tij[1] + (li[2] * Sij[0] - li[0] * Sij[2]),
-                                Tij[2] + (li[0] * Sij[1] - li[1] * Sij[0])};
-          const double Tj[3] = {Tji[0] + (lj[1] * Sji[2] - lj[2] * Sji[1]), Tji[1] + (lj[2] * Sji[0] - lj[0] * Sji[2]),
-                                Tji[2] + (lj[0] * Sji[1] - lj[1] * Sji[0])};
-#pragma unroll
-          for (int r = 0; r < 3; r++) {
-            out[2 + r] = -pr * (0.5 * (Sij[r] - Sji[r]));
-            out[5 + r] = -pr * Ti[r];
-            out[8 + r] = -pr * Tj[r];
-            out[11 + r] = (A.c[r * st + i] - 0.5 * d[r]) + (Gs[0][r] + Gs[1][r]) / V;
-          }
-          if (A.dissip) contact_dissipation(A, i, j, shp_i, shp_j, d, lj, out);
-        }
-      }
-#pragma unroll
-      for (int r = 0; r < 14; r++) A.pres[(size_t)r * A.pres_stride + p] = out[r];
-      const int eij = A.pair_eij[p], eji = A.pair_eji[p];
-#pragma unroll
-      for (int r = 0; r < 3; r++) {
-        A.slot[(size_t)r * A.slot_stride + eij] = out[2 + r];
-        A.slot[(size_t)(3 + r) * A.slot_stride + eij] = out[5 + r];
-        if (eji >= 0) {
-          A.slot[(size_t)r * A.slot_stride + eji] = -out[2 + r];
-          A.slot[(size_t)(3 + r) * A.slot_stride + eji] = out[8 + r];
-        }
-      }
-    }
+      } else if (S.out_zero[p]) S.out_zero[p] = 0;
+    }
+    const unsigned m = __ballot_sync(0xffffffffu, hit);
+    int base = 0;
+    if (lane == 0 && m) base = atomicAdd(&s_n, __popc(m));
+    base = __shfl_sync(0xffffffffu, base, 0);
+    if (hit) s_list[base + __popc(m & ((1u << lane) - 1u))] = p;
   }
   c_pairs = __reduce_add_sync(0xffffffffu, c_pairs); c_trans = __reduce_add_sync(0xffffffffu, c_trans);
-  c_inside = __reduce_add_sync(0xffffffffu, c_inside); c_ghost = __reduce_add_sync(0xffffffffu, c_ghost);
-  if ((threadIdx.x & 31) == 0) {
+  c_ghost = __reduce_add_sync(0xffffffffu, c_ghost);
+  if (lane == 0) {
     if (c_pairs) atomicAdd(&A.counters[0], (unsigned long long)c_pairs);
     if (c_trans) atomicAdd(&A.counters[1], (unsigned long long)c_trans);
-    if (c_inside) atomicAdd(&A.counters[3], (unsigned long long)c_inside);
     if (c_ghost) atomicAdd(&A.counters[4], (unsigned long long)c_ghost);
   }
-}
-
-}
+  __syncthreads();
+  const int n = s_n;
+  int c_inside = 0;
+  for (int t = threadIdx.x; t < n; t += 128) c_inside += reduce_contact_pair(A, S, s_list[t]);
+  c_inside = __reduce_add_sync(0xffffffffu, c_inside);
+  if (lane == 0 && c_inside) atomicAdd(&A.counters[3], (unsigned long long)c_inside);
+}
+
+}
diff --git a/lammps-spherharm_b200/csrc/shgpu_api.cu b/lammps-spherharm_b200/csrc/shgpu_api.cu
--- a/lammps-spherharm_b200/csrc/shgpu_api.cu
+++ b/lammps-spherharm_b200/csrc/shgpu_api.cu
@@ -24,7 +24,7 @@
 
 struct ShapeDev {
   DevBuf<double> Ap, node;
-  DevBuf<double2> ab;
+  DevBuf<double2> ab, pn;
   DevBuf<float> row_x, cubew[SH_CACHE_LEVELS];
   DevBuf<float2> cube;
   DevBuf<float4> pf4;
@@ -80,7 +80,9 @@
       nbr_j, pair_i, pair_j, pair_eij, pair_eji, pair_img, scalars;
   DevBuf<double> bbox, slot, pres, stage;
   DevBuf<SurvRec> pool;
-  DevBuf<unsigned char> pool_flag;
+  DevBuf<int> pool_kin;
+  DevBuf<unsigned char> out_zero;
+  bool out_zero_valid = false;
   DevBuf<long long> pool_base, pool_cap;
   DevBuf<PdEntry> pd;
   DevBuf<PairHot> cache_hot[2];
@@ -103,7 +105,6 @@
   int64_t cache_age = 0;
   bool cache_exhausted = false;
   int cube_n = 0;
-  int reduce_occ = 0;
   int eval_pts = 0, eval_occ = 0, eval_mode = 0;
   long long last_records = 0;
   DevBuf<unsigned short> cache_pool[2];
@@ -195,6 +196,17 @@
         CU(cudaMemcpy(d.node.p + (size_t)e * t.nq, t.node_p[e].data(), t.nq * sizeof(double), cudaMemcpyHostToDevice));
         CU(cudaMemcpy(d.node.p + (size_t)(3 + e) * t.nq, t.node_n[e].data(), t.nq * sizeof(double), cudaMemcpyHostToDevice));
       }
+      {
+        std::vector<double2> pn((size_t)4 * t.nq);
+        for (int k = 0; k < t.nq; k++) {
+          pn[4 * (size_t)k] = make_double2(t.node_p[0][k], t.node_p[1][k]);
+          pn[4 * (size_t)k + 1] = make_double2(t.node_p[2][k], t.node_n[0][k]);
+          pn[4 * (size_t)k + 2] = make_double2(t.node_n[1][k], t.node_n[2][k]);
+          pn[4 * (size_t)k + 3] = make_double2(0.0, 0.0);
+        }
+        d.pn.ensure(pn.size());
+        CU(cudaMemcpy(d.pn.p, pn.data(), pn.size() * sizeof(double2), cudaMemcpyHostToDevice));
+      }
       DevShape &v = h->shape_host_view[s];
       v.lmax = t.lmax; v.nterms = t.nterms; v.nq = t.nq; v.nchunks = (t.nq + 31) / 32;
       v.rmax = t.rmax; v.rmin = t.rmin; v.rmax2 = t.rmax * t.rmax; v.rmin2 = t.rmin * t.rmin;
@@ -204,6 +216,7 @@
       v.Ap = d.Ap.p; v.ab = d.ab.p;
       v.px = d.node.p; v.py = d.node.p + t.nq; v.pz = d.node.p + 2 * (size_t)t.nq;
       v.nx = d.node.p + 3 * (size_t)t.nq; v.ny = d.node.p + 4 * (size_t)t.nq; v.nz = d.node.p + 5 * (size_t)t.nq;
+      v.pn = d.pn.p;
       v.n_theta = t.n_theta; v.n_phi = t.n_phi; v.nterms4 = (t.nterms + 3) / 4 * 4; v.row_x = d.row_x.p; v.cube_ul = d.cube.p; v.cube_n = t.cube_n; v.pad2_ = 0; v.pf4 = d.pf4.p;
       for (int lv = 0; lv < SH_CACHE_LEVELS; lv++) { v.cube_w2[lv] = d.cubew[lv].p; v.cache_delta[lv] = t.cache_delta[lv]; }
     }
@@ -350,6 +363,7 @@
   CU(cudaGetLastError());
   h->npairs = npairs; h->nentries = nentries;
   h->list_valid = true; h->steps_since_build = 0; h->neighbor_builds++;
+  h->out_zero_valid = false;
   h->cache_state = keep_cache ? CACHE_REMAP : CACHE_INVALID;
   if (!keep_cache) h->carry = false;
   return 0;
@@ -465,6 +479,7 @@
   if ((rc = absorb_split_feedback(h))) return rc;
   try {
     h->pd.ensure((size_t)2 * np + 2); h->big_list.ensure(np + 1); h->slow_list.ensure(np + 1);
+    if (h->out_zero.cap < (size_t)np + 1) { h->out_zero.ensure(np + 1); h->out_zero_valid = false; }
     h->pool_base.ensure(SH_MAX_SHAPES); h->pool_cap.ensure(SH_MAX_SHAPES); h->split_sc.ensure(1); h->eval_plan.ensure(1); h->split_flags.ensure(4);
   } catch (std::string &e) { return fail(h, e); }
   if (!h->h_pool_count) {
@@ -576,13 +591,13 @@
   for (int s2 = 0; s2 < ns; s2++) { base[s2] = tot; tot += h->h_pool_cap[s2]; }
   if (h->h_in_cap < (long long)np * 2 + 4096) h->h_in_cap = (long long)np * 2 + 4096;
   if (h->h_in_cap > 0xfffffff0LL) h->h_in_cap = 0xfffffff0LL;
-  try { h->pool.ensure((size_t)tot + 64); h->pool_flag.ensure((size_t)tot + 64); h->inpool.ensure((size_t)h->h_in_cap + 64); } catch (std::string &e) { return fail(h, e); }
+  try { h->pool.ensure((size_t)tot + 64); h->pool_kin.ensure((size_t)tot + 64); h->inpool.ensure((size_t)h->h_in_cap + 64); } catch (std::string &e) { return fail(h, e); }
   CU(cudaMemcpyAsync(h->pool_base.p, base.data(), ns * sizeof(long long), cudaMemcpyHostToDevice, h->stream));
   CU(cudaMemcpyAsync(h->pool_cap.p, h->h_pool_cap.data(), ns * sizeof(long long), cudaMemcpyHostToDevice, h->stream));
   CU(cudaMemsetAsync(h->split_sc.p, 0, sizeof(SplitScalars), h->stream));
   SplitArgs S;
-  S.pool = h->pool.p; S.pool_flag = h->pool_flag.p; S.pool_base = h->pool_base.p; S.pool_cap = h->pool_cap.p; S.sc = h->split_sc.p;
-  S.pd = h->pd.p; S.big_list = h->big_list.p; S.slow_list = h->slow_list.p; S.inpool = h->inpool.p; S.in_cap = h->h_in_cap;
+  S.pool = h->pool.p; S.pool_kin = h->pool_kin.p; S.pool_base = h->pool_base.p; S.pool_cap = h->pool_cap.p; S.sc = h->split_sc.p;
+  S.pd = h->pd.p; S.out_zero = h->out_zero.p; S.big_list = h->big_list.p; S.slow_list = h->slow_list.p; S.inpool = h->inpool.p; S.in_cap = h->h_in_cap;
   if (tick(0)) return -2;
   if (C.enabled) {
     const int cw = h->tune_cull_wpb > 0 ? h->tune_cull_wpb : 1;
@@ -616,9 +631,11 @@
   tock();
   h->eval_launches++;
   if (tick(2)) return -2;
-  if (h->reduce_occ == 4) pair_reduce_kernel<4><<<cdiv(np, 128), 128, 0, h->stream>>>(P, S);
-  else if (h->reduce_occ == 8) pair_reduce_kernel<8><<<cdiv(np, 128), 128, 0, h->stream>>>(P, S);
-  else pair_reduce_kernel<6><<<cdiv(np, 128), 128, 0, h->stream>>>(P, S);
+  if (!h->out_zero_valid) {
+    CU(cudaMemsetAsync(h->out_zero.p, 0, (size_t)np, h->stream));
+    h->out_zero_valid = true;
+  }
+  pair_reduce_kernel<<<cdiv(np, 256), 128, 0, h->stream>>>(P, S);
   tock();
   h->kernel_launches++;
   {
@@ -662,10 +679,12 @@
     CU(cudaEventRecord(h->ev[h->ev_used], h->stream));
     int rc;
     if (h->tune_variant & 1) {
+      h->out_zero_valid = false;
       if (nt == 256) rc = launch_pair<256>(h, P, h->tune_ctas_per_sm, pair_smem_bytes(maxT, maxq, 8));
       else if (nt == 64) rc = launch_pair<64>(h, P, h->tune_ctas_per_sm, pair_smem_bytes(maxT, maxq, 2));
       else rc = launch_pair<128>(h, P, h->tune_ctas_per_sm, pair_smem_bytes(maxT, maxq, 4));
     } else if ((h->tune_variant & 4) || (!(h->tune_variant & 16) && h->npairs < 16384)) {
+      h->out_zero_valid = false;
       rc = launch_fused(h, P);
     } else {
       rc = run_split_pipeline(h, P);
@@ -803,7 +822,7 @@
   if (!h) return 0;
   cudaSetDevice(h->device);
   cudaStreamSynchronize(h->stream);
-  for (auto &d : h->shape_dev) { d.Ap.release(); d.ab.release(); d.node.release(); d.row_x.release(); d.cube.release(); d.pf4.release(); for (auto &w : d.cubew) w.release(); }
+  for (auto &d : h->shape_dev) { d.Ap.release(); d.ab.release(); d.node.release(); d.row_x.release(); d.cube.release(); d.pf4.release(); d.pn.release(); for (auto &w : d.cubew) w.release(); }
   h->d_shapes.release(); h->d_pk.release(); h->d_pm.release(); h->d_pgn.release(); h->d_pgt.release(); h->d_pmu.release(); h->stress_part.release();
   DevBuf<double> *db[] = {&h->x, &h->v, &h->q, &h->L, &h->f, &h->tq, &h->c, &h->Rs, &h->c0, &h->wallf, &h->ewall, &h->ke, &h->bbox, &h->slot, &h->pres};
   for (auto *b : db) b->release();
@@ -814,8 +833,8 @@
   h->as_vir.release(); h->as_kin.release(); h->as_en.release(); h->as_send.release(); h->as_recv.release(); h->as_cnt.release(); h->as_epair.release();
   for (auto &e : h->ev) cudaEventDestroy(e);
   for (auto &e : h->ev2) cudaEventDestroy(e);
-  h->pool.release(); h->pool_flag.release(); h->pool_base.release(); h->pool_cap.release(); h->split_sc.release(); h->eval_plan.release(); h->slow_list.release();
-  h->pd.release(); h->big_list.release(); h->split_flags.release(); h->inpool.release();
+  h->pool.release(); h->pool_kin.release(); h->pool_base.release(); h->pool_cap.release(); h->split_sc.release(); h->eval_plan.release(); h->slow_list.release();
+  h->pd.release(); h->out_zero.release(); h->big_list.release(); h->split_flags.release(); h->inpool.release();
   for (int k = 0; k < 2; k++) { h->cache_hot[k].release(); h->cache_pool[k].release(); }
   h->old_c.release(); h->old_cc0.release(); h->old_cq0.release(); h->old_tag.release(); h->ghost_hash.release(); h->amap.release();
   h->old_half_off.release(); h->old_pair_j.release(); h->fresh_list.release(); h->cache_count.release(); h->cc0.release(); h->cq0.release(); h->drift.release();
@@ -1631,7 +1650,6 @@
   const int v = (int)value;
   if (k == "cull_wpb") { if (v != 0 && v != 1 && v != 2 && v != 4 && v != 8) return fail(h, "cull_wpb must be 0, 1, 2, 4 or 8"); h->tune_cull_wpb = v; }
   else if (k == "cull_lpp") { if (v != 0 && v != 16 && v != 32) return fail(h, "cull_lpp must be 0, 16 or 32"); h->tune_cull_lpp = v; }
-  else if (k == "reduce_occ") { if (v != 0 && v != 4 && v != 6 && v != 8) return fail(h, "reduce_occ must be 0, 4, 6 or 8"); h->reduce_occ = v; }
   else if (k == "eval_pts") { if (v != 0 && v != 2 && v != 4) return fail(h, "eval_pts must be 0, 2 or 4"); h->eval_pts = v; }
   else if (k == "eval_occ") { if (v != 0 && v != 3 && v != 4) return fail(h, "eval_occ must be 0, 3 or 4"); h->eval_occ = v; }
   else if (k == "eval_mode") { if (v < 0 || v > 2) return fail(h, "eval_mode must be 0 (default), 1 (one block per CTA) or 2 (persistent chunks)"); h->eval_mode = v; }
```
